# hmatuschek/libsdr

Hardware: AMD Instinct MI355X
Metric: Msamples/s through baseband->FIR->demod chain (higher is better)
Workload: dtype i16

## Files before the change

### include/sdrhip.h

```cpp
#ifndef SDRHIP_H
#define SDRHIP_H

#include <stddef.h>
#include <stdint.h>

#ifdef __cplusplus
extern "C" {
#endif

#define SDRHIP_VERSION 100

enum {
  SDRHIP_OK = 0,
  SDRHIP_E_INVALID = -1,
  SDRHIP_E_NODEVICE = -2,
  SDRHIP_E_HIP = -3,
  SDRHIP_E_NOMEM = -4,
  SDRHIP_E_UNSUPPORTED = -5,
  SDRHIP_E_SIZE = -6
};

enum {
  SDRHIP_EPI_NONE = 0,
  SDRHIP_EPI_FM = 1,
  SDRHIP_EPI_AM = 2,
  SDRHIP_EPI_USB = 3
};

typedef struct sdrhip_ctx sdrhip_ctx;
typedef struct sdrhip_timer sdrhip_timer;
typedef struct sdrhip_iqbb_i16 sdrhip_iqbb_i16;
typedef struct sdrhip_fir sdrhip_fir;
typedef struct sdrhip_demod sdrhip_demod;
typedef struct sdrhip_subsample sdrhip_subsample;
typedef struct sdrhip_fftconv sdrhip_fftconv;
typedef struct sdrhip_fbb_f32 sdrhip_fbb_f32;

int sdrhip_version(void);
const char *sdrhip_strerror(int code);
const char *sdrhip_last_error(void);
int sdrhip_device_count(int *count);

int sdrhip_ctx_create(int device, void *stream, sdrhip_ctx **out);
int sdrhip_ctx_destroy(sdrhip_ctx *ctx);
int sdrhip_ctx_synchronize(sdrhip_ctx *ctx);
int sdrhip_ctx_device_name(sdrhip_ctx *ctx, char *buf, size_t len);

int sdrhip_malloc(sdrhip_ctx *ctx, size_t bytes, void **dptr);
int sdrhip_free(sdrhip_ctx *ctx, void *dptr);
int sdrhip_memcpy_h2d(sdrhip_ctx *ctx, void *dst_dev, const void *src_host, size_t bytes);
int sdrhip_memcpy_d2h(sdrhip_ctx *ctx, void *dst_host, const void *src_dev, size_t bytes);
int sdrhip_memset(sdrhip_ctx *ctx, void *dst_dev, int value, size_t bytes);

int sdrhip_timer_create(sdrhip_ctx *ctx, sdrhip_timer **out);
int sdrhip_timer_start(sdrhip_timer *t);
int sdrhip_timer_stop(sdrhip_timer *t);
int sdrhip_timer_elapsed_ms(sdrhip_timer *t, float *ms);
int sdrhip_timer_destroy(sdrhip_timer *t);

int sdrhip_bench_stream_read(sdrhip_ctx *ctx, const void *dev, size_t bytes, int iters, double *gb_per_s);

int sdrhip_design_iqbb_taps(double filter_freq, double width, double sample_rate, int order, int32_t *taps);
int sdrhip_design_bb_taps(double filter_freq, double width, double sample_rate, int order, int32_t *taps);
int sdrhip_design_iqbb_decim(double sample_rate, int sub_sample, double out_rate, int *decim);
int sdrhip_design_freqshift_lut_i16(int32_t *lut);
int sdrhip_design_freqshift_inc(double shift, double sample_rate, uint32_t *inc);
int sdrhip_design_fir_lowpass(int order, double upper_freq, double sample_rate, double *alpha);
int sdrhip_design_fftfilt_kernel(int n, double fmin, double fmax, double sample_rate, float *h);
int sdrhip_design_fftfilt_spectrum(int n, const float *h, float *spectrum);
int sdrhip_design_fftfilt_kernel_f64(int n, double fmin, double fmax, double sample_rate, double *h);
int sdrhip_design_fftfilt_spectrum_f64(int n, const double *h, double *spectrum);

int sdrhip_iqbb_i16_create(sdrhip_ctx *ctx, const int32_t *taps, int order, const int32_t *lut,
                           uint32_t lut_inc, int negative, int decim, int channels, size_t max_in,
                           int epilogue, sdrhip_iqbb_i16 **out);
int sdrhip_iqbb_i16_path(sdrhip_iqbb_i16 *h, int *path);
int sdrhip_iqbb_i16_kernel_names(sdrhip_iqbb_i16 *h, char *buf, size_t len);
int sdrhip_iqbb_i16_plan_info(sdrhip_iqbb_i16 *h, int *info, int n);
int sdrhip_iqbb_i16_out_count(sdrhip_iqbb_i16 *h, size_t n_in, size_t *n_out);
int sdrhip_iqbb_i16_process(sdrhip_iqbb_i16 *h, const int16_t *in_host, size_t n_in, size_t in_stride,
                            void *out_host, size_t out_stride, size_t *n_out);
int sdrhip_iqbb_i16_process_dev(sdrhip_iqbb_i16 *h, const int16_t *in_dev, size_t n_in, size_t in_stride,
                                void *out_dev, size_t out_stride, size_t *n_out);
int sdrhip_iqbb_i16_process_dev_multi(sdrhip_iqbb_i16 *h, const int16_t *in_dev, size_t n_buffers, size_t n_per_buffer, size_t in_stride,
                                      void *out_dev, size_t out_stride, size_t *n_out_per_buffer, size_t *n_out_total);
enum { SDRHIP_IN_CS16 = 0, SDRHIP_IN_CU8 = 1 };
int sdrhip_iqbb_i16_set_input_format(sdrhip_iqbb_i16 *h, int format);
int sdrhip_bb_i16_create(sdrhip_ctx *ctx, const int32_t *taps, int order, const int32_t *lut,
                         uint32_t lut_inc, int negative, int decim, int channels, size_t max_in,
                         int epilogue, sdrhip_iqbb_i16 **out);
int sdrhip_design_freqshift_lut_i8(int32_t *lut);
int sdrhip_iqbb_i8_create(sdrhip_ctx *ctx, const int32_t *taps, int order, const int32_t *lut, uint32_t lut_inc,
                          int negative, int decim, int channels, size_t max_in, int epilogue, sdrhip_iqbb_i16 **out);
int sdrhip_iqbb_i16_set_taps(sdrhip_iqbb_i16 *h, const int32_t *taps);
int sdrhip_iqbb_i16_set_shift(sdrhip_iqbb_i16 *h, uint32_t lut_inc, int negative);
int sdrhip_iqbb_i16_reset(sdrhip_iqbb_i16 *h, int keep_history);
enum { SDRHIP_KEEP_RING = 1, SDRHIP_KEEP_FM = 2, SDRHIP_KEEP_COUNTERS = 4 };
int sdrhip_iqbb_i16_adopt_state(sdrhip_iqbb_i16 *h, sdrhip_iqbb_i16 *from, int what);
int sdrhip_iqbb_i16_destroy(sdrhip_iqbb_i16 *h);

typedef struct sdrhip_tuner_i16 sdrhip_tuner_i16;
int sdrhip_tuner_i16_create(sdrhip_ctx *ctx, const int32_t *taps, int order, const int32_t *lut, const uint32_t *lut_inc,
                            const int *negative, int decim, int channels, size_t max_in, int epilogue, sdrhip_tuner_i16 **out);
int sdrhip_tunermodes_i16_create(sdrhip_ctx *ctx, const int32_t *taps, int order, const int32_t *lut, const uint32_t *lut_inc,
                                 const int *negative, const int *modes, int decim, int channels, size_t max_in,
                                 sdrhip_tuner_i16 **out);
int sdrhip_tunerbb_i16_create(sdrhip_ctx *ctx, const int32_t *taps, int order, const int32_t *lut, const uint32_t *lut_inc,
                              const int *negative, int decim, int channels, size_t max_in, int epilogue, sdrhip_tuner_i16 **out);
int sdrhip_tunermodes_bb_i16_create(sdrhip_ctx *ctx, const int32_t *taps, int order, const int32_t *lut, const uint32_t *lut_inc,
                                    const int *negative, const int *modes, int decim, int channels, size_t max_in,
                                    sdrhip_tuner_i16 **out);
int sdrhip_tunermodes_i16_set_mode(sdrhip_tuner_i16 *h, int channel, int mode);
int sdrhip_tunermodes_i16_get_modes(sdrhip_tuner_i16 *h, int *modes, int n);
int sdrhip_tuner_i16_kernel_names(sdrhip_tuner_i16 *h, char *buf, size_t len);
int sdrhip_tuner_i16_plan_info(sdrhip_tuner_i16 *h, size_t n_in, int *info, int n);
int sdrhip_tuner_i16_out_count(sdrhip_tuner_i16 *h, size_t n_in, size_t *n_out);
int sdrhip_tuner_i16_process(sdrhip_tuner_i16 *h, const void *in_host, size_t n_in, void *out_host, size_t out_stride, size_t *n_out);
int sdrhip_tuner_i16_process_dev(sdrhip_tuner_i16 *h, const void *in_dev, size_t n_in, void *out_dev, size_t out_stride, size_t *n_out);
int sdrhip_tuner_i16_set_taps(sdrhip_tuner_i16 *h, int channel, const int32_t *taps);
int sdrhip_tuner_i16_set_shift(sdrhip_tuner_i16 *h, int channel, uint32_t lut_inc, int negative);
int sdrhip_tuner_i16_set_input_format(sdrhip_tuner_i16 *h, int format);
int sdrhip_tuner_i16_reset(sdrhip_tuner_i16 *h, int keep_history);
int sdrhip_tuner_i16_destroy(sdrhip_tuner_i16 *h);

enum {
  SDRHIP_FIR_CS16_EXACT = 0,
  SDRHIP_FIR_CF32 = 1
};
int sdrhip_fir_create(sdrhip_ctx *ctx, int kind, const double *alpha, int order, int decim, int channels,
                      size_t max_in, int epilogue, sdrhip_fir **out);
int sdrhip_fir_out_count(sdrhip_fir *h, size_t n_in, size_t *n_out);
int sdrhip_fir_kernel_names(sdrhip_fir *h, size_t n_in, char *buf, size_t len);
int sdrhip_fir_last_kernels(sdrhip_fir *h, char *buf, size_t len);
int sdrhip_fir_process(sdrhip_fir *h, const void *in_host, size_t n_in, size_t in_stride, void *out_host,
                       size_t out_stride, size_t *n_out);
int sdrhip_fir_process_dev(sdrhip_fir *h, const void *in_dev, size_t n_in, size_t in_stride, void *out_dev,
                           size_t out_stride, size_t *n_out);
int sdrhip_fir_set_taps(sdrhip_fir *h, const double *alpha);
int sdrhip_fir_reset(sdrhip_fir *h);
int sdrhip_fir_destroy(sdrhip_fir *h);

enum { SDRHIP_T_CS16 = 0, SDRHIP_T_CF32 = 1, SDRHIP_T_CS8 = 2 ,
       SDRHIP_T_CF64 = 3  };
int sdrhip_demod_create(sdrhip_ctx *ctx, int kind, int dtype, int channels, size_t max_in, int inplace_fm0,
                        sdrhip_demod **out);
int sdrhip_demod_process(sdrhip_demod *h, const void *in_host, size_t n, size_t in_stride, void *out_host,
                         size_t out_stride);
int sdrhip_demod_process_dev(sdrhip_demod *h, const void *in_dev, size_t n, size_t in_stride, void *out_dev,
                             size_t out_stride);
int sdrhip_demod_reset(sdrhip_demod *h);
int sdrhip_demod_destroy(sdrhip_demod *h);

typedef struct sdrhip_deemph sdrhip_deemph;
int sdrhip_design_fmdeemph_alpha(double sample_rate, int *alpha);
int sdrhip_deemph_i16_create(sdrhip_ctx *ctx, int alpha, int channels, size_t max_in, sdrhip_deemph **out);
int sdrhip_deemph_i16_process(sdrhip_deemph *h, const int16_t *in_host, size_t n, size_t in_stride, int16_t *out_host,
                              size_t out_stride);
int sdrhip_deemph_i16_process_dev(sdrhip_deemph *h, const int16_t *in_dev, size_t n, size_t in_stride, int16_t *out_dev,
                                  size_t out_stride);
int sdrhip_deemph_i16_kernel_names(sdrhip_deemph *h, size_t n, char *buf, size_t len);
int sdrhip_deemph_i16_reset(sdrhip_deemph *h);
int sdrhip_deemph_i16_destroy(sdrhip_deemph *h);

int sdrhip_design_fsk_lut(double sample_rate, float baud, float freq, int *corr_len, float *lut, int lut_cap);
enum { SDRHIP_DET_FSK = 0, SDRHIP_DET_ASK = 1 };
typedef struct sdrhip_detector sdrhip_detector;
int sdrhip_detector_create(sdrhip_ctx *ctx, int kind, const float *mark_lut, const float *space_lut, int corr_len, int invert,
                           int channels, size_t max_in, sdrhip_detector **out);
int sdrhip_detector_process(sdrhip_detector *h, const int16_t *in_host, size_t n, size_t in_stride, uint8_t *out_host,
                            size_t out_stride);
int sdrhip_detector_process_dev(sdrhip_detector *h, const int16_t *in_dev, size_t n, size_t in_stride, uint8_t *out_dev,
                                size_t out_stride);
int sdrhip_detector_kernel_names(sdrhip_detector *h, char *buf, size_t len);
int sdrhip_detector_reset(sdrhip_detector *h);
int sdrhip_detector_destroy(sdrhip_detector *h);
enum { SDRHIP_BITS_NORMAL = 0, SDRHIP_BITS_TRANSITION = 1 };
typedef struct sdrhip_bits sdrhip_bits;
int sdrhip_bits_create(sdrhip_ctx *ctx, double sample_rate, float baud, int mode, int channels, size_t max_in, sdrhip_bits **out);
int sdrhip_bits_corr_len(sdrhip_bits *h, int *corr_len);
int sdrhip_bits_out_capacity(sdrhip_bits *h, size_t n_in, size_t *cap);
int sdrhip_bits_process(sdrhip_bits *h, const uint8_t *sym_host, size_t n, size_t in_stride, uint8_t *bits_host, size_t out_stride,
                        uint32_t *counts_host);
int sdrhip_bits_process_dev(sdrhip_bits *h, const uint8_t *sym_dev, size_t n, size_t in_stride, uint8_t *bits_dev, size_t out_stride,
                            uint32_t *counts_dev);
int sdrhip_bits_kernel_names(sdrhip_bits *h, char *buf, size_t len);
int sdrhip_bits_reset(sdrhip_bits *h);
int sdrhip_bits_destroy(sdrhip_bits *h);
int sdrhip_detectorbank_create(sdrhip_ctx *ctx, const int *kinds, const int *corr_len, const int *invert, const float *mark_luts,
                               const float *space_luts, int max_corr_len, int channels, size_t max_in, sdrhip_detector **out);
int sdrhip_detectorbank_set_channel(sdrhip_detector *h, int channel, int kind, const float *mark_lut, const float *space_lut,
                                    int corr_len, int invert);
int sdrhip_bitsbank_create(sdrhip_ctx *ctx, double sample_rate, const float *baud, const int *mode, int channels, size_t max_in,
                           int max_corr_len, sdrhip_bits **out);
int sdrhip_bitsbank_set_channel(sdrhip_bits *h, int channel, float baud, int mode);
int sdrhip_bitsbank_channel_info(sdrhip_bits *h, int channel, size_t n_in, int *corr_len, float *omega_min, float *omega_max,
                                 size_t *cap);

int sdrhip_subsample_create(sdrhip_ctx *ctx, int dtype, size_t n, int channels, size_t max_in,
                            sdrhip_subsample **out);
int sdrhip_subsample_out_count(sdrhip_subsample *h, size_t n_in, size_t *n_out);
int sdrhip_subsample_process(sdrhip_subsample *h, const void *in_host, size_t n_in, size_t in_stride,
                             void *out_host, size_t out_stride, size_t *n_out);
int sdrhip_subsample_process_dev(sdrhip_subsample *h, const void *in_dev, size_t n_in, size_t in_stride,
                                 void *out_dev, size_t out_stride, size_t *n_out);
int sdrhip_subsample_reset(sdrhip_subsample *h);
int sdrhip_subsample_destroy(sdrhip_subsample *h);

enum {
  SDRHIP_FFTCONV_OLA = 0,
  SDRHIP_FFTCONV_OLS = 1
};
int sdrhip_fftconv_create(sdrhip_ctx *ctx, int mode, int fft_size, const float *kernel, int n_taps,
                          int channels, size_t max_in, sdrhip_fftconv **out);
int sdrhip_fftconv_create_bank(sdrhip_ctx *ctx, int mode, int fft_size, const float *kernels, int n_taps, int n_bands,
                               int channels, size_t max_in, sdrhip_fftconv **out);
int sdrhip_fftconv_bands(sdrhip_fftconv *h, int *n_bands);
int sdrhip_fftconv_set_kernel(sdrhip_fftconv *h, int band, const float *kernel);
int sdrhip_fftconv_process(sdrhip_fftconv *h, const float *in_host, size_t n_in, size_t in_stride,
                           float *out_host, size_t out_stride);
int sdrhip_fftconv_process_dev(sdrhip_fftconv *h, const float *in_dev, size_t n_in, size_t in_stride,
                               float *out_dev, size_t out_stride);
int sdrhip_fftconv_last_kernels(sdrhip_fftconv *h, char *buf, size_t len);
int sdrhip_fftconv_reset(sdrhip_fftconv *h);
int sdrhip_fftconv_destroy(sdrhip_fftconv *h);
int sdrhip_fftconv_f64_create_bank(sdrhip_ctx *ctx, int mode, int fft_size, const double *kernels, int n_taps, int n_bands,
                                   int channels, size_t max_in, sdrhip_fftconv **out);
int sdrhip_fftconv_f64_set_kernel(sdrhip_fftconv *h, int band, const double *kernel);
int sdrhip_fftconv_f64_process(sdrhip_fftconv *h, const double *in_host, size_t n_in, size_t in_stride,
                               double *out_host, size_t out_stride);
int sdrhip_fftconv_f64_process_dev(sdrhip_fftconv *h, const double *in_dev, size_t n_in, size_t in_stride,
                                   double *out_dev, size_t out_stride);
// ... 70 lines not shown
```

### libsdr_amd/abi.py

```python
import ctypes as C
import os
import re

_HERE = os.path.dirname(os.path.abspath(__file__))
ROOT = os.path.dirname(_HERE)
SO_PATH = os.path.join(_HERE, "libsdrhip.so")
if os.environ.get("SDRHIP_LIB"):
    SO_PATH = os.path.abspath(os.environ["SDRHIP_LIB"])
HEADER = os.path.join(ROOT, "include", "sdrhip.h")

OK, E_INVALID, E_NODEVICE, E_HIP, E_NOMEM, E_UNSUPPORTED, E_SIZE = 0, -1, -2, -3, -4, -5, -6
EPI_NONE, EPI_FM, EPI_AM, EPI_USB = 0, 1, 2, 3
FIR_CS16_EXACT, FIR_CF32 = 0, 1
T_CS16, T_CF32, T_CS8, T_CF64 = 0, 1, 2, 3
IN_CS16, IN_CU8 = 0, 1
KEEP_RING, KEEP_FM, KEEP_COUNTERS = 1, 2, 4
FFTCONV_OLA, FFTCONV_OLS = 0, 1
DET_FSK, DET_ASK = 0, 1
BITS_NORMAL, BITS_TRANSITION = 0, 1


class SdrHipError(RuntimeError):
    def __init__(self, code, text):
        super().__init__("sdrhip error %d: %s" % (code, text))
        self.code = code


def header_functions():
    src = open(HEADER).read()
    src = re.sub(r"/\*.*?\*/", "", src, flags=re.S)
    return sorted(set(re.findall(r"\b(sdrhip_[a-z0-9_]+)\s*\(", src)))


def _signatures():
    vp, sz = C.c_void_p, C.c_size_t
    pvp, psz = C.POINTER(C.c_void_p), C.POINTER(C.c_size_t)
    i32p, f32p, f64p = C.POINTER(C.c_int32), C.POINTER(C.c_float), C.POINTER(C.c_double)
    return {
        "sdrhip_version": (C.c_int, []),
        "sdrhip_strerror": (C.c_char_p, [C.c_int]),
        "sdrhip_last_error": (C.c_char_p, []),
        "sdrhip_device_count": (C.c_int, [C.POINTER(C.c_int)]),
        "sdrhip_ctx_create": (C.c_int, [C.c_int, vp, pvp]),
        "sdrhip_ctx_destroy": (C.c_int, [vp]),
        "sdrhip_ctx_synchronize": (C.c_int, [vp]),
        "sdrhip_ctx_device_name": (C.c_int, [vp, C.c_char_p, sz]),
        "sdrhip_malloc": (C.c_int, [vp, sz, pvp]),
        "sdrhip_free": (C.c_int, [vp, vp]),
        "sdrhip_memcpy_h2d": (C.c_int, [vp, vp, vp, sz]),
        "sdrhip_memcpy_d2h": (C.c_int, [vp, vp, vp, sz]),
        "sdrhip_memset": (C.c_int, [vp, vp, C.c_int, sz]),
        "sdrhip_timer_create": (C.c_int, [vp, pvp]),
        "sdrhip_timer_start": (C.c_int, [vp]),
        "sdrhip_timer_stop": (C.c_int, [vp]),
        "sdrhip_timer_elapsed_ms": (C.c_int, [vp, f32p]),
        "sdrhip_timer_destroy": (C.c_int, [vp]),
        "sdrhip_bench_stream_read": (C.c_int, [vp, vp, sz, C.c_int, C.POINTER(C.c_double)]),
        "sdrhip_design_iqbb_taps": (C.c_int, [C.c_double, C.c_double, C.c_double, C.c_int, i32p]),
        "sdrhip_design_bb_taps": (C.c_int, [C.c_double, C.c_double, C.c_double, C.c_int, i32p]),
        "sdrhip_design_iqbb_decim": (C.c_int, [C.c_double, C.c_int, C.c_double, C.POINTER(C.c_int)]),
        "sdrhip_design_freqshift_lut_i16": (C.c_int, [i32p]),
        "sdrhip_design_freqshift_inc": (C.c_int, [C.c_double, C.c_double, C.POINTER(C.c_uint32)]),
        "sdrhip_design_fir_lowpass": (C.c_int, [C.c_int, C.c_double, C.c_double, f64p]),
        "sdrhip_design_fftfilt_kernel": (C.c_int, [C.c_int, C.c_double, C.c_double, C.c_double, f32p]),
        "sdrhip_design_fftfilt_spectrum": (C.c_int, [C.c_int, f32p, f32p]),
        "sdrhip_iqbb_i16_create": (C.c_int, [vp, i32p, C.c_int, i32p, C.c_uint32, C.c_int, C.c_int, C.c_int,
                                             sz, C.c_int, pvp]),
        "sdrhip_bb_i16_create": (C.c_int, [vp, i32p, C.c_int, i32p, C.c_uint32, C.c_int, C.c_int, C.c_int,
                                           sz, C.c_int, pvp]),
        "sdrhip_iqbb_i16_path": (C.c_int, [vp, C.POINTER(C.c_int)]),
        "sdrhip_design_freqshift_lut_i8": (C.c_int, [i32p]),
        "sdrhip_iqbb_i8_create": (C.c_int, [vp, i32p, C.c_int, i32p, C.c_uint32, C.c_int, C.c_int, C.c_int, sz, C.c_int, pvp]),
        "sdrhip_iqbb_i16_kernel_names": (C.c_int, [vp, C.c_char_p, sz]),
        "sdrhip_iqbb_i16_set_taps": (C.c_int, [vp, i32p]),
        "sdrhip_iqbb_i16_set_shift": (C.c_int, [vp, C.c_uint32, C.c_int]),
        "sdrhip_iqbb_i16_out_count": (C.c_int, [vp, sz, psz]),
        "sdrhip_iqbb_i16_process": (C.c_int, [vp, vp, sz, sz, vp, sz, psz]),
        "sdrhip_iqbb_i16_process_dev": (C.c_int, [vp, vp, sz, sz, vp, sz, psz]),
        "sdrhip_iqbb_i16_plan_info": (C.c_int, [vp, C.POINTER(C.c_int), C.c_int]),
        "sdrhip_iqbb_i16_process_dev_multi": (C.c_int, [vp, vp, sz, sz, sz, vp, sz, psz, psz]),
        "sdrhip_iqbb_i16_reset": (C.c_int, [vp, C.c_int]),
        "sdrhip_iqbb_i16_adopt_state": (C.c_int, [vp, vp, C.c_int]),
        "sdrhip_iqbb_i16_destroy": (C.c_int, [vp]),
        "sdrhip_tuner_i16_create": (C.c_int, [vp, i32p, C.c_int, i32p, C.POINTER(C.c_uint32), C.POINTER(C.c_int), C.c_int, C.c_int,
                                              sz, C.c_int, pvp]),
        "sdrhip_tunermodes_i16_create": (C.c_int, [vp, i32p, C.c_int, i32p, C.POINTER(C.c_uint32), C.POINTER(C.c_int), C.POINTER(C.c_int),
                                                   C.c_int, C.c_int, sz, pvp]),
        "sdrhip_tunerbb_i16_create": (C.c_int, [vp, i32p, C.c_int, i32p, C.POINTER(C.c_uint32), C.POINTER(C.c_int), C.c_int, C.c_int,
                                                sz, C.c_int, pvp]),
        "sdrhip_tunermodes_bb_i16_create": (C.c_int, [vp, i32p, C.c_int, i32p, C.POINTER(C.c_uint32), C.POINTER(C.c_int), C.POINTER(C.c_int),
                                                      C.c_int, C.c_int, sz, pvp]),
        "sdrhip_tunermodes_i16_set_mode": (C.c_int, [vp, C.c_int, C.c_int]),
        "sdrhip_tunermodes_i16_get_modes": (C.c_int, [vp, C.POINTER(C.c_int), C.c_int]),
        "sdrhip_tuner_i16_kernel_names": (C.c_int, [vp, C.c_char_p, sz]),
        "sdrhip_tuner_i16_plan_info": (C.c_int, [vp, sz, C.POINTER(C.c_int), C.c_int]),
        "sdrhip_tuner_i16_out_count": (C.c_int, [vp, sz, psz]),
        "sdrhip_tuner_i16_process": (C.c_int, [vp, vp, sz, vp, sz, psz]),
        "sdrhip_tuner_i16_process_dev": (C.c_int, [vp, vp, sz, vp, sz, psz]),
        "sdrhip_tuner_i16_set_taps": (C.c_int, [vp, C.c_int, i32p]),
        "sdrhip_tuner_i16_set_shift": (C.c_int, [vp, C.c_int, C.c_uint32, C.c_int]),
        "sdrhip_tuner_i16_set_input_format": (C.c_int, [vp, C.c_int]),
        "sdrhip_tuner_i16_reset": (C.c_int, [vp, C.c_int]),
        "sdrhip_tuner_i16_destroy": (C.c_int, [vp]),
        "sdrhip_fir_create": (C.c_int, [vp, C.c_int, f64p, C.c_int, C.c_int, C.c_int, sz, C.c_int, pvp]),
        "sdrhip_fir_out_count": (C.c_int, [vp, sz, psz]),
        "sdrhip_fir_kernel_names": (C.c_int, [vp, sz, C.c_char_p, sz]),
        "sdrhip_fir_last_kernels": (C.c_int, [vp, C.c_char_p, sz]),
        "sdrhip_fir_process": (C.c_int, [vp, vp, sz, sz, vp, sz, psz]),
        "sdrhip_fir_process_dev": (C.c_int, [vp, vp, sz, sz, vp, sz, psz]),
        "sdrhip_fir_reset": (C.c_int, [vp]),
        "sdrhip_fir_set_taps": (C.c_int, [vp, f64p]),
        "sdrhip_fir_destroy": (C.c_int, [vp]),
        "sdrhip_demod_create": (C.c_int, [vp, C.c_int, C.c_int, C.c_int, sz, C.c_int, pvp]),
        "sdrhip_demod_process": (C.c_int, [vp, vp, sz, sz, vp, sz]),
        "sdrhip_demod_process_dev": (C.c_int, [vp, vp, sz, sz, vp, sz]),
        "sdrhip_demod_reset": (C.c_int, [vp]),
        "sdrhip_demod_destroy": (C.c_int, [vp]),
        "sdrhip_design_fmdeemph_alpha": (C.c_int, [C.c_double, C.POINTER(C.c_int)]),
        "sdrhip_deemph_i16_create": (C.c_int, [vp, C.c_int, C.c_int, sz, pvp]),
        "sdrhip_deemph_i16_process": (C.c_int, [vp, vp, sz, sz, vp, sz]),
        "sdrhip_deemph_i16_process_dev": (C.c_int, [vp, vp, sz, sz, vp, sz]),
        "sdrhip_deemph_i16_kernel_names": (C.c_int, [vp, sz, C.c_char_p, sz]),
        "sdrhip_deemph_i16_reset": (C.c_int, [vp]),
        "sdrhip_deemph_i16_destroy": (C.c_int, [vp]),
        "sdrhip_design_fsk_lut": (C.c_int, [C.c_double, C.c_float, C.c_float, C.POINTER(C.c_int), f32p, C.c_int]),
        "sdrhip_detector_create": (C.c_int, [vp, C.c_int, f32p, f32p, C.c_int, C.c_int, C.c_int, sz, pvp]),
        "sdrhip_detector_process": (C.c_int, [vp, vp, sz, sz, vp, sz]),
        "sdrhip_detector_process_dev": (C.c_int, [vp, vp, sz, sz, vp, sz]),
        "sdrhip_detector_kernel_names": (C.c_int, [vp, C.c_char_p, sz]),
        "sdrhip_detector_reset": (C.c_int, [vp]),
        "sdrhip_detector_destroy": (C.c_int, [vp]),
        "sdrhip_bits_create": (C.c_int, [vp, C.c_double, C.c_float, C.c_int, C.c_int, sz, pvp]),
        "sdrhip_bits_corr_len": (C.c_int, [vp, C.POINTER(C.c_int)]),
        "sdrhip_bits_out_capacity": (C.c_int, [vp, sz, psz]),
        "sdrhip_bits_process": (C.c_int, [vp, vp, sz, sz, vp, sz, vp]),
        "sdrhip_bits_process_dev": (C.c_int, [vp, vp, sz, sz, vp, sz, vp]),
        "sdrhip_bits_kernel_names": (C.c_int, [vp, C.c_char_p, sz]),
        "sdrhip_bits_reset": (C.c_int, [vp]),
        "sdrhip_bits_destroy": (C.c_int, [vp]),
        "sdrhip_detectorbank_create": (C.c_int, [vp, C.POINTER(C.c_int), C.POINTER(C.c_int), C.POINTER(C.c_int), f32p, f32p,
                                                         C.c_int, C.c_int, sz, pvp]),
        "sdrhip_detectorbank_set_channel": (C.c_int, [vp, C.c_int, C.c_int, f32p, f32p, C.c_int, C.c_int]),
        "sdrhip_bitsbank_create": (C.c_int, [vp, C.c_double, f32p, C.POINTER(C.c_int), C.c_int, sz, C.c_int, pvp]),
        "sdrhip_bitsbank_set_channel": (C.c_int, [vp, C.c_int, C.c_float, C.c_int]),
        "sdrhip_bitsbank_channel_info": (C.c_int, [vp, C.c_int, sz, C.POINTER(C.c_int), f32p, f32p, psz]),
        "sdrhip_iqbb_i16_set_input_format": (C.c_int, [vp, C.c_int]),
        "sdrhip_subsample_create": (C.c_int, [vp, C.c_int, sz, C.c_int, sz, pvp]),
        "sdrhip_subsample_out_count": (C.c_int, [vp, sz, psz]),
        "sdrhip_subsample_process": (C.c_int, [vp, vp, sz, sz, vp, sz, psz]),
        "sdrhip_subsample_process_dev": (C.c_int, [vp, vp, sz, sz, vp, sz, psz]),
        "sdrhip_subsample_reset": (C.c_int, [vp]),
        "sdrhip_subsample_destroy": (C.c_int, [vp]),
        "sdrhip_fftconv_create": (C.c_int, [vp, C.c_int, C.c_int, f32p, C.c_int, C.c_int, sz, pvp]),
        "sdrhip_fftconv_process": (C.c_int, [vp, vp, sz, sz, vp, sz]),
        "sdrhip_fftconv_process_dev": (C.c_int, [vp, vp, sz, sz, vp, sz]),
        "sdrhip_fftconv_last_kernels": (C.c_int, [vp, C.c_char_p, sz]),
        "sdrhip_fftconv_reset": (C.c_int, [vp]),
        "sdrhip_fftconv_destroy": (C.c_int, [vp]),
        "sdrhip_fft_c2c": (C.c_int, [vp, C.c_int, C.c_int, C.c_int, vp, vp]),
        "sdrhip_fft_c2c_f64": (C.c_int, [vp, C.c_int, C.c_int, C.c_int, vp, vp]),
        "sdrhip_fft_exec": (C.c_int, [vp, C.c_int, C.c_int, C.c_int, vp, vp]),
        "sdrhip_fbb_f32_create": (C.c_int, [vp, C.c_double, C.c_double, f64p, C.c_int, C.c_int, C.c_int, sz, pvp]),
        "sdrhip_fbb_f32_out_count": (C.c_int, [vp, sz, psz]),
        "sdrhip_fbb_f32_kernel_names": (C.c_int, [vp, sz, C.c_char_p, sz]),
        "sdrhip_fbb_f32_last_kernels": (C.c_int, [vp, C.c_char_p, sz]),
        "sdrhip_fbb_f32_process": (C.c_int, [vp, vp, sz, sz, vp, sz, psz]),
        "sdrhip_fbb_f32_process_dev": (C.c_int, [vp, vp, sz, sz, vp, sz, psz]),
        "sdrhip_fbb_f32_reset": (C.c_int, [vp]),
        "sdrhip_fbb_f32_set_taps": (C.c_int, [vp, f64p]),
        "sdrhip_fbb_f32_set_shift": (C.c_int, [vp, C.c_double]),
        "sdrhip_fbb_f32_destroy": (C.c_int, [vp]),
        "sdrhip_fftconv_create_bank": (C.c_int, [vp, C.c_int, C.c_int, f32p, C.c_int, C.c_int, C.c_int, sz, pvp]),
        "sdrhip_fftconv_bands": (C.c_int, [vp, C.POINTER(C.c_int)]),
        "sdrhip_fftconv_set_kernel": (C.c_int, [vp, C.c_int, f32p]),
        "sdrhip_design_fftfilt_kernel_f64": (C.c_int, [C.c_int, C.c_double, C.c_double, C.c_double, f64p]),
        "sdrhip_design_fftfilt_spectrum_f64": (C.c_int, [C.c_int, f64p, f64p]),
        "sdrhip_fftconv_f64_create_bank": (C.c_int, [vp, C.c_int, C.c_int, f64p, C.c_int, C.c_int, C.c_int, sz, pvp]),
        "sdrhip_fftconv_f64_set_kernel": (C.c_int, [vp, C.c_int, f64p]),
        "sdrhip_fftconv_f64_process": (C.c_int, [vp, vp, sz, sz, vp, sz]),
        "sdrhip_fftconv_f64_process_dev": (C.c_int, [vp, vp, sz, sz, vp, sz]),
        "sdrhip_fft_plan_create": (C.c_int, [vp, C.c_int, C.c_int, pvp]),
        "sdrhip_fft_plan_form": (C.c_int, [vp, C.POINTER(C.c_char_p)]),
        "sdrhip_fft_plan_exec_dev": (C.c_int, [vp, C.c_int, C.c_int, vp, vp]),
        "sdrhip_fft_plan_exec": (C.c_int, [vp, C.c_int, vp, vp]),
        "sdrhip_fft_plan_destroy": (C.c_int, [vp]),
        "sdrhip_fftsink_create": (C.c_int, [vp, C.c_int, C.c_int, C.c_int, sz, pvp]),
        "sdrhip_fftsink_process": (C.c_int, [vp, vp, sz, sz, vp, sz]),
        "sdrhip_fftsink_process_dev": (C.c_int, [vp, vp, sz, sz, vp, sz]),
        "sdrhip_fftsink_form": (C.c_int, [vp, C.POINTER(C.c_char_p)]),
        "sdrhip_fftsink_destroy": (C.c_int, [vp]),
        "sdrhip_fftsource_create": (C.c_int, [vp, C.c_int, C.c_int, vp, C.c_int, sz, pvp]),
        "sdrhip_fftsource_set_kernel": (C.c_int, [vp, vp]),
        "sdrhip_fftsource_process": (C.c_int, [vp, vp, sz, sz, vp, sz]),
        "sdrhip_fftsource_process_dev": (C.c_int, [vp, vp, sz, sz, vp, sz]),
        "sdrhip_fftsource_form": (C.c_int, [vp, C.POINTER(C.c_char_p)]),
        "sdrhip_fftsource_reset": (C.c_int, [vp]),
        "sdrhip_fftsource_destroy": (C.c_int, [vp]),
        "sdrhip_comm_create": (C.c_int, [C.POINTER(C.c_int), C.c_int, pvp]),
        "sdrhip_comm_size": (C.c_int, [vp, C.POINTER(C.c_int)]),
        "sdrhip_comm_ctx": (C.c_int, [vp, C.c_int, pvp]),
        "sdrhip_comm_transport": (C.c_int, [vp, C.POINTER(C.c_char_p)]),
        "sdrhip_comm_broadcast": (C.c_int, [vp, pvp, sz, C.c_int]),
        "sdrhip_comm_gather": (C.c_int, [vp, pvp, psz, vp, C.c_int]),
        "sdrhip_comm_gather_begin": (C.c_int, [vp, C.c_int, pvp, psz, vp, C.c_int]),
        "sdrhip_comm_gather_wait": (C.c_int, [vp, C.c_int]),
        "sdrhip_comm_synchronize": (C.c_int, [vp]),
        "sdrhip_comm_destroy": (C.c_int, [vp]),
        "sdrhip_host_alloc": (C.c_int, [sz, pvp]),
        "sdrhip_host_free": (C.c_int, [vp]),
        "sdrhip_host_register": (C.c_int, [vp, sz]),
        "sdrhip_host_unregister": (C.c_int, [vp]),
        "sdrhip_memcpy_h2d_async": (C.c_int, [vp, vp, vp, sz]),
        "sdrhip_memcpy_d2h_async": (C.c_int, [vp, vp, vp, sz]),
        "sdrhip_memcpy2d_d2h_async": (C.c_int, [vp, vp, sz, vp, sz, sz, sz]),
    }


SIGNATURES = _signatures()

_lib = None


def lib():
    global _lib
    if _lib is None:
        if not os.path.exists(SO_PATH):
            raise ImportError("libsdrhip.so not built: run `python -c 'import __graft_entry__ as g; g.build()'` "
                              "(make -C libsdr_amd/csrc); there is no CPU fallback")
        L = C.CDLL(SO_PATH)
        for name, (res, args) in SIGNATURES.items():
            fn = getattr(L, name)
            fn.restype, fn.argtypes = res, args
# ... 10 lines not shown
```

### libsdr_amd/csrc/iqbb_common.hpp

```cpp
#pragma once
#include "fm_phi.hpp"
#include "sdrhip_internal.hpp"

#include <cstdlib>

using namespace sdrhip;

namespace sdrhip {

constexpr int TPB = 256;
constexpr int R = 8;
constexpr int TI = TPB * R;
constexpr int TAPC = 8;
constexpr int MAX_ORDER = 2048;

typedef short s16x2 __attribute__((ext_vector_type(2)));
typedef int v4i __attribute__((ext_vector_type(4)));
typedef int v16i __attribute__((ext_vector_type(16)));

struct IqbbArgs {
  const uint32_t *in; long in_stride;
  int in_cu8;
  int in_real;
  int i8;
  const uint32_t *hist_old; uint32_t *hist_new;
  const int2 *acc_old; int2 *acc_new;
  const short *fm_old; short *fm_new;
  const uint2 *taps;
  const int2 *lut; uint32_t inc; int negative;
  int OP, HH, D, N;
  uint32_t n0_lo;
  int base0_rel;
  int n_groups;
  int n_out;
  int extra0;
  int CG, OG, ovl;
  int CGr;
  void *out; long out_stride; int epilogue;
  const v4i *tapfrag; int cre, cim;
  unsigned ah_mask;
  int lpg;
  int tiles, tpw;
  int bt_hi;
  int fix_lo, fix_hi;
};

constexpr int HOT_EPI_PARTIAL = 4;

struct HotArgs {
  const void *in; long in_stride;
  void *out; long out_stride;
  const v4i *tapfrag; const int2 *lut;
  uint32_t inc, n0_lo; int negative;
  int base0_rel, OG, ovl;
  int t_lo, t_hi, tpw;
  int G, U, dq, dr;
  int N, n_out;
  int C;
  int cre, cim;
  int D, GS, lpg_sh; float inv_d;
  short *philast; int philast_stride;
  int tiles_h;
  long long reserved[2];
  int2 *part; int part_stride;
  int Dreal, base_real;
  int fin_groups, fin_out, fin_epi;
  int mb_q1, mb_p, mb_qlast; unsigned mb_magic;
  unsigned long long *stamps;
};

}

namespace {

__device__ __forceinline__ uint32_t cast_cu8(uint32_t u16) {
  return (((u16 & 0xffu) + 129u) & 0xffu) << 8 | ((((u16 >> 8) & 0xffu) + 129u) & 0xffu) << 24;
}
__device__ __forceinline__ uint32_t raw_x(const IqbbArgs &a, int c, long rel) {
  if (a.in_cu8) return cast_cu8(reinterpret_cast<const uint16_t *>(a.in)[(long)c * a.in_stride + rel]);
  if (a.in_real) return (uint32_t)(int)reinterpret_cast<const short *>(a.in)[(long)c * a.in_stride + rel];
  if (a.i8) {
    const uint32_t u = reinterpret_cast<const uint16_t *>(a.in)[(long)c * a.in_stride + rel];
    return ((uint32_t)(int)(signed char)(u & 0xffu) & 0xffffu) | ((uint32_t)(int)(signed char)(u >> 8) << 16);
  }
  return a.in[(long)c * a.in_stride + rel];
}
__device__ __forceinline__ uint32_t load_x(const IqbbArgs &a, int c, int rel) {
  if (rel >= 0) return rel < a.N ? raw_x(a, c, rel) : 0u;
  const int h = a.HH + rel;
  return h >= 0 ? a.hist_old[(long)c * a.HH + h] : 0u;
}

__device__ __forceinline__ int dot2(uint32_t x, uint32_t k, int acc) {
  return __builtin_amdgcn_sdot2(__builtin_bit_cast(s16x2, x), __builtin_bit_cast(s16x2, k), acc, false);
}

__device__ __forceinline__ int2 rotate_i16(uint32_t inc, int negative, const int2 *lut_s, int2 r, uint32_t n_lo) {
  if (inc == 0) return r;
  uint32_t idx = (__umul24(n_lo & 32767u, inc & 32767u) & 32767u) >> 8;
  if (negative) idx = 127u - idx;
  const int2 L = lut_s[idx];
  int2 v;
  v.x = (int)((unsigned)__mul24(L.x, r.x) - (unsigned)__mul24(L.y, r.y)) >> 16;
  v.y = (int)((unsigned)__mul24(L.x, r.y) + (unsigned)__mul24(L.y, r.x)) >> 16;
  return v;
}
__device__ __forceinline__ int2 rotate(const IqbbArgs &a, const int2 *lut_s, int2 r, uint32_t n_lo) {
  if (a.i8) {
    r.x = (short)r.x; r.y = (short)r.y;
    if (a.inc == 0) return r;
    uint32_t idx = (__umul24(n_lo & 32767u, a.inc & 32767u) & 32767u) >> 8;
    if (a.negative) idx = 127u - idx;
    const int2 L = lut_s[idx];
    int2 v;
    v.x = (int)(short)(mulw(L.x, r.x) - mulw(L.y, r.y)) >> 8;
    v.y = (int)(short)(mulw(L.x, r.y) + mulw(L.y, r.x)) >> 8;
    return v;
  }
  return rotate_i16(a.inc, a.negative, lut_s, r, n_lo);
}

__device__ __forceinline__ int box_div(int s, int D) {
  const int n = mulw(D, D);
  const int r = mulw(s, D);
  if (n == 0) return 0;
  if (r == (int)0x80000000 && n == -1) return r;
  return r / n;
}


struct BigdArgs {
  const int2 *part; int part_stride;
  int D, base0_rel, N, n_groups, n_out, epi, C;
  const int2 *acc_old; int2 *acc_new;
  const short *fm_old; short *fm_new;
  void *out; long out_stride;
};
__device__ __forceinline__ void bigd_finish_group(const BigdArgs &a, int c, int q) {
  const int2 *pc = a.part + (long)c * a.part_stride;
  auto group_sum = [&](int g) {
    const long lo = g == 0 ? 0 : (long)a.base0_rel + (long)g * a.D, hi = min((long)a.base0_rel + (long)(g + 1) * a.D, (long)a.N);
    int2 s = make_int2(0, 0);
    if (g == 0) s = a.acc_old[c];
    for (long sl = lo >> 9; sl <= (hi - 1) >> 9; sl++) {
      const long x0 = sl << 9;
      const int gf = x0 < a.base0_rel ? 0 : (int)((x0 - a.base0_rel) / a.D);
      const int2 v = pc[3 * sl + (g - gf)];
      s.x = (int)((unsigned)s.x + (unsigned)v.x); s.y = (int)((unsigned)s.y + (unsigned)v.y);
    }
    return s;
  };
  const int2 s = group_sum(q);
  const bool emits = q < a.n_out;
  if (q == a.n_groups - 1) a.acc_new[c] = emits ? make_int2(0, 0) : s;
  if (!emits) return;
  const int yr = (short)box_div(s.x, a.D), yi = (short)box_div(s.y, a.D);
  if (a.epi == SDRHIP_EPI_NONE) {
    reinterpret_cast<uint32_t *>(a.out)[(long)c * a.out_stride + q] = ((uint32_t)(uint16_t)yr) | ((uint32_t)(uint16_t)yi << 16);
  } else if (a.epi == SDRHIP_EPI_AM) {
    reinterpret_cast<short *>(a.out)[(long)c * a.out_stride + q] = am_i16(yr, yi);
  } else if (a.epi == SDRHIP_EPI_USB) {
    reinterpret_cast<short *>(a.out)[(long)c * a.out_stride + q] = usb_i16(yr, yi);
  } else {
    const int phi = fm_phi(yr, yi);
    short o;
    if (q == 0) o = (short)yr;
    else if (q == 1) o = (short)((int)a.fm_old[c] - phi);
    else {
      const int2 sp = group_sum(q - 1);
      o = (short)(fm_phi((short)box_div(sp.x, a.D), (short)box_div(sp.y, a.D)) - phi);
    }
    reinterpret_cast<short *>(a.out)[(long)c * a.out_stride + q] = o;
    if (q == a.n_out - 1 && a.n_out >= 2) a.fm_new[c] = (short)phi;
  }
}

__device__ __forceinline__ void finalize_group(const IqbbArgs &a, int c, const int2 *lut_s, uint32_t *ybuf, int ql, int q, int2 s, int D) {
  if (q == 0) {
    const int2 carry = a.acc_old[c];
    s.x = (int)((unsigned)s.x + (unsigned)carry.x);
    s.y = (int)((unsigned)s.y + (unsigned)carry.y);
    if (a.extra0) {
      int er = 0, ei = 0;
      for (int i = 0; i < a.OP; i++) {
        const uint32_t x = load_x(a, c, -(a.OP - 1) + i);
        const uint2 k = a.taps[i];
        er = dot2(x, k.x, er); ei = dot2(x, k.y, ei);
      }
      const int2 v = rotate(a, lut_s, make_int2(er >> 14, ei >> 14), a.n0_lo);
      s.x = (int)((unsigned)s.x + (unsigned)v.x);
      s.y = (int)((unsigned)s.y + (unsigned)v.y);
    }
  }
  const bool emits = q < a.n_out;
  if (emits) {
    int yr = (short)box_div(s.x, D), yi = (short)box_div(s.y, D);
    if (a.i8) { yr = (signed char)yr; yi = (signed char)yi; }
    ybuf[ql] = ((uint32_t)(uint16_t)yr) | ((uint32_t)(uint16_t)yi << 16);
    if (a.epilogue == SDRHIP_EPI_FM) reinterpret_cast<int *>(ybuf + a.CGr)[ql] = fm_phi(yr, yi);
  }
  if (q == a.n_groups - 1) a.acc_new[c] = emits ? make_int2(0, 0) : s;
}

__device__ __forceinline__ void epilogue_and_roll(const IqbbArgs &a, int c, int tile, int tid, int q0, int groups_here,
                                                  const uint32_t *ybuf) {
  for (int ql = a.ovl + tid; ql < groups_here; ql += TPB) {
    const int j = q0 + ql;
    if (j >= a.n_out) continue;
    const uint32_t y = ybuf[ql];
    const int yr = (short)(y & 0xffffu), yi = (short)(y >> 16);
    if (a.epilogue == SDRHIP_EPI_NONE) {
      if (a.i8) reinterpret_cast<uint16_t *>(a.out)[(long)c * a.out_stride + j] = (uint16_t)((yr & 0xff) | ((yi & 0xff) << 8));
      else reinterpret_cast<uint32_t *>(a.out)[(long)c * a.out_stride + j] = y;
    } else {
      short o;
      if (a.epilogue == SDRHIP_EPI_AM) o = am_i16(yr, yi);
      else if (a.epilogue == SDRHIP_EPI_USB) o = usb_i16(yr, yi);
      else {
        const int *phib = reinterpret_cast<const int *>(ybuf + a.CGr);
        const int phi = phib[ql];
// ... 229 lines not shown
```

### libsdr_amd/csrc/iqbb_hot.hpp

```cpp
#pragma once
#include <atomic>
#include "iqbb_common.hpp"

#include <iterator>
#include <type_traits>
#include <utility>

namespace sdrhip {

enum { HOT_CS16 = 0, HOT_CU8 = 1, HOT_REAL = 2, HOT_CS8 = 3 };
constexpr bool hot_one_plane(int in) { return in == HOT_CU8 || in == HOT_CS8; }
constexpr int hot_halo(int S, int in) { return in == HOT_REAL ? 32 * S - 16 : 16 * (S - 1); }
constexpr int hot_win(int S, int in) { return 512 + hot_halo(S, in) + (in == HOT_REAL ? 16 : 0); }
constexpr int hot_plb(int S, int in) { return in == HOT_REAL ? hot_win(S, in) : 2 * hot_win(S, in) + 32; }
constexpr int hot_bufb(int S, int in) { return hot_one_plane(in) ? hot_plb(S, in) : 2 * hot_plb(S, in); }
constexpr int hot_lds_bytes(int S, int NH, int in, int NW, bool wide) {
  return (wide ? 4096 : 1024) + (S + NH) * 1024 + NW * 2 * hot_bufb(S, in);
}
constexpr int hot_lds_cap(int NW, int S = 0) { return S >= 33 ? 163840 : NW == 4 ? 40960 : NW == 8 ? 81920 : 163840; }
constexpr bool hot_wide(int S, int NH, int in, int NW, int extra = 0) { return hot_lds_bytes(S, NH, in, NW, true) + extra <= hot_lds_cap(NW, S); }
constexpr int hot_anyd_extra(int, int, bool = true, int NW = 4) { return NW * 512; }

constexpr int hot_sd_extra(int S, int in, bool rot, int NW = 4) { return (hot_bufb(S, in) >= 2048 ? 0 : NW * 2048) + (rot ? 0 : NW * 2048); }
constexpr bool hot_sd_fits(int S, int NH, int in, bool rot, int NW = 4) { return hot_lds_bytes(S, NH, in, NW, false) + hot_sd_extra(S, in, rot, NW) <= hot_lds_cap(NW); }
constexpr int hot_sd_nw(int S, int NH, int in, bool rot, int nw0) {
  for (int nw = nw0; nw <= 16; nw *= 2) if (hot_sd_fits(S, NH, in, rot, nw)) return nw;
  return 0;
}

struct HotRange { int S0, NH, NW; };
constexpr HotRange hot_ranges_2[] = {{0, 2, 4}};
constexpr HotRange hot_ranges_3[] = {{1, 2, 4}, {0, 3, 4}};
constexpr HotRange hot_ranges_5[] = {{1, 3, 4}, {0, 5, 4}};
constexpr HotRange hot_ranges_9[] = {{3, 3, 4}, {2, 5, 4}, {1, 7, 4}, {0, 9, 4}};
constexpr HotRange hot_ranges_17[] = {{6, 5, 8}, {4, 9, 8}, {0, 17, 16}};
constexpr HotRange hot_ranges_33[] = {{12, 9, 8}, {16, 9, 8}, {18, 9, 8}, {8, 17, 8}, {0, 33, 8}};
struct HotLoRange { int L0, NL; };
constexpr HotLoRange hot_lo_ranges_9[] = {{1, 7}, {0, 9}};
template <int S> constexpr HotLoRange hot_lo_full[] = {{0, S}};

constexpr int hot_steps[] = {2, 3, 5, 9, 17, 33};
template <int S> constexpr auto &hot_ranges_of() {
  if constexpr (S == 2) return hot_ranges_2;
  else if constexpr (S == 3) return hot_ranges_3;
  else if constexpr (S == 5) return hot_ranges_5;
  else if constexpr (S == 9) return hot_ranges_9;
  else if constexpr (S == 17) return hot_ranges_17;
  else return hot_ranges_33;
}
template <int S> constexpr auto &hot_lo_ranges_of() {
  if constexpr (S == 9) return hot_lo_ranges_9;
  else return hot_lo_full<S>;
}
template <int N, class F, int... I>
void hot_pick(int i, F &&f, std::integer_sequence<int, I...>) {
  if (i < 0 || i >= N) i = N - 1;
  ((i == I ? f(std::integral_constant<int, I>{}) : void()), ...);
}
template <int N, class F> void hot_pick(int i, F &&f) { hot_pick<N>(i, f, std::make_integer_sequence<int, N>{}); }
template <class F> bool hot_with_steps(int S, F &&f) {
  constexpr int N = (int)std::size(hot_steps);
  for (int i = 0; i < N; i++)
    if (hot_steps[i] == S) { hot_pick<N>(i, [&](auto k) { f(std::integral_constant<int, hot_steps[decltype(k)::value]>{}); }); return true; }
  return false;
}
inline const HotRange *hot_ranges(int S, int *count) {
  const HotRange *r = nullptr;
  *count = 0;
  hot_with_steps(S, [&](auto s) { r = hot_ranges_of<s>(); *count = (int)std::size(hot_ranges_of<s>()); });
  return r;
}
inline const HotLoRange *hot_lo_ranges(int S, int *count) {
  const HotLoRange *r = nullptr;
  *count = 0;
  hot_with_steps(S, [&](auto s) { r = hot_lo_ranges_of<s>(); *count = (int)std::size(hot_lo_ranges_of<s>()); });
  return r;
}

enum { HOT_D8 = 0, HOT_ANYD = 1, HOT_SD = 2 };
constexpr bool hot_class(int form, int S, int in) {
  if (in == HOT_REAL) return S == 3 || S == 5 || S == 9;
  if (in == HOT_CS8) return form != HOT_SD && (S == 2 || S == 3 || S == 5 || S == 9);
  return S == 2 || S == 3 || S == 5 || S == 9 || S == 17 || (S == 33 && form != HOT_SD);
}
constexpr int hot_sd_range_waves(int S, const HotRange &r, int in, bool rot) {
  const int nw = hot_sd_nw(S, r.NH, in, rot, r.NW);
  return in != HOT_REAL || nw == 4 ? nw : 0;
}
inline int hot_sd_waves(int S, int in, int range, bool rot) {
  int n = 0;
  const HotRange *rg = hot_ranges(S, &n);
  if (!hot_class(HOT_SD, S, in)) return 0;
  return hot_sd_range_waves(S, rg[range >= 0 && range < n ? range : n - 1], in, rot);
}

struct HotLaunch { unsigned grid; hipStream_t stream; };
template <int FORM, int S, int IN> struct HotClass {
  static void launch(int range, int lo, bool rot, int epi, const HotLaunch &, const HotArgs &, const IqbbArgs &);
};
void hot_launch(int form, int S, int in, int range, int lo, bool rot, int epi, const HotLaunch &, const HotArgs &, const IqbbArgs &);

}

namespace {

__device__ __forceinline__ uint32_t ror8(uint32_t x) { return __builtin_amdgcn_alignbit(x, x, 8); }
__device__ __forceinline__ uint32_t add129_rot(uint32_t x) {
  unsigned k = 0x81008100u;
  asm("" : "+s"(k));
  uint32_t t;
  asm("v_pk_add_u16 %0, %1, %2" : "=v"(t) : "v"(x), "s"(k));
  t = ror8(t);
  asm("v_pk_add_u16 %0, %1, %2" : "=v"(t) : "v"(t), "s"(k));
  return t;
}

__host__ __device__ __forceinline__ bool slice_is_hot(int halo, int win, int base0_rel, int OG, int ovl, int N, int n_out, int tile, int w,
                                                      int D = 8, int GS = 64) {
  const int qf = tile * OG - ovl + w * (GS - ovl);
  const int ws = base0_rel + qf * D - halo;
  return ws >= 0 && ws + win <= N && qf >= (GS == 1 ? 2 : 1) && qf + GS - 1 < n_out - 1;
}

template <int S, int S0, int NH, bool ROT, int EPI, int IN, int NW, bool DG = false, bool SD = false, int L0 = 0, int NL = S>
__device__ __forceinline__ void iqbb_hot_body(const HotArgs &a, const IqbbArgs &b_kernarg) {
  IqbbArgs b_late;
  const IqbbArgs &b = DG ? b_late : b_kernarg;
  constexpr bool CS8 = IN == HOT_CS8, CU8 = IN == HOT_CU8 || CS8, REAL = IN == HOT_REAL;
  static_assert(!CS8 || (!SD && EPI != HOT_EPI_PARTIAL && (EPI == SDRHIP_EPI_NONE || EPI == SDRHIP_EPI_FM)), "int8 chain: /8 and any-D forms, no demodulator or FM");
  constexpr bool PART = EPI == HOT_EPI_PARTIAL;
  static_assert(!PART || (DG && !SD), "partial sums: a variant of the any-D form");
  static_assert(!SD || DG, "the small-decimation form is a variant of the any-D form");

  const int DD = DG ? a.D : 8, GS = DG ? a.GS : 64;
  static_assert(S >= 2 && S0 >= 0 && NH >= 1 && S0 + NH <= S, "high-plane range inside the K loop");
  static_assert(L0 >= 0 && L0 + NL <= S && S0 >= L0 && S0 + NH <= L0 + NL, "high-plane range inside the low-plane range");
  static_assert(!REAL || NW == 4, "real input: 4-wave workgroups");
  static_assert(NW == 4 || NW == 8 || NW == 16, "4-wave virtual workgroups");
  constexpr int HALO = hot_halo(S, IN), WIN = hot_win(S, IN), PLB = hot_plb(S, IN), HALF = PLB / 2, BUFB = hot_bufb(S, IN);
  constexpr int NPIECE = (IN == HOT_CS16 ? 4 * WIN : 2 * WIN) / 16;
  constexpr int KSB = REAL ? 32 : 16;
  constexpr int FSH = REAL ? 16 : 14;
  constexpr int NDMA = (NPIECE + 63) / 64;
  constexpr int LASTL = NPIECE - 64 * (NDMA - 1);
  static_assert(NDMA <= 4, "immediate offsets 0 / 1024 / 2048 / 3072");
  constexpr bool WIDE = SD ? false : hot_wide(S, NH, IN, NW, DG ? hot_anyd_extra(S, IN, ROT, NW) : 0);
  static_assert(!SD || hot_sd_fits(S, NH, IN, ROT, NW), "small-decimation form: LDS budget");
  constexpr int NBUF = 2;
  static_assert(hot_lds_bytes(S, NH, IN, NW, WIDE) <= hot_lds_cap(NW, S), "LDS budget for 4 waves per SIMD");
  constexpr int TBLW = WIDE ? 1024 : 256;
  constexpr int TPBH = 64 * NW;
  extern __shared__ __attribute__((aligned(16))) uint32_t smem[];
  int2 *lut_s = reinterpret_cast<int2 *>(smem);
  v4i *taps_s = reinterpret_cast<v4i *>(smem + TBLW);
  const int tid = threadIdx.x, w = __builtin_amdgcn_readfirstlane(tid >> 6), l = tid & 63, n = l & 31, h = l >> 5;
  const int wv = w & 3;
  const int bx = (int)blockIdx.x * (NW / 4) + (w >> 2), gx = (int)gridDim.x * (NW / 4);
  char *wbase = reinterpret_cast<char *>(smem + TBLW + (S + NH) * 64 * 4) + w * (NBUF * BUFB);
  char *pendb = reinterpret_cast<char *>(smem + TBLW + (S + NH) * 64 * 4) + NW * (NBUF * BUFB) + w * 512;
  char *gscb = reinterpret_cast<char *>(smem + TBLW + (S + NH) * 64 * 4) + NW * (NBUF * BUFB) + (SD ? 0 : NW * 512) + w * 2048;
  char *gscb2 = gscb + NW * 2048;
  for (int i = tid; i < S * 64; i += TPBH) taps_s[i] = a.tapfrag[(2 * (i >> 6) + 1) * 64 + (i & 63)];
  for (int i = tid; i < NH * 64; i += TPBH) taps_s[S * 64 + i] = a.tapfrag[(2 * (S0 + (i >> 6))) * 64 + (i & 63)];
  if (tid < 256) {
    const int2 e = a.lut[(tid & 127) ^ (a.negative ? 127 : 0)];
    if (WIDE) reinterpret_cast<v4i *>(smem)[tid] = v4i{e.x, e.y, -e.y, 0};
    else if (tid < 128) lut_s[tid] = e;
  }

  const int OGw = GS - a.ovl, gw = wv * OGw;
  int hl = a.t_lo, hh = a.t_hi;
  while (hl < hh && !slice_is_hot(HALO, WIN, a.base0_rel, a.OG, a.ovl, a.N, a.n_out, hl, wv, DD, GS)) hl++;
  while (hh > hl && !slice_is_hot(HALO, WIN, a.base0_rel, a.OG, a.ovl, a.N, a.n_out, hh - 1, wv, DD, GS)) hh--;
  int u = bx;
  int c = u / a.G, g = u - c * a.G;
  int tile = max(a.t_lo + g * a.tpw, hl), tend = min(a.t_lo + g * a.tpw + a.tpw, hh);
  auto next_unit = [&](int &u_, int &c_, int &g_, int &tile_, int &tend_) {
    do {
      u_ += gx; c_ += a.dq; g_ += a.dr;
      if (g_ >= a.G) { g_ -= a.G; c_++; }
      tile_ = max(a.t_lo + g_ * a.tpw, hl); tend_ = min(a.t_lo + g_ * a.tpw + a.tpw, hh);
    } while (u_ < a.U && tile_ >= tend_);
  };
  if (u < a.U && tile >= tend) next_unit(u, c, g, tile, tend);
  const uint32_t lane_byte = 16u * (uint32_t)l;
  constexpr int SB = IN == HOT_CS16 ? 4 : 2;
  constexpr int OB = (EPI == SDRHIP_EPI_NONE && !CS8) ? 4 : 2;
  const int tile_in_bytes = a.OG * DD * SB, tile_out_bytes = a.OG * OB;
  const uint32_t tile_cnt = (uint32_t)(a.OG * DD) * a.inc;
  const uint32_t cnt0 = (a.n0_lo + (uint32_t)(a.base0_rel + (gw - a.ovl) * DD)) * a.inc;
  auto chan_src = [&](int c_) { return reinterpret_cast<const char *>(a.in) + ((long)c_ * a.in_stride + (a.base0_rel + (gw - a.ovl) * DD - HALO)) * SB; };
  auto chan_out = [&](int c_) { return reinterpret_cast<char *>(a.out) + ((long)c_ * a.out_stride + (gw - a.ovl)) * OB; };
  const char *srcb = chan_src(c);
  char *outb = chan_out(c);
  auto dma_issue = [&](const char *src, char *buf) {
    const unsigned ldsb = __builtin_amdgcn_readfirstlane((unsigned)(uintptr_t)buf);
#pragma clang diagnostic push
#pragma clang diagnostic ignored "-Winline-asm"
    if (NDMA == 1) {
      if (l < LASTL) asm volatile("s_mov_b32 m0, %1\n\ts_nop 0\n\tglobal_load_lds_dwordx4 %0, off" :: "v"(src), "s"(ldsb) : "memory", "m0");
    } else if (NDMA == 2) {
      asm volatile("s_mov_b32 m0, %1\n\ts_nop 0\n\tglobal_load_lds_dwordx4 %0, off" :: "v"(src), "s"(ldsb) : "memory", "m0");
      if (l < LASTL) asm volatile("s_mov_b32 m0, %1\n\ts_nop 0\n\tglobal_load_lds_dwordx4 %0, off offset:1024" :: "v"(src), "s"(ldsb) : "memory", "m0");
    } else if (NDMA == 3) {
      asm volatile("s_mov_b32 m0, %1\n\ts_nop 0\n\tglobal_load_lds_dwordx4 %0, off\n\tglobal_load_lds_dwordx4 %0, off offset:1024" :: "v"(src), "s"(ldsb) : "memory", "m0");
      if (l < LASTL) asm volatile("s_mov_b32 m0, %1\n\ts_nop 0\n\tglobal_load_lds_dwordx4 %0, off offset:2048" :: "v"(src), "s"(ldsb) : "memory", "m0");
    } else {
      asm volatile("s_mov_b32 m0, %1\n\ts_nop 0\n\tglobal_load_lds_dwordx4 %0, off\n\tglobal_load_lds_dwordx4 %0, off offset:1024\n\tglobal_load_lds_dwordx4 %0, off offset:2048"
                   :: "v"(src), "s"(ldsb) : "memory", "m0");
      if (l < LASTL) asm volatile("s_mov_b32 m0, %1\n\ts_nop 0\n\tglobal_load_lds_dwordx4 %0, off offset:3072" :: "v"(src), "s"(ldsb) : "memory", "m0");
    }
#pragma clang diagnostic pop
  };
  if (u < a.U) dma_issue(srcb + (long)tile * tile_in_bytes + lane_byte, wbase);
  __syncthreads();

  int dofs[NDMA];
#pragma unroll
  for (int k = 0; k < NDMA; k++) {
    const int p = l + 64 * k;
    if (REAL) dofs[k] = 8 * p;
    else if (CU8) dofs[k] = (p & 1) * HALF + (p >> 1) * 16;
    else { const int j = p >> 1; dofs[k] = (j & 1) * HALF + (j >> 1) * 16 + (p & 1) * 8; }
  }
  const int coff = REAL ? 16 * (n + h) : h * HALF + 16 * n;
  const uint32_t lane_cnt = (uint32_t)(MF_BLK * n + 8 * h) * a.inc;
  const uint32_t lane_pair = (lane_cnt & 0xffffu) | ((lane_cnt + a.inc) << 16);

  v16i cinit;
#pragma unroll
  for (int r = 0; r < 16; r++) cinit[r] = (r & 1) ? a.cim : a.cre;
  asm volatile("" : "+v"(cinit));

#ifdef K1_STAMPS
  unsigned long long st_acc[6] = {0, 0, 0, 0, 0, 0}, st_t = __builtin_amdgcn_s_memtime();
  const unsigned long long st_r0 = __builtin_amdgcn_s_memrealtime();
  unsigned st_tiles = 0;
#define K1_STAMP(i_) do { asm volatile("s_waitcnt lgkmcnt(0)" ::: "memory"); const unsigned long long t_ = __builtin_amdgcn_s_memtime(); st_acc[i_] += t_ - st_t; st_t = t_; } while (0)
#else
#define K1_STAMP(i_) do { } while (0)
#endif
  constexpr int K1_PRIO_ROT = 1, K1_PRIO_SHIFT = 11;
  unsigned prio_it = 0;
  const unsigned prio_slot = __builtin_amdgcn_s_getreg((3 << 11) | 4) & 3u;

  auto stageP = [&](char *cb) __attribute__((always_inline)) {
    uint4 x[NDMA];
#pragma unroll
    for (int k = 0; k < NDMA; k++)
      if (k < NDMA - 1 || l < LASTL) x[k] = *reinterpret_cast<const uint4 *>(cb + 16 * (l + 64 * k));
    asm volatile("" ::: "memory");
#pragma unroll
    for (int k = 0; k < NDMA; k++) {
      if (k < NDMA - 1 || l < LASTL) {
        if (CS8) {
          *reinterpret_cast<uint4 *>(cb + dofs[k]) = make_uint4(x[k].x, x[k].y, x[k].z, x[k].w);
        } else if (CU8) {
          *reinterpret_cast<uint4 *>(cb + dofs[k]) = make_uint4(add129_rot(x[k].x), add129_rot(x[k].y), add129_rot(x[k].z), add129_rot(x[k].w));
        } else {
          uint2 l2, h2;
          l2.x = __builtin_amdgcn_perm(x[k].y, x[k].x, 0x06040200u) ^ 0x80808080u;
          l2.y = __builtin_amdgcn_perm(x[k].w, x[k].z, 0x06040200u) ^ 0x80808080u;
          h2.x = __builtin_amdgcn_perm(x[k].y, x[k].x, 0x07050301u);
          h2.y = __builtin_amdgcn_perm(x[k].w, x[k].z, 0x07050301u);
          *reinterpret_cast<uint2 *>(cb + dofs[k]) = l2;
          *reinterpret_cast<uint2 *>(cb + PLB + dofs[k]) = h2;
        }
      }
    }
  };
  struct KOps { v4i uh, ul, Al, Ah; };
  auto stageK_begin = [&](const char *cb, KOps &o) __attribute__((always_inline)) {
    const char *pl = cb + coff + KSB * L0, *ph = cb + (CU8 ? 0 : PLB) + coff + KSB * L0;
    o.uh = *reinterpret_cast<const v4i *>(ph); o.ul = o.uh;
    if (!CU8) o.ul = *reinterpret_cast<const v4i *>(pl);
    o.Al = taps_s[L0 * 64 + l]; o.Ah = o.Al;
    if (S0 == L0) o.Ah = taps_s[S * 64 + l];
  };
  auto stageK = [&](const char *cb, KOps &o, v16i &acc_hh, v16i &acc_mid, v16i &acc_ll) __attribute__((always_inline)) {
    constexpr int SA = L0, SB = L0 + NL;
    const char *pl = cb + coff, *ph = cb + (CU8 ? 0 : PLB) + coff;
#pragma unroll
    for (int s = SA; s < SB; s++) {
      KOps nx = o;
      if (s + 1 < SB) {
        nx.uh = *reinterpret_cast<const v4i *>(ph + KSB * (s + 1));
        if (!CU8) nx.ul = *reinterpret_cast<const v4i *>(pl + KSB * (s + 1));
        nx.Al = taps_s[(s + 1) * 64 + l];
        if (s + 1 >= S0 && s + 1 < S0 + NH) nx.Ah = taps_s[(S + s + 1 - S0) * 64 + l];
      }
      acc_mid = __builtin_amdgcn_mfma_i32_32x32x32_i8(o.Al, o.uh, acc_mid, 0, 0, 0);
      asm volatile("" : "+v"(acc_mid));
      if (s >= S0 && s < S0 + NH) {
        acc_hh = __builtin_amdgcn_mfma_i32_32x32x32_i8(o.Ah, o.uh, acc_hh, 0, 0, 0);
        asm volatile("" : "+v"(acc_hh));
        if (!CU8) { acc_mid = __builtin_amdgcn_mfma_i32_32x32x32_i8(o.Ah, o.ul, acc_mid, 0, 0, 0); asm volatile("" : "+v"(acc_mid)); }
      }
      if (!CU8) { acc_ll = __builtin_amdgcn_mfma_i32_32x32x32_i8(o.Al, o.ul, acc_ll, 0, 0, 0); asm volatile("" : "+v"(acc_ll)); }
      o = nx;
    }
  };
  int tm_sp = 8, tm_a0 = 0, tm_a1 = 0;
  unsigned tm_m[4] = {0u, 0u, 0u, 0u};
  bool tm_end = false;
  if (DG) {
    const int Lb = 2 * n + h;
    const int g = (8 * Lb + DD - 1) / DD, pos = g * DD;
    tm_sp = (g <= GS && pos < 8 * Lb + 8) ? pos - 8 * Lb : 8;
    const int kk = min(l >> a.lpg_sh, GS - 1);
    const int b0 = (kk * DD) >> 3, b1 = ((kk + 1) * DD) >> 3, b1c = min(b1, 63);
    tm_a0 = 4 * ((b0 >> 1) + 32 * (b0 & 1));
    tm_a1 = 4 * ((b1c >> 1) + 32 * (b1c & 1));
    tm_end = b1 >= 64;
    const int spm = tm_sp < 8 ? tm_sp : (Lb == 63 && GS * DD == 512) ? 8 : 0;
#pragma unroll
    for (int jj = 0; jj < 4; jj++) tm_m[jj] = (2 * jj < spm ? 1u : 0u) | (2 * jj + 1 < spm ? 0x10000u : 0u);
  }
  (void)tm_sp; (void)tm_a0; (void)tm_a1; (void)tm_end; (void)tm_m;
  auto stageE = [&](auto edge_, const v16i &acc_hh, const v16i &acc_mid, const v16i &acc_ll, uint32_t wave_cnt, char *escr, int erel0,
                    int2 *pdst = nullptr, int ob0 = 0) __attribute__((always_inline)) {
    constexpr bool EDGE = decltype(edge_)::value;
    int L[8][3];
    if (ROT) {
      typedef int v2i __attribute__((ext_vector_type(2)));
#pragma unroll
      for (int jj = 0; jj < 4; jj++) {
        const uint32_t wc = (wave_cnt + 2u * jj * a.inc) & 0xffffu, wpair = wc | (wc << 16);
        uint32_t pr, o0, o1;
        asm("v_pk_add_u16 %0, %1, %2" : "=v"(pr) : "v"(lane_pair), "s"(wpair));
        if (WIDE) {
          asm("v_lshlrev_b32_sdwa %0, %1, %2 dst_sel:DWORD dst_unused:UNUSED_PAD src0_sel:DWORD src1_sel:BYTE_1" : "=v"(o0) : "s"(4), "v"(pr));
          asm("v_lshlrev_b32_sdwa %0, %1, %2 dst_sel:DWORD dst_unused:UNUSED_PAD src0_sel:DWORD src1_sel:BYTE_3" : "=v"(o1) : "s"(4), "v"(pr));
          const v4i e0 = *reinterpret_cast<__attribute__((address_space(3))) const v4i *>((uintptr_t)o0);
          const v4i e1 = *reinterpret_cast<__attribute__((address_space(3))) const v4i *>((uintptr_t)o1);
          L[2 * jj][0] = e0.x; L[2 * jj][1] = e0.y; L[2 * jj][2] = e0.z;
          L[2 * jj + 1][0] = e1.x; L[2 * jj + 1][1] = e1.y; L[2 * jj + 1][2] = e1.z;
        } else {
          o0 = (pr >> 5) & (127u << 3); o1 = (pr >> 21) & (127u << 3);
          const v2i e0 = *reinterpret_cast<__attribute__((address_space(3))) const v2i *>((uintptr_t)o0);
          const v2i e1 = *reinterpret_cast<__attribute__((address_space(3))) const v2i *>((uintptr_t)o1);
          L[2 * jj][0] = e0.x; L[2 * jj][1] = e0.y; L[2 * jj + 1][0] = e1.x; L[2 * jj + 1][1] = e1.y;
        }
      }
    }
    int2 sum = make_int2(0, 0);
    int vx[8], vy[8];
#pragma unroll
    for (int j = 0; j < 8; j++) {
      unsigned tre = ((unsigned)acc_hh[2 * j] << 8) + (unsigned)acc_mid[2 * j];
      unsigned tim = ((unsigned)acc_hh[2 * j + 1] << 8) + (unsigned)acc_mid[2 * j + 1];
      int rr, ri;
      if (CS8) {
        asm("v_bfe_i32 %0, %1, 14, 16" : "=v"(rr) : "v"(tre));
        asm("v_bfe_i32 %0, %1, 14, 16" : "=v"(ri) : "v"(tim));
      } else if (CU8) {
        asm("v_bfe_i32 %0, %1, 6, 18" : "=v"(rr) : "v"(tre));
        asm("v_bfe_i32 %0, %1, 6, 18" : "=v"(ri) : "v"(tim));
      } else {
        asm("" : "+v"(tre)); asm("" : "+v"(tim));
        rr = (int)((tre << 8) + (unsigned)acc_ll[2 * j]) >> FSH; ri = (int)((tim << 8) + (unsigned)acc_ll[2 * j + 1]) >> FSH;
      }
      if (EDGE) {
        const int rel = erel0 + j;
        if (rel < 0 || rel >= a.N) { rr = 0; ri = 0; }
      }
      if (ROT) {
        int x = WIDE ? mad24a(L[j][0], rr, mul24a(L[j][2], ri)) : sub32(mul24a(L[j][0], rr), mul24a(L[j][1], ri));
        int y = mad24a(L[j][0], ri, mul24a(L[j][1], rr));
        if (CS8) {
          asm("v_bfe_i32 %0, %0, 8, 8" : "+v"(x));
          asm("v_bfe_i32 %0, %0, 8, 8" : "+v"(y));
        }
        if (DG) { vx[j] = x; vy[j] = y; }
        else if (CS8) { sum.x += x; sum.y += y; }
        else { sum.x = add_hi16(x, sum.x); sum.y = add_hi16(y, sum.y); }
      } else if (DG) {
        vx[j] = rr; vy[j] = ri;
      } else {
        sum.x = (int)((unsigned)sum.x + (unsigned)rr); sum.y = (int)((unsigned)sum.y + (unsigned)ri);
      }
    }
    if (SD) {
      unsigned *gsc = reinterpret_cast<unsigned *>(BUFB >= 2048 ? escr : gscb);
      unsigned *gsy = reinterpret_cast<unsigned *>(BUFB >= 2048 ? gscb : gscb2);
      unsigned q8[8];
#pragma unroll
      for (int j = 0; j < 8; j++) q8[j] = ROT ? __builtin_amdgcn_perm((unsigned)vy[j], (unsigned)vx[j], 0x07060302u) : (unsigned)vx[j];
      *reinterpret_cast<uint4 *>(gsc + 8 * (2 * n + h)) = make_uint4(q8[0], q8[1], q8[2], q8[3]);
      *reinterpret_cast<uint4 *>(gsc + 8 * (2 * n + h) + 4) = make_uint4(q8[4], q8[5], q8[6], q8[7]);
      if (!ROT) {
        *reinterpret_cast<uint4 *>(gsy + 8 * (2 * n + h)) = make_uint4((unsigned)vy[0], (unsigned)vy[1], (unsigned)vy[2], (unsigned)vy[3]);
        *reinterpret_cast<uint4 *>(gsy + 8 * (2 * n + h) + 4) = make_uint4((unsigned)vy[4], (unsigned)vy[5], (unsigned)vy[6], (unsigned)vy[7]);
      }
      asm volatile("" ::: "memory");
      return sum;
    }
    if (DG) {
      int tX, tY, aX, aY;
      int px[4], py[4];
      if (ROT) {
#pragma unroll
        for (int jj = 0; jj < 4; jj++) {
          px[jj] = (int)__builtin_amdgcn_perm((unsigned)vx[2 * jj + 1], (unsigned)vx[2 * jj], CS8 ? 0x05040100u : 0x07060302u);
          py[jj] = (int)__builtin_amdgcn_perm((unsigned)vy[2 * jj + 1], (unsigned)vy[2 * jj], CS8 ? 0x05040100u : 0x07060302u);
        }
        auto dsum = [&](const int *p4, unsigned m0, unsigned m1, unsigned m2, unsigned m3) __attribute__((always_inline)) {
          int acc = __builtin_amdgcn_sdot2(__builtin_bit_cast(s16x2, p4[0]), __builtin_bit_cast(s16x2, m0), 0, false);
          acc = __builtin_amdgcn_sdot2(__builtin_bit_cast(s16x2, p4[1]), __builtin_bit_cast(s16x2, m1), acc, false);
          acc = __builtin_amdgcn_sdot2(__builtin_bit_cast(s16x2, p4[2]), __builtin_bit_cast(s16x2, m2), acc, false);
          return __builtin_amdgcn_sdot2(__builtin_bit_cast(s16x2, p4[3]), __builtin_bit_cast(s16x2, m3), acc, false);
        };
        unsigned ones = 0x00010001u;
        asm("" : "+s"(ones));
        tX = dsum(px, ones, ones, ones, ones); tY = dsum(py, ones, ones, ones, ones);
        if (!PART) { aX = dsum(px, tm_m[0], tm_m[1], tm_m[2], tm_m[3]); aY = dsum(py, tm_m[0], tm_m[1], tm_m[2], tm_m[3]); }
        else { aX = 0; aY = 0; }
      } else {
        int rx[8], ry[8];
        rx[0] = vx[0]; ry[0] = vy[0];
#pragma unroll
        for (int j = 1; j < 8; j++) { rx[j] = (int)((unsigned)rx[j - 1] + (unsigned)vx[j]); ry[j] = (int)((unsigned)ry[j - 1] + (unsigned)vy[j]); }
        const int ti = tm_sp - 1;
        const bool tb0 = (ti & 1) != 0, tb1 = (ti & 2) != 0, tb2 = (ti & 4) != 0, tok = ti >= 0 && ti <= 6;
        auto pick7 = [&](const int *v) __attribute__((always_inline)) {
          const int t0 = tb0 ? v[1] : v[0], t1 = tb0 ? v[3] : v[2], t2 = tb0 ? v[5] : v[4], t3 = v[6];
          const int u0 = tb1 ? t1 : t0, u1 = tb1 ? t3 : t2;
          return tok ? (tb2 ? u1 : u0) : 0;
        };
        tX = rx[7]; tY = ry[7];
        aX = pick7(rx); aY = pick7(ry);
        if (PART) {
#pragma unroll
          for (int j = 0; j < 8; j++) { vx[j] = rx[j]; vy[j] = ry[j]; }
        }
      }
      const auto tx = __builtin_amdgcn_permlane32_swap((unsigned)tX, (unsigned)tX, false, false);
      const auto ty = __builtin_amdgcn_permlane32_swap((unsigned)tY, (unsigned)tY, false, false);
      const int cx = (int)(tx[0] + tx[1]), cy = (int)(ty[0] + ty[1]);
      int ix = cx, iy = cy;
      ix += __builtin_amdgcn_update_dpp(0, ix, 0x111, 0xf, 0xf, true); iy += __builtin_amdgcn_update_dpp(0, iy, 0x111, 0xf, 0xf, true);
      ix += __builtin_amdgcn_update_dpp(0, ix, 0x112, 0xf, 0xf, true); iy += __builtin_amdgcn_update_dpp(0, iy, 0x112, 0xf, 0xf, true);
      ix += __builtin_amdgcn_update_dpp(0, ix, 0x114, 0xf, 0xf, true); iy += __builtin_amdgcn_update_dpp(0, iy, 0x114, 0xf, 0xf, true);
      ix += __builtin_amdgcn_update_dpp(0, ix, 0x118, 0xf, 0xf, true); iy += __builtin_amdgcn_update_dpp(0, iy, 0x118, 0xf, 0xf, true);
      ix += __builtin_amdgcn_update_dpp(0, ix, 0x142 , 0xa, 0xf, false); iy += __builtin_amdgcn_update_dpp(0, iy, 0x142, 0xa, 0xf, false);
      const int bpx = ix - (h ? (int)tx[1] : cx), bpy = iy - (h ? (int)ty[1] : cy);
      if (PART) {
        const int totx = __builtin_amdgcn_readlane(ix, 31), toty = __builtin_amdgcn_readlane(iy, 31);
        auto prefix_at = [&](int p, int &ox, int &oy) __attribute__((always_inline)) {
          const int j = p & 7, lb = p >> 3, ln = (lb >> 1) + 32 * (lb & 1);
          int wx = bpx, wy = bpy;
          if (ROT) {
            unsigned m[4];
// ... 333 lines not shown
    if (CS8) { yr = (signed char)yr; yi = (signed char)yi; }
    if (EPI == SDRHIP_EPI_NONE && CS8) {
      if (emits) reinterpret_cast<uint16_t *>(a.out)[(long)cc * a.out_stride + q] = (uint16_t)((yr & 0xff) | ((yi & 0xff) << 8));
    } else if (EPI == SDRHIP_EPI_NONE) {
      if (emits) reinterpret_cast<uint32_t *>(a.out)[(long)cc * a.out_stride + q] = ((uint32_t)(uint16_t)yr) | ((uint32_t)(uint16_t)yi << 16);
    } else if (EPI == SDRHIP_EPI_AM) {
      const short o = am_i16(yr, yi);
      if (emits) reinterpret_cast<short *>(a.out)[(long)cc * a.out_stride + q] = o;
    } else if (EPI == SDRHIP_EPI_USB) {
      const short o = usb_i16(yr, yi);
      if (emits) reinterpret_cast<short *>(a.out)[(long)cc * a.out_stride + q] = o;
    } else {
      const int phi = fm_phi(yr, yi);
      const int prev = __builtin_amdgcn_ds_bpermute(4 * (((k - 1) << lsh) & 63), phi);
      short o;
      if (q == 0) o = CS8 ? (short)((yr & 0xff) | ((yi & 0xff) << 8))
                          : (short)yr;
      else if (q == 1) o = (short)((int)b.fm_old[cc] - phi);
      else o = (short)((k > 0 ? prev : 0) - phi);
      if (emits) reinterpret_cast<short *>(a.out)[(long)cc * a.out_stride + q] = o;
      if (emits && k == GS - 1) a.philast[(long)cc * a.philast_stride + sid] = (short)phi;
      if (emits && q == b.n_out - 1 && b.n_out >= 2) b.fm_new[cc] = (short)phi;
    }
  };

#if defined(__HIP_DEVICE_COMPILE__)
  if (DG) {
    typedef const uint32_t __attribute__((address_space(4))) *KernargP;
    constexpr size_t B_OFF = (sizeof(HotArgs) + alignof(IqbbArgs) - 1) / alignof(IqbbArgs) * alignof(IqbbArgs);
    const char __attribute__((address_space(4))) *kp = (const char __attribute__((address_space(4))) *)__builtin_amdgcn_kernarg_segment_ptr();
    asm volatile("" : "+s"(kp) :: "memory");
    static_assert(sizeof(IqbbArgs) % 4 == 0, "copied by dwords");
    uint32_t *dst = reinterpret_cast<uint32_t *>(&b_late);
#pragma unroll
    for (int i = 0; i < (int)(sizeof(IqbbArgs) / 4); i++) dst[i] = ((KernargP)(kp + B_OFF))[i];
  }
#endif
  {
    char *cb = wbase;
    for (int cc = bx; cc < a.C; cc += gx) {
      for (int t = 0; t < (DG ? a.tiles_h : b.tiles); t = DG ? t + 1 : (t == 0 ? max(b.bt_hi, 1) : t + 1)) {
        const int q0 = t * a.OG - a.ovl, groups_here = DG ? 0 : min(b.CG, b.n_groups - q0);
        if (DG) { if ((t >= hl && t < hh) || (q0 + gw) >= b.n_groups) continue; }
        else if (slice_is_hot(HALO, WIN, a.base0_rel, a.OG, a.ovl, a.N, a.n_out, t, wv) || gw + a.ovl >= groups_here) continue;
        const int first = a.base0_rel + (q0 + gw) * DD - HALO;
        const uint32_t *hrow = b.hist_old + (long)cc * b.HH;
        if (REAL) {
          const uint16_t *row = reinterpret_cast<const uint16_t *>(a.in) + (long)cc * a.in_stride;
          uint32_t v[NDMA][8];
#pragma unroll
          for (int k = 0; k < NDMA; k++) {
            const int pp = min(l + 64 * k, NPIECE - 1);
#pragma unroll
            for (int j = 0; j < 8; j++) v[k][j] = row[max(min(first + 8 * pp + j, a.N - 1), 0)];
          }
#pragma unroll
          for (int k = 0; k < NDMA; k++) {
            const int pp = min(l + 64 * k, NPIECE - 1);
#pragma unroll
            for (int j = 0; j < 8; j++) {
              const int rel = first + 8 * pp + j;
              if (rel >= a.N) v[k][j] = 0u;
              if (first < 0) {
                const uint32_t xh = hrow[max(b.HH + rel, 0)];
                if (rel < 0) v[k][j] = (b.HH + rel >= 0) ? (xh & 0xffffu) : 0u;
              }
            }
            if (k < NDMA - 1 || l < LASTL) {
              const uint32_t x0 = v[k][0] | (v[k][1] << 16), x1 = v[k][2] | (v[k][3] << 16), x2 = v[k][4] | (v[k][5] << 16), x3 = v[k][6] | (v[k][7] << 16);
              uint2 l2, h2;
              l2.x = __builtin_amdgcn_perm(x1, x0, 0x06040200u) ^ 0x80808080u;
              l2.y = __builtin_amdgcn_perm(x3, x2, 0x06040200u) ^ 0x80808080u;
              h2.x = __builtin_amdgcn_perm(x1, x0, 0x07050301u);
              h2.y = __builtin_amdgcn_perm(x3, x2, 0x07050301u);
              *reinterpret_cast<uint2 *>(cb + dofs[k]) = l2;
              *reinterpret_cast<uint2 *>(cb + PLB + dofs[k]) = h2;
            }
          }
        } else if (CU8) {
          const uint16_t *row = reinterpret_cast<const uint16_t *>(a.in) + (long)cc * a.in_stride;
          uint32_t v[NDMA][8];
#pragma unroll
          for (int k = 0; k < NDMA; k++) {
            const int pp = min(l + 64 * k, NPIECE - 1);
#pragma unroll
            for (int j = 0; j < 8; j++) v[k][j] = row[max(min(first + 8 * pp + j, a.N - 1), 0)];
          }
#pragma unroll
          for (int k = 0; k < NDMA; k++) {
            const int pp = min(l + 64 * k, NPIECE - 1);
#pragma unroll
            for (int j = 0; j < 8; j++) {
              const int rel = first + 8 * pp + j;
              uint32_t hb = CS8 ? v[k][j] : ((v[k][j] + 0x81u) & 0xffu) | ((v[k][j] + 0x8100u) & 0xff00u);
              if (rel >= a.N) hb = 0u;
              if (first < 0) {
                const uint32_t xh = hrow[max(b.HH + rel, 0)];
                if (rel < 0) hb = (b.HH + rel >= 0) ? (CS8 ? ((xh & 0xffu) | ((xh >> 8) & 0xff00u)) : (((xh >> 8) & 0xffu) | ((xh >> 16) & 0xff00u))) : 0u;
              }
              v[k][j] = hb;
            }
            auto rotb = [](uint32_t d) __attribute__((always_inline)) { return CS8 ? d : ror8(d); };
            if (k < NDMA - 1 || l < LASTL)
              *reinterpret_cast<uint4 *>(cb + dofs[k]) = make_uint4(rotb(v[k][0] | (v[k][1] << 16)), rotb(v[k][2] | (v[k][3] << 16)),
                                                                    rotb(v[k][4] | (v[k][5] << 16)), rotb(v[k][6] | (v[k][7] << 16)));
          }
        } else {
          const uint32_t *row = reinterpret_cast<const uint32_t *>(a.in) + (long)cc * a.in_stride;
          uint32_t v[NDMA][4];
#pragma unroll
          for (int k = 0; k < NDMA; k++) {
            const int pp = min(l + 64 * k, NPIECE - 1);
#pragma unroll
            for (int j = 0; j < 4; j++) {
              const int rel = first + 4 * pp + j, hh = b.HH + rel;
              const uint32_t *src = rel >= 0 ? row + min(rel, a.N - 1) : hrow + max(hh, 0);
              v[k][j] = *src;
            }
          }
#pragma unroll
          for (int k = 0; k < NDMA; k++) {
            const int pp = min(l + 64 * k, NPIECE - 1);
#pragma unroll
            for (int j = 0; j < 4; j++) {
              const int rel = first + 4 * pp + j;
              if (rel >= a.N || b.HH + rel < 0) v[k][j] = 0u;
            }
            if (k < NDMA - 1 || l < LASTL) {
              uint2 l2, h2;
              l2.x = __builtin_amdgcn_perm(v[k][1], v[k][0], 0x06040200u) ^ 0x80808080u;
              l2.y = __builtin_amdgcn_perm(v[k][3], v[k][2], 0x06040200u) ^ 0x80808080u;
              h2.x = __builtin_amdgcn_perm(v[k][1], v[k][0], 0x07050301u);
              h2.y = __builtin_amdgcn_perm(v[k][3], v[k][2], 0x07050301u);
              *reinterpret_cast<uint2 *>(cb + dofs[k]) = l2;
              *reinterpret_cast<uint2 *>(cb + PLB + dofs[k]) = h2;
            }
          }
        }
        asm volatile("" ::: "memory");
        v16i acc_hh = {0}, acc_mid = {0}, acc_ll = {0};
        if (!CU8) {
#pragma unroll
          for (int r = 0; r < 16; r++) acc_ll[r] = (r & 1) ? a.cim : a.cre;
        }
        const char *pl = cb + coff, *ph = cb + (CU8 ? 0 : PLB) + coff;
#pragma unroll
        for (int s_ = 0; s_ < S; s_++) {
          const v4i uh = *reinterpret_cast<const v4i *>(ph + KSB * s_);
          const v4i Al = taps_s[s_ * 64 + l];
          acc_mid = __builtin_amdgcn_mfma_i32_32x32x32_i8(Al, uh, acc_mid, 0, 0, 0);
          if (!CU8) {
            const v4i ul = *reinterpret_cast<const v4i *>(pl + KSB * s_);
            acc_ll = __builtin_amdgcn_mfma_i32_32x32x32_i8(Al, ul, acc_ll, 0, 0, 0);
            if (s_ >= S0 && s_ < S0 + NH) {
              const v4i Ah = taps_s[(S + s_ - S0) * 64 + l];
              acc_hh = __builtin_amdgcn_mfma_i32_32x32x32_i8(Ah, uh, acc_hh, 0, 0, 0);
              acc_mid = __builtin_amdgcn_mfma_i32_32x32x32_i8(Ah, ul, acc_mid, 0, 0, 0);
            }
          } else if (s_ >= S0 && s_ < S0 + NH) {
            acc_hh = __builtin_amdgcn_mfma_i32_32x32x32_i8(taps_s[(S + s_ - S0) * 64 + l], uh, acc_hh, 0, 0, 0);
          }
        }
        if (DG) {
          const int s0 = a.base0_rel + (q0 + gw) * DD;
          int2 *pdst = nullptr;
          int ob0 = 0;
          if (PART) {
            const int t0 = s0 - a.base_real;
            ob0 = t0 < 0 ? a.Dreal - t0 : a.Dreal - (int)((unsigned)t0 % (unsigned)a.Dreal);
            pdst = a.part + (long)cc * a.part_stride + 3 * (4 * t + wv);
          }
          const int2 sum = stageE(std::true_type{}, acc_hh, acc_mid, acc_ll, (a.n0_lo + (uint32_t)s0) * a.inc, cb, s0 + MF_BLK * n + 8 * h, pdst, ob0);
          if (SD) sd_finish_cold(cb, cc, 4 * t + wv);
          else if (!PART) cold_finish_gen(sum, cc, 4 * t + wv);
        } else {
          const int tb = a.base0_rel + q0 * 8, rel0 = tb + 8 * gw + MF_BLK * n + 8 * h;
          const int2 sum = group_sum<ROT, CU8, true, WIDE ? 2 : 1, FSH, CS8>(b, acc_hh, acc_mid, acc_ll, rel0);
          group_finish(b, b.lut, cc, n, h, gw, q0, groups_here, sum);
        }
        asm volatile("" ::: "memory");
      }
      for (int k = tid & 255; k < b.HH; k += 256) {
        const long qq = (long)a.N + k;
        b.hist_new[(long)cc * b.HH + k] = qq < b.HH ? b.hist_old[(long)cc * b.HH + qq] : raw_x(b, cc, qq - b.HH);
      }
    }
  }
  if (DG && EPI == SDRHIP_EPI_FM) {
    if (b.fix_hi > b.fix_lo) {
      __syncthreads();
      for (int cc = bx; cc < a.C; cc += gx) {
        short *row = reinterpret_cast<short *>(a.out) + (long)cc * a.out_stride;
        short *pl = a.philast + (long)cc * a.philast_stride;
        for (int sl = b.fix_lo + (tid & 255); sl < b.fix_hi; sl += 256) {
          short *o = row + (long)sl * GS;
          *o = (short)(*o + pl[sl - 1]);
        }
      }
    }
  }
  if (PART) {
    if (a.fin_groups > 0) {
      __syncthreads();
      BigdArgs f;
      f.part = a.part; f.part_stride = a.part_stride;
      f.D = a.Dreal; f.base0_rel = a.base_real; f.N = a.N; f.n_groups = a.fin_groups; f.n_out = a.fin_out; f.epi = a.fin_epi; f.C = a.C;
      f.acc_old = b.acc_old; f.acc_new = b.acc_new; f.fm_old = b.fm_old; f.fm_new = b.fm_new;
      f.out = a.out; f.out_stride = a.out_stride;
      for (int cc = bx; cc < a.C; cc += gx)
        for (int q = tid & 255; q < f.n_groups; q += 256) bigd_finish_group(f, cc, q);
    }
  }
#ifdef K1_STAMPS
  if (l == 0 && a.stamps) {
    unsigned long long *o = a.stamps + (size_t)((((unsigned)bx * 4 + wv) & 32767u) * 16);
    for (int i = 0; i < 6; i++) o[i] = st_acc[i];
    o[8] = st_tiles; o[9] = __builtin_amdgcn_s_getreg((15 << 11) | 4);
    o[10] = st_r0; o[11] = __builtin_amdgcn_s_memrealtime(); o[12] = __builtin_amdgcn_s_getreg((3 << 11) | 20);
  }
#endif
}

constexpr int K1_MINWAVES = 4;
template <int S, int S0, int NH, bool ROT, int EPI, int IN, int NW, int L0 = 0, int NL = S>
__global__ __launch_bounds__(64 * NW, K1_MINWAVES) void iqbb_hot_kernel(const HotArgs a, const IqbbArgs b) {
  iqbb_hot_body<S, S0, NH, ROT, EPI, IN, NW, false, false, L0, NL>(a, b);
}
template <int S, int S0, int NH, bool ROT, int EPI, int IN, int NW = 4>
__global__ __launch_bounds__(64 * NW, K1_MINWAVES) void iqbb_hot_anyd_kernel(const HotArgs a, const IqbbArgs b) {
  iqbb_hot_body<S, S0, NH, ROT, EPI, IN, NW, true>(a, b);
}

template <int S, int S0, int NH, bool ROT, int EPI, int IN, int NW = 4>
__global__ __launch_bounds__(64 * NW, K1_MINWAVES) void iqbb_hot_sd_kernel(const HotArgs a, const IqbbArgs b) {
  iqbb_hot_body<S, S0, NH, ROT, EPI, IN, NW, true, true>(a, b);
}

template <class F>
inline void once_per_device(std::atomic<uint64_t> &mask, F &&set_attributes) {
  int d = 0;
  SDRHIP_CHECK_HIP(hipGetDevice(&d));
  const uint64_t bit = 1ull << (d & 63);
  if (mask.load(std::memory_order_acquire) & bit) return;
  set_attributes();
  mask.fetch_or(bit, std::memory_order_release);
}

template <int FORM, int S, int S0, int NH, bool ROT, int EPI, int IN, int NW, int L0, int NL>
constexpr auto hot_kernel() {
  if constexpr (FORM == HOT_D8) return &iqbb_hot_kernel<S, S0, NH, ROT, EPI, IN, NW, L0, NL>;
  else if constexpr (FORM == HOT_ANYD) return &iqbb_hot_anyd_kernel<S, S0, NH, ROT, EPI, IN, NW>;
  else return &iqbb_hot_sd_kernel<S, S0, NH, ROT, EPI, IN, NW>;
}
constexpr bool hot_has_epi(int form, int in, int epi) {
  if (epi == HOT_EPI_PARTIAL) return form == HOT_ANYD && in != HOT_REAL && in != HOT_CS8;
  return in != HOT_CS8 || epi == SDRHIP_EPI_FM || epi == SDRHIP_EPI_NONE;
}

template <int FORM, int S, int S0, int NH, int IN, int NW, int L0, int NL>
void hot_launch_form(bool rot, int epi, const HotLaunch &hl, const HotArgs &ha, const IqbbArgs &b) {
  auto run = [&](auto rot_c) {
    constexpr bool ROT = decltype(rot_c)::value;
    constexpr int NWL = FORM == HOT_SD ? hot_sd_range_waves(S, HotRange{S0, NH, NW}, IN, ROT) : NW;
    if constexpr (NWL > 0) {
      constexpr int extra = FORM == HOT_ANYD ? hot_anyd_extra(S, IN, ROT, NW) : FORM == HOT_SD ? hot_sd_extra(S, IN, ROT, NWL) : 0;
      constexpr size_t lds = FORM == HOT_D8 ? hot_lds_bytes(S, NH, IN, NW, hot_wide(S, NH, IN, NW))
                           : FORM == HOT_ANYD ? hot_lds_bytes(S, NH, IN, NW, hot_wide(S, NH, IN, NW, extra)) + extra
                                              : hot_lds_bytes(S, NH, IN, NWL, false) + extra;
      static_assert(FORM != HOT_ANYD || hot_lds_bytes(S, NH, IN, NW, false) + hot_anyd_extra(S, IN, false, NW) <= 163840, "any-D form: a workgroup's LDS");
      constexpr int anyd_cap = hot_lds_cap(NW, S) + hot_anyd_extra(S, IN, false, NW);
      constexpr int attr = FORM == HOT_ANYD ? (anyd_cap > 163840 ? 163840 : anyd_cap) : (int)lds;
      if constexpr (IN != HOT_CS8) if (FORM == HOT_ANYD ? NW > 4 : lds > 64 * 1024) {
        static std::atomic<uint64_t> attr_set{0};
        once_per_device(attr_set, [] {
          auto set = [](auto e) {
            constexpr int E = decltype(e)::value;
            if constexpr (E != HOT_EPI_PARTIAL || FORM == HOT_ANYD)
              SDRHIP_CHECK_HIP(hipFuncSetAttribute(reinterpret_cast<const void *>(hot_kernel<FORM, S, S0, NH, ROT, E, IN, NWL, L0, NL>()),
                                                   hipFuncAttributeMaxDynamicSharedMemorySize, attr));
          };
          set(std::integral_constant<int, SDRHIP_EPI_FM>{}); set(std::integral_constant<int, SDRHIP_EPI_AM>{});
          set(std::integral_constant<int, SDRHIP_EPI_USB>{}); set(std::integral_constant<int, SDRHIP_EPI_NONE>{});
          set(std::integral_constant<int, HOT_EPI_PARTIAL>{});
        });
      }
      auto go = [&](auto e) {
        constexpr int E = decltype(e)::value;
        if constexpr (hot_has_epi(FORM, IN, E))
          hipLaunchKernelGGL((hot_kernel<FORM, S, S0, NH, ROT, E, IN, NWL, L0, NL>()), dim3(hl.grid, 1), dim3(64 * NWL), lds, hl.stream, ha, b);
      };
      switch (epi) {
        case SDRHIP_EPI_FM: go(std::integral_constant<int, SDRHIP_EPI_FM>{}); break;
        case SDRHIP_EPI_AM: go(std::integral_constant<int, SDRHIP_EPI_AM>{}); break;
        case SDRHIP_EPI_USB: go(std::integral_constant<int, SDRHIP_EPI_USB>{}); break;
        case HOT_EPI_PARTIAL: go(std::integral_constant<int, HOT_EPI_PARTIAL>{}); break;
        default: go(std::integral_constant<int, SDRHIP_EPI_NONE>{}); break;
      }
    }
  };
  if (rot) run(std::true_type{}); else run(std::false_type{});
}

}

#ifdef SDRHIP_HOT_INSTANTIATE
namespace sdrhip {
template <int FORM, int S, int IN>
void HotClass<FORM, S, IN>::launch(int range, int lo, bool rot, int epi, const HotLaunch &hl, const HotArgs &ha, const IqbbArgs &b) {
  hot_pick<(int)std::size(hot_ranges_of<S>())>(range, [&](auto r) {
    constexpr HotRange R = hot_ranges_of<S>()[decltype(r)::value];
    if constexpr (FORM == HOT_D8 && (IN == HOT_CS16 || IN == HOT_CU8)) {
      hot_pick<(int)std::size(hot_lo_ranges_of<S>())>(lo, [&](auto l) {
        constexpr HotLoRange L = hot_lo_ranges_of<S>()[decltype(l)::value];
        constexpr bool inside = R.S0 >= L.L0 && R.S0 + R.NH <= L.L0 + L.NL;
        hot_launch_form<FORM, S, R.S0, R.NH, IN, R.NW, inside ? L.L0 : 0, inside ? L.NL : S>(rot, epi, hl, ha, b);
      });
    } else {
      hot_launch_form<FORM, S, R.S0, R.NH, IN, R.NW, 0, S>(rot, epi, hl, ha, b);
    }
  });
}
}
#endif
```

### libsdr_amd/csrc/iqbb_i16.hip

```cpp
#include "iqbb_common.hpp"
#include "iqbb_host.hpp"
#include "iqbb_hot.hpp"
#include "entry.hpp"

namespace {

template <int S, bool ROT, bool CU8>
__global__ __launch_bounds__(TPB, CU8 ? 5 : 4) void iqbb_i16_mfma_kernel(const IqbbArgs a) {
  extern __shared__ __attribute__((aligned(16))) uint32_t smem[];
  const int PLW = (2 * (TI + a.OP) + 64 + 31) / 32 * 8;
  constexpr int NPL = CU8 ? 1 : 2;
  int2 *lut_s = reinterpret_cast<int2 *>(smem);
  uint32_t *planes = smem + 256;
  v4i *taps_s = reinterpret_cast<v4i *>(smem + 256 + 2 * NPL * PLW);

  const int c = blockIdx.y, tid = threadIdx.x;
  const int w = tid >> 6, l = tid & 63, n = l & 31, h = l >> 5;
  for (int i = tid; i < S * 2 * 64; i += TPB) taps_s[i] = a.tapfrag[i];
  if (tid < 128) lut_s[tid] = a.lut[tid];

  constexpr int NQ = (TI + 16 * (S - 1) + 1 + 2 + 4 * TPB - 1) / (4 * TPB);
  struct __attribute__((packed, aligned(4))) Quad { uint32_t v[4]; };
  Quad px[NQ];
  auto fetch = [&](int tile_) {
// ... 472 lines not shown
      const v4i uh = *reinterpret_cast<const v4i *>(ph + 16 * s);
      const v4i Al = taps_s[(2 * s + 1) * 64 + l];
      acc_mid = __builtin_amdgcn_mfma_i32_32x32x32_i8(Al, uh, acc_mid, 0, 0, 0);
      if (CU8) {
        if (has_ah) acc_hh = __builtin_amdgcn_mfma_i32_32x32x32_i8(taps_s[(2 * s) * 64 + l], uh, acc_hh, 0, 0, 0);
      } else {
        const v4i ul = *reinterpret_cast<const v4i *>(pl + 16 * s);
        acc_ll = __builtin_amdgcn_mfma_i32_32x32x32_i8(Al, ul, acc_ll, 0, 0, 0);
        if (has_ah) {
          const v4i Ah = taps_s[(2 * s) * 64 + l];
          acc_hh = __builtin_amdgcn_mfma_i32_32x32x32_i8(Ah, uh, acc_hh, 0, 0, 0);
          acc_mid = __builtin_amdgcn_mfma_i32_32x32x32_i8(Ah, ul, acc_mid, 0, 0, 0);
        }
      }
    }
    const int pos0 = 512 * w + MF_BLK * n + 2 * h;
    uint32_t cnt0 = 0;
    if (ROT) cnt0 = (a.n0_lo + (uint32_t)(tb + pos0)) * a.inc;
    const uint32_t negx = a.negative ? (127u << 3) : 0u;
#pragma unroll
    for (int k = 0; k < 8; k++) {
      const int rr = 4 * (k >> 1) + 2 * (k & 1), dk = 4 * (k >> 1) + (k & 1);
      unsigned tre = ((unsigned)acc_hh[rr] << 8) + (unsigned)acc_mid[rr];
      unsigned tim = ((unsigned)acc_hh[rr + 1] << 8) + (unsigned)acc_mid[rr + 1];
      int2 v;
      if (CU8) {
        v = make_int2((int)(tre << 8) >> 14, (int)(tim << 8) >> 14);
      } else {
        asm("" : "+v"(tre)); asm("" : "+v"(tim));
        const unsigned sre = (tre << 8) + (unsigned)acc_ll[rr], sim = (tim << 8) + (unsigned)acc_ll[rr + 1];
        v = make_int2((int)sre >> 14, (int)sim >> 14);
      }
      if (ROT) {
        const uint32_t off = (((cnt0 + (uint32_t)dk * a.inc) >> 5) & (127u << 3)) ^ negx;
        const int2 L = *reinterpret_cast<const int2 *>(reinterpret_cast<const char *>(lut_s) + off);
        const int2 r = v;
        v.x = mad24a(L.x, r.x, -mul24a(L.y, r.y)) >> 16;
        v.y = mad24a(L.x, r.y, mul24a(L.y, r.x)) >> 16;
      }
      const int rel = tb + pos0 + dk;
      if (rel < 0 || rel >= a.N) v = make_int2(0, 0);
      vbuf[PADV(pos0 + dk)] = v;
    }
  }
  __syncthreads();

  {
    const int lpg = a.lpg, sub = tid & (lpg - 1), gpp = TPB / lpg;
    for (int g0 = 0; g0 < groups_here; g0 += gpp) {
      const int ql = g0 + tid / lpg, q = q0 + ql;
      int2 s = make_int2(0, 0);
      if (ql < groups_here) {
        for (int k = sub; k < a.D; k += lpg) {
          const int2 v = vbuf[PADV(ql * a.D + k)];
          s.x = (int)((unsigned)s.x + (unsigned)v.x);
          s.y = (int)((unsigned)s.y + (unsigned)v.y);
        }
      }
      for (int m = lpg >> 1; m >= 1; m >>= 1) {
        s.x = (int)((unsigned)s.x + (unsigned)__shfl_xor(s.x, m));
        s.y = (int)((unsigned)s.y + (unsigned)__shfl_xor(s.y, m));
      }
      if (sub == 0 && ql < groups_here && q >= 0)
        finalize_group(a, c, lut_s, ybuf, ql, q, s, a.D);
    }
  }
  __syncthreads();
  epilogue_and_roll(a, c, tile, tid, q0, groups_here, ybuf);
  }
}

__global__ void iqbb_fm_fixup_kernel(short *__restrict__ out, long out_stride, const short *__restrict__ philast, int philast_stride, int fix_lo, int fix_hi, int fix_gs, int C) {
  const int c = blockIdx.y, sl = fix_lo + blockIdx.x * blockDim.x + threadIdx.x;
  if (sl >= fix_hi) return;
  short *row = out + (long)c * out_stride;
  row[sl * fix_gs] = (short)(row[sl * fix_gs] + philast[(long)c * philast_stride + sl - 1]);
}

struct MultiFix { int nb; int q[63]; };
__global__ __launch_bounds__(256) void iqbb_fm_multi_fixup_kernel(const IqbbArgs a, const MultiFix f) {
  __shared__ int2 part[256];
  const int c = blockIdx.y, q = f.q[blockIdx.x], tid = threadIdx.x, D = a.D;
  int TL = 1;
  while (TL < 256 && 2 * TL * min(D, 256) <= 256) TL *= 2;
  const int SB = 256 / TL, il = tid / TL, ts = tid - il * TL;
  const int first = a.base0_rel + q * D;
  int2 vsum = make_int2(0, 0);
  for (int p0 = 0; p0 < D; p0 += SB) {
    const int i = p0 + il, rel = first + i;
    int er = 0, ei = 0;
    if (i < D)
      for (int k = ts; k < a.OP; k += TL) {
        const uint32_t x = load_x(a, c, rel - (a.OP - 1) + k);
        const uint2 kk = a.taps[k];
        if (a.in_real) { er = (int)((unsigned)er + (unsigned)mulw((int)kk.x, (int)x)); ei = (int)((unsigned)ei + (unsigned)mulw((int)kk.y, (int)x)); }
        else { er = dot2(x, kk.x, er); ei = dot2(x, kk.y, ei); }
      }
    part[tid] = make_int2(er, ei);
    __syncthreads();
    if (ts == 0 && i < D) {
      for (int t = 1; t < TL; t++) { er = (int)((unsigned)er + (unsigned)part[tid + t].x); ei = (int)((unsigned)ei + (unsigned)part[tid + t].y); }
      const int sh = a.in_real ? 16 : 14;
      const int2 v = rotate(a, a.lut, make_int2(er >> sh, ei >> sh), a.n0_lo + (uint32_t)rel);
      vsum.x = (int)((unsigned)vsum.x + (unsigned)v.x); vsum.y = (int)((unsigned)vsum.y + (unsigned)v.y);
    }
    __syncthreads();
  }
  part[tid] = vsum;
  __syncthreads();
  if (tid == 0) {
    int sx = 0;
    for (int t = 0; t < 256; t += TL) sx = (int)((unsigned)sx + (unsigned)part[t].x);
    short *row = reinterpret_cast<short *>(a.out) + (long)c * a.out_stride;
    const short l0 = row[q], l1 = row[q + 1];
    row[q + 1] = (short)(l0 + l1);
    row[q] = (short)box_div(sx, D);
  }
}

__global__ __launch_bounds__(256) void iqbb_bigd_finish_kernel(const BigdArgs a) {
  const int q = blockIdx.x * 256 + threadIdx.x;
  if (q < a.n_groups) bigd_finish_group(a, (int)blockIdx.y, q);
}

}

void sdrhip::hot_launch(int form, int S, int in, int range, int lo, bool rot, int epi, const HotLaunch &hl, const HotArgs &ha, const IqbbArgs &b) {
  bool done = false;
  hot_with_steps(S, [&](auto s) {
    hot_pick<3>(form, [&](auto f) {
      hot_pick<4>(in, [&](auto k) {
        constexpr int SC = decltype(s)::value, F = decltype(f)::value, IN = decltype(k)::value;
        if constexpr (hot_class(F, SC, IN))
          if (form == F && in == IN) { HotClass<F, SC, IN>::launch(range, lo, rot, epi, hl, ha, b); done = true; }
      });
    });
  });
  SDRHIP_REQUIRE(done, SDRHIP_E_UNSUPPORTED, "no hot kernel class for form %d, %d K steps, input kind %d", form, S, in);
}

namespace {
bool check_taps(const int32_t *taps, int order, bool real, bool need_planes) {
  bool planes = true;
  for (int i = 0; i < 2 * order; i++) {
    SDRHIP_REQUIRE(tap_in_range(taps[i], real), SDRHIP_E_UNSUPPORTED,
                   real ? "tap %d = %d exceeds 24 bits" : "tap %d = %d does not fit the packed int16 path", i / 2, taps[i]);
    const bool fits = tap_fits_planes(taps[i]);
    if (need_planes)
      SDRHIP_REQUIRE(fits, SDRHIP_E_UNSUPPORTED, "tap %d = %d does not fit the plan's int8 byte planes: create a new plan", i / 2, taps[i]);
    planes = planes && fits;
  }
  return planes;
}
}

struct sdrhip_iqbb_i16 {
  sdrhip_ctx *ctx = nullptr;
  int order = 0, OP = 0, HH = 0, D = 1, C = 1, epi = 0, negative = 0;
  uint32_t inc = 0;
  size_t max_in = 0;
  uint64_t n0 = 0;
  uint64_t phase0 = 0;
  uint64_t ring_n0 = 0;
  int ring_off0 = 0;
  int ring_offset() const { return (int)(((uint64_t)ring_off0 + (n0 - ring_n0)) % (uint64_t)order); }
  int par = 0, par_fm = 0;
  int CG = 0, OG = 0, ovl = 0;
  bool fast8 = false;
  bool use_hot = true;
  int env_tpw = 0, env_wgpcu = 0;
  int env_fm_resident = -1;
  int hot_range = -1;
  int lo_range = -1;
  bool env_trim = true;
  int in_cu8 = 0, real = 0, i8 = 0;
  int path = 0, S = 0, cre = 0, cim = 0;
  uint64_t ah_mask = 0;
  uint64_t al_mask = 0;
  DevBuf<v4i> tapfrag;
  DevBuf<v4i> tapfrag_hot;
  DevBuf<v4i> tapfrag_rot;
  size_t lds_bytes = 0;
  DevBuf<uint2> taps;
  DevBuf<int2> lut;
  DevBuf<uint32_t> hist[2];
  DevBuf<int2> acc[2];
  DevBuf<short> fm[2];
  Staging stage;
  size_t max_out = 0;
#ifdef K1_STAMPS
  DevBuf<unsigned long long> k1_stamps;
#endif
  DevBuf<short> philast;
  DevBuf<int2> part;
  int bigd_min = 257, bigd_skip_lo = 465;
  bool bigd_always = false;


  void load_taps(const int32_t *taps) {
    ah_mask = 0; al_mask = 0; hot_range = -1; lo_range = -1;
    std::vector<uint2> tp(OP);
    pack_valu_taps(taps, order, OP, real, tp.data());
    if (path == 4) {
      const int OPm = 32 * S - 15, padm = OPm - order;
      std::vector<int> kre(OPm, 0), kim(OPm, 0);
      for (int i = 0; i < order; i++) { kre[padm + i] = taps[2 * i]; kim[padm + i] = taps[2 * i + 1]; }
      cre = planes_const(kre.data(), OPm); cim = planes_const(kim.data(), OPm);
      std::vector<int8_t> frag((size_t)S * 2 * 64 * 16, 0);
      for (int st = 0; st < S; st++)
        for (int l = 0; l < 64; l++)
          for (int j = 0; j < 16; j++) {
            const int hh = l >> 5;
            int t, comp, ah, al;
            hot_row(l & 31, t, comp);
            const int idx = 32 * st + 16 * hh + j - t;
            split_planes((idx >= 0 && idx < OPm) ? (comp ? kim[idx] : kre[idx]) : 0, ah, al);
            frag[(((size_t)(2 * st) * 64 + l) * 16) + j] = (int8_t)ah;
            if (ah != 0) ah_mask |= (uint64_t)1 << st;
            if (al != 0) al_mask |= (uint64_t)1 << st;
            frag[(((size_t)(2 * st + 1) * 64 + l) * 16) + j] = (int8_t)al;
          }
      if (!tapfrag.p) tapfrag.alloc((size_t)S * 2 * 64);
      tapfrag.upload(reinterpret_cast<const v4i *>(frag.data()), (size_t)S * 2 * 64, ctx->stream);
    } else if (path >= 1) {
      const int OPm = 16 * (S - 1) + 1, padm = OPm - order;
      std::vector<int> are(2 * OPm, 0), aim(2 * OPm, 0);
      for (int i = 0; i < order; i++) {
        const int kr = taps[2 * i], ki = taps[2 * i + 1];
        are[2 * (padm + i)] = kr; are[2 * (padm + i) + 1] = -ki;
        aim[2 * (padm + i)] = ki; aim[2 * (padm + i) + 1] = kr;
      }
      cre = planes_const(are.data(), 2 * OPm); cim = planes_const(aim.data(), 2 * OPm);
      std::vector<int8_t> frag((size_t)S * 2 * 64 * 16, 0);
      auto build = [&](bool permuted) {
        for (int st = 0; st < S; st++)
          for (int l = 0; l < 64; l++)
            for (int j = 0; j < 16; j++) {
              const int m = l & 31, hh = l >> 5;
              int t = m >> 1, comp = m & 1, ah, al;
              if (permuted) hot_row(m, t, comp);
              const int idx = 32 * st + 16 * hh + j - 2 * t;
              split_planes((idx >= 0 && idx < 2 * OPm) ? (comp ? aim[idx] : are[idx]) : 0, ah, al);
              frag[(((size_t)(2 * st) * 64 + l) * 16) + j] = (int8_t)ah;
              if (ah != 0) ah_mask |= (uint64_t)1 << st;
              if (al != 0) al_mask |= (uint64_t)1 << st;
              frag[(((size_t)(2 * st + 1) * 64 + l) * 16) + j] = (int8_t)al;
            }
      };
      auto upload_rot = [&]() {
        std::vector<int8_t> r(frag.size());
        for (size_t i = 0; i < frag.size(); i++) r[i] = frag[(i & ~(size_t)3) | ((i + 1) & 3)];
        if (!tapfrag_rot.p) tapfrag_rot.alloc((size_t)S * 2 * 64);
        tapfrag_rot.upload(reinterpret_cast<const v4i *>(r.data()), (size_t)S * 2 * 64, ctx->stream);
      };
      if (path == 3) {
        build(true);
        if (!tapfrag_hot.p) tapfrag_hot.alloc((size_t)S * 2 * 64);
        tapfrag_hot.upload(reinterpret_cast<const v4i *>(frag.data()), (size_t)S * 2 * 64, ctx->stream);
        upload_rot();
      }
      build(path == 1);
      if (path == 1) upload_rot();
      if (!tapfrag.p) tapfrag.alloc((size_t)S * 2 * 64);
      tapfrag.upload(reinterpret_cast<const v4i *>(frag.data()), (size_t)S * 2 * 64, ctx->stream);
    }
    if (path != 0) pick_hot_ranges();
    if (!this->taps.p) this->taps.alloc(OP);
    this->taps.upload(tp.data(), OP, ctx->stream);
  }
  void pick_hot_ranges() {
    auto covers = [](uint64_t mask, int first, int n) { return (mask & ~((((uint64_t)1 << n) - 1u) << first)) == 0; };
    int nr = 0, nl = 0;
    const HotRange *rg = hot_ranges(S, &nr);
    for (int r = 0; r < nr && hot_range < 0; r++)
      if (covers(ah_mask, rg[r].S0, rg[r].NH)) hot_range = r;
    if (path != 1 || hot_range < 0) return;
    const HotLoRange *lr = hot_lo_ranges(S, &nl);
    for (int r = 0; r < nl && lo_range < 0; r++) {
      const bool inside = rg[hot_range].S0 >= lr[r].L0 && rg[hot_range].S0 + rg[hot_range].NH <= lr[r].L0 + lr[r].NL;
      if ((covers(al_mask, lr[r].L0, lr[r].NL) && inside && env_trim) || r == nl - 1) lo_range = r;
    }
  }
  size_t valu_lds() const { return (TI + (size_t)OP + 8 + 256 + 2 * (((size_t)CG + 3) & ~(size_t)3)) * 4 + (fast8 ? 0 : (size_t)TI * 8); }
  int hot_nw() const { int n = 0; const HotRange *rg = hot_ranges(S, &n); return rg[std::min(hot_range, n - 1)].NW; }

  Geometry geometry(size_t N) const { return call_geometry(n0, N, D, real != 0); }
  size_t out_elem_bytes() const { return epi == SDRHIP_EPI_NONE ? (i8 ? 2 : 4) : 2; }
  size_t in_elem_bytes() const { return (in_cu8 || real || i8) ? 2 : 4; }

  HotArgs hot_args(const uint32_t *in_dev, size_t N, size_t in_stride, void *out_dev, size_t out_stride, const v4i *tapfrag_) const {
    HotArgs ha{};
    ha.in = in_dev; ha.in_stride = (long)in_stride; ha.out = out_dev; ha.out_stride = (long)out_stride;
    ha.tapfrag = tapfrag_; ha.lut = lut.p; ha.inc = inc; ha.n0_lo = (uint32_t)(n0 - phase0); ha.negative = negative;
    ha.cre = cre; ha.cim = cim; ha.N = (int)N; ha.C = C; ha.stamps = nullptr;
    return ha;
  }
  unsigned hot_grid(HotArgs &ha, int tiles, int NW, bool resident) const {
    const int nvwg = wgpcu() * ctx->prop.multiProcessorCount;
    int htpw = 4; while (htpw > 1 && (size_t)ceil_div((size_t)tiles, (size_t)htpw) * C < 4 * (size_t)nvwg) htpw >>= 1;
    if (resident) htpw = tiles;
    else if (env_tpw) htpw = env_tpw;
    ha.tpw = htpw;
    ha.G = (int)ceil_div((size_t)tiles, (size_t)htpw); ha.U = ha.G * C;
    const int vper = NW / 4;
    const int grid = (int)ceil_div((size_t)std::max(1, std::min(nvwg, std::max(ha.U, C))), (size_t)vper);
    const int gx = grid * vper;
    ha.dq = gx / ha.G; ha.dr = gx % ha.G;
    return (unsigned)grid;
  }

  bool launch_hot_call(IqbbArgs &a, const Geometry &g, const uint32_t *in_dev, size_t N, size_t in_stride, void *out_dev,
                       size_t out_stride, int tiles) {
    const int kind = hot_kind(), halo = hot_halo(S, kind), win = hot_win(S, kind);
    auto host_hot = [&](int t, int w) { return slice_is_hot(halo, win, g.base0_rel, OG, ovl, (int)N, g.n_out, t, w); };
    long t = tiles - 1;
    while (t >= 2 && !(host_hot((int)t - 1, 0) && host_hot((int)t - 1, 1) && host_hot((int)t - 1, 2) && host_hot((int)t - 1, 3))) t--;
    if (t < 2) return false;
    HotArgs ha = hot_args(in_dev, N, in_stride, out_dev, out_stride, in_cu8 ? tapfrag_rot.p : tapfrag.p);
    ha.base0_rel = g.base0_rel; ha.OG = OG; ha.ovl = ovl; ha.t_lo = 0; ha.t_hi = tiles; ha.n_out = g.n_out;
    ha.D = 8; ha.GS = 64; ha.lpg_sh = 0; ha.inv_d = 0.125f; ha.philast = nullptr; ha.philast_stride = 0; ha.part = nullptr; ha.fin_groups = 0;
    ha.mb_p = 0; ha.mb_q1 = 0; ha.mb_qlast = 0; ha.mb_magic = 0;
    if (!mb_q.empty() && epi == SDRHIP_EPI_FM && !i8) {
      const int per = 64 - ovl;
      long P = mb_q.size() >= 2 ? (long)mb_q[1] - mb_q[0] : (long)1 << 30;
      bool uniform = P >= 128;
      for (size_t j = 2; j < mb_q.size(); j++) uniform = uniform && (long)mb_q[j] - mb_q[j - 1] == P;
      if (uniform) {
        ha.mb_q1 = mb_q[0]; ha.mb_p = (int)P; ha.mb_qlast = mb_q.back(); ha.mb_magic = (unsigned)((((unsigned long long)1) << 32) / (unsigned long long)P);
        std::vector<int> left;
        for (int q : mb_q) {
          const int tl = q / OG, w = (q % OG) / per, lane = (q % OG) % per + ovl;
          if (!(lane <= 62 && host_hot(tl, w))) left.push_back(q);
        }
        mb_q.swap(left);
      }
    }
#ifdef K1_STAMPS
    if (!k1_stamps.p) { k1_stamps.alloc(32768 * 16); k1_stamps.zero(ctx->stream); }
    ha.stamps = k1_stamps.p;
#endif
    const HotLaunch hl{hot_grid(ha, tiles, hot_nw(), false), ctx->stream};
    a.bt_hi = (int)t; a.tpw = 1;
    hot_launch(HOT_D8, S, kind, hot_range, lo_range, inc != 0, epi, hl, ha, a);
    return true;
  }

  bool bigd_plan() const {
    return path == 3 && use_hot && hot_range >= 0 && S <= 33 && !i8 && !real && D >= bigd_min && D >= 257 && !(D >= bigd_skip_lo && D <= 512) && part.p != nullptr;
  }
  bool launch_bigd_call(const IqbbArgs &a0, const Geometry &g, const uint32_t *in_dev, size_t N, size_t in_stride, void *out_dev, size_t out_stride) {
    const int kind = hot_kind(), halo = hot_halo(S, kind), win = hot_win(S, kind);
    const int nsl = (int)ceil_div(N, (size_t)512), tiles_h = (int)ceil_div((size_t)nsl, (size_t)4);
    auto slice_hot = [&](int sl) { return slice_is_hot(halo, win, 0, 4, 0, (int)N, nsl, sl >> 2, sl & 3, 512, 1); };
    int s_lo = 0, s_hi = 4 * tiles_h;
    while (s_lo < s_hi && !slice_hot(s_lo)) s_lo++;
    while (s_hi > s_lo && !slice_hot(s_hi - 1)) s_hi--;
    if (s_hi - s_lo < 16 && !bigd_always) return false;
    SDRHIP_REQUIRE(part.n >= (size_t)C * 12 * tiles_h, SDRHIP_E_SIZE, "part holds %zu entries, the call needs %zu", part.n, (size_t)C * 12 * tiles_h);
    IqbbArgs a = a0;
    a.base0_rel = 0; a.n_groups = nsl; a.n_out = nsl; a.extra0 = 0; a.D = 512; a.fix_lo = a.fix_hi = 0;
    HotArgs ha = hot_args(in_dev, N, in_stride, out_dev, out_stride, in_cu8 ? tapfrag_rot.p : tapfrag_hot.p);
    ha.base0_rel = 0; ha.OG = 4; ha.ovl = 0; ha.t_lo = s_lo >> 2; ha.t_hi = (s_hi + 3) >> 2; ha.n_out = nsl;
    ha.D = 512; ha.GS = 1; ha.tiles_h = tiles_h; ha.lpg_sh = 6; ha.inv_d = 0.f;
    ha.philast = nullptr; ha.philast_stride = 0;
    ha.part = part.p; ha.part_stride = 12 * tiles_h; ha.Dreal = D; ha.base_real = g.base0_rel;
    const bool resident = channel_units();
    ha.fin_groups = resident ? g.n_groups : 0; ha.fin_out = g.n_out; ha.fin_epi = epi;
    const HotLaunch hl{hot_grid(ha, tiles_h, hot_nw(), resident), ctx->stream};
    hot_launch(HOT_ANYD, S, kind, hot_range, -1, inc != 0, HOT_EPI_PARTIAL, hl, ha, a);
    if (resident) return true;
    BigdArgs f;
    f.part = part.p; f.part_stride = 12 * tiles_h;
    f.D = D; f.base0_rel = g.base0_rel; f.N = (int)N; f.n_groups = g.n_groups; f.n_out = g.n_out; f.epi = epi; f.C = C;
    f.acc_old = a0.acc_old; f.acc_new = a0.acc_new; f.fm_old = a0.fm_old; f.fm_new = a0.fm_new;
    f.out = out_dev; f.out_stride = (long)out_stride;
    hipLaunchKernelGGL(iqbb_bigd_finish_kernel, dim3((unsigned)ceil_div((size_t)g.n_groups, (size_t)256), (unsigned)C), dim3(256), 0, ctx->stream, f);
    return true;
  }
  int wgpcu() const { return env_wgpcu ? env_wgpcu : S >= 33 ? 2 : 4; }
  bool long_filter() const { return (path == 1 || path == 3) && (S >= 33 || i8); }
  bool channel_units() const {
    if (env_fm_resident >= 0) return env_fm_resident != 0;
    const size_t nvwg = (size_t)wgpcu() * (size_t)ctx->prop.multiProcessorCount, rounds = ceil_div((size_t)C, nvwg);
    return (size_t)C * 100 >= rounds * nvwg * 97;
  }
  bool real_anyd() const { return path == 4 && D != R; }
  int hot_kind() const { return real ? HOT_REAL : i8 ? HOT_CS8 : in_cu8 ? HOT_CU8 : HOT_CS16; }
  bool anyd_plan() const {
    if (!(((path == 3 && !real) || real_anyd()) && use_hot && hot_range >= 0 && S <= 33)) return false;
    if (D >= 9 && D <= 512) return true;
    if (i8) return false;
    return D >= 1 && D <= 7 && hot_sd_waves(S, hot_kind(), hot_range, inc != 0) != 0;
  }
  bool launch_anyd_call(IqbbArgs &a, const Geometry &g, const uint32_t *in_dev, size_t N, size_t in_stride, void *out_dev,
                        size_t out_stride) {
    const int kind = hot_kind(), halo = hot_halo(S, kind), win = hot_win(S, kind);
    const int GS = 512 / D, OGh = 4 * GS;
    const int tiles_h = (int)ceil_div((size_t)g.n_groups, (size_t)OGh);
    auto slice_hot = [&](int sl) { return slice_is_hot(halo, win, g.base0_rel, OGh, 0, (int)N, g.n_out, sl >> 2, sl & 3, D, GS); };
    int s_lo = 0, s_hi = 4 * tiles_h;
    while (s_lo < s_hi && !slice_hot(s_lo)) s_lo++;
    while (s_hi > s_lo && !slice_hot(s_hi - 1)) s_hi--;
    if (s_hi - s_lo < 16) return false;
    const int t_lo = s_lo >> 2, t_hi = (s_hi + 3) >> 2;
    HotArgs ha = hot_args(in_dev, N, in_stride, out_dev, out_stride, real ? tapfrag.p : in_cu8 ? tapfrag_rot.p : tapfrag_hot.p);
    ha.base0_rel = g.base0_rel; ha.OG = OGh; ha.ovl = 0; ha.t_lo = t_lo; ha.t_hi = t_hi; ha.n_out = g.n_out;
    ha.D = D; ha.GS = GS; ha.tiles_h = tiles_h;
    { int lpg = 1; while (2 * lpg <= 64 && 2 * lpg * GS <= 64) lpg *= 2; int sh = 0; while ((1 << sh) < lpg) sh++; ha.lpg_sh = sh; }
    ha.inv_d = (float)((1.0 / D) * (1.0 - 1.0 / 1048576.0));
    ha.philast = nullptr; ha.philast_stride = 4 * tiles_h; ha.part = nullptr; ha.fin_groups = 0;
    if (epi == SDRHIP_EPI_FM) {
      SDRHIP_REQUIRE(philast.n >= (size_t)C * 4 * tiles_h, SDRHIP_E_SIZE, "philast holds %zu entries, the call needs %zu", philast.n, (size_t)C * 4 * tiles_h);
      ha.philast = philast.p;
    }
#ifdef K1_STAMPS
    if (!k1_stamps.p) { k1_stamps.alloc(32768 * 16); k1_stamps.zero(ctx->stream); }
    ha.stamps = k1_stamps.p;
#endif
    const int fix_lo = GS == 1 ? 2 : 1, fix_hi = epi == SDRHIP_EPI_FM ? (int)ceil_div((size_t)g.n_out, (size_t)GS) : 0;
    const bool resident = fix_hi > fix_lo && channel_units();
    a.fix_lo = resident ? fix_lo : 0; a.fix_hi = resident ? fix_hi : 0;
    const int NW = D < 8 ? hot_sd_waves(S, kind, hot_range, inc != 0) : hot_nw();
    const HotLaunch hl{hot_grid(ha, tiles_h, NW, resident), ctx->stream};
    hot_launch(D < 8 ? HOT_SD : HOT_ANYD, S, kind, hot_range, -1, inc != 0, epi, hl, ha, a);
    if (!resident && fix_hi > fix_lo)
      hipLaunchKernelGGL(iqbb_fm_fixup_kernel, dim3((unsigned)ceil_div((size_t)(fix_hi - fix_lo), (size_t)256), (unsigned)C), dim3(256), 0, ctx->stream,
                         reinterpret_cast<short *>(out_dev), (long)out_stride, philast.p, 4 * tiles_h, fix_lo, fix_hi, GS, C);
    return true;
  }

  void launch(const uint32_t *in_dev, size_t N, size_t in_stride, void *out_dev, size_t out_stride, size_t *n_out) {
    ctx->use();
    if (N == 0) { if (n_out) *n_out = 0; return; }
    const Geometry g = geometry(N);
    SDRHIP_REQUIRE(out_stride >= (size_t)g.n_out, SDRHIP_E_SIZE, "out_stride %zu < outputs %d", out_stride, g.n_out);
    IqbbArgs a;
    a.in = in_dev; a.in_stride = (long)in_stride; a.in_cu8 = in_cu8; a.in_real = real; a.i8 = i8;
    a.hist_old = hist[par].p; a.hist_new = hist[par ^ 1].p; a.HH = HH;
    a.acc_old = acc[par].p; a.acc_new = acc[par ^ 1].p;
    const bool fm_flip = (epi == SDRHIP_EPI_FM && g.n_out >= 2);
    a.fm_old = fm[par_fm].p; a.fm_new = fm[par_fm ^ 1].p;
    a.taps = taps.p; a.lut = lut.p; a.inc = inc; a.negative = negative;
    a.OP = OP; a.D = D; a.N = (int)N; a.n0_lo = (uint32_t)(n0 - phase0);
    a.base0_rel = g.base0_rel; a.n_groups = g.n_groups; a.n_out = g.n_out; a.extra0 = g.extra0;
    a.CG = CG; a.OG = OG; a.ovl = ovl; a.CGr = (CG + 3) & ~3;
    a.out = out_dev; a.out_stride = (long)out_stride; a.epilogue = epi;
    a.tapfrag = tapfrag.p; a.cre = cre; a.cim = cim; a.ah_mask = (unsigned)ah_mask;
    const int tiles = (int)ceil_div((size_t)g.n_groups, (size_t)OG);
    int tpw = 1;
    const bool mf8 = (path == 1 && !long_filter()) || (path == 4 && D == R);
    if (mf8) { tpw = 8; while (tpw > 1 && (size_t)ceil_div((size_t)tiles, (size_t)tpw) * C < 2048) tpw >>= 1; }
    if (env_tpw && mf8) tpw = env_tpw;
    a.tiles = tiles; a.tpw = tpw; a.bt_hi = 0; a.fix_lo = a.fix_hi = 0;
    a.lpg = 1; while (a.lpg < 64 && a.lpg * 8 < D) a.lpg <<= 1;
    bool done = false;
    const CallForms cf = call_forms();
    for (int i = 0; i < cf.n_long && !done; i++) {
      if (cf.long_form[i] == LONG_HOT8) done = tiles >= 3 && launch_hot_call(a, g, in_dev, N, in_stride, out_dev, out_stride, tiles);
      else if (cf.long_form[i] == LONG_BIGD) done = launch_bigd_call(a, g, in_dev, N, in_stride, out_dev, out_stride);
      else done = launch_anyd_call(a, g, in_dev, N, in_stride, out_dev, out_stride);
    }
    if (!done) launch_short(cf.short_form, a, tiles);
    SDRHIP_CHECK_HIP(hipGetLastError());
    par ^= 1;
    if (fm_flip) par_fm ^= 1;
    n0 += N;
    if (n_out) *n_out = (size_t)g.n_out;
    last_args = a;
  }
  enum { LONG_HOT8, LONG_BIGD, LONG_ANYD };
  enum { SHORT_REAL_MFMA, SHORT_VALU, SHORT_MFMAG, SHORT_MFMA_CU8, SHORT_MFMA_DMA };
// ... 3 lines not shown
    if ((path == 1 || (path == 4 && D == R)) && use_hot && hot_range >= 0) f.long_form[f.n_long++] = LONG_HOT8;
    if (bigd_plan()) f.long_form[f.n_long++] = LONG_BIGD;
    if (anyd_plan()) f.long_form[f.n_long++] = LONG_ANYD;
    f.short_form = path == 4 && D == R ? SHORT_REAL_MFMA
                 : path == 0 || path == 4 || long_filter() ? SHORT_VALU
                 : path == 3 ? SHORT_MFMAG
                 : in_cu8 ? SHORT_MFMA_CU8 : SHORT_MFMA_DMA;
    return f;
  }
  std::string call_kernel_names() const {
    const CallForms f = call_forms();
    static const char *const general[] = {"bb_real_mfma_kernel", "iqbb_i16_kernel", "iqbb_i16_mfmag_kernel", "iqbb_i16_mfma_kernel", "iqbb_i16_mfma_dma_kernel"};
    if (f.n_long == 0) return general[f.short_form];
    if (f.long_form[0] == LONG_HOT8) return "iqbb_hot_kernel";
    if (f.long_form[0] == LONG_BIGD) return channel_units() ? "iqbb_hot_anyd_kernel" : "iqbb_hot_anyd_kernel,iqbb_bigd_finish_kernel";
    const bool fixup = epi == SDRHIP_EPI_FM && !channel_units();
    return std::string(D < 8 ? "iqbb_hot_sd_kernel" : "iqbb_hot_anyd_kernel") + (fixup ? ",iqbb_fm_fixup_kernel" : "");
  }
  void launch_short(int form, IqbbArgs &a, int tiles) {
    const dim3 grid((unsigned)ceil_div((size_t)tiles, (size_t)a.tpw), C), block(TPB);
    switch (form) {
      case SHORT_REAL_MFMA:
#define SDRHIP_MFR(S_) do { if (inc != 0) hipLaunchKernelGGL((bb_real_mfma_kernel<S_, true>), grid, block, lds_bytes, ctx->stream, a); \
                             else hipLaunchKernelGGL((bb_real_mfma_kernel<S_, false>), grid, block, lds_bytes, ctx->stream, a); } while (0)
        switch (S) {
          case 3: SDRHIP_MFR(3); break;
          case 5: SDRHIP_MFR(5); break;
          default: SDRHIP_MFR(9); break;
        }
#undef SDRHIP_MFR
        break;
      case SHORT_MFMAG: {
        int tpw3 = 8; while (tpw3 > 1 && (size_t)ceil_div((size_t)tiles, (size_t)tpw3) * C < 2048) tpw3 >>= 1;
        if (env_tpw) tpw3 = env_tpw;
        a.tpw = tpw3;
        const dim3 grid3((unsigned)ceil_div((size_t)tiles, (size_t)tpw3), C);
#define SDRHIP_MFG(S_) do { if (in_cu8 && inc != 0) hipLaunchKernelGGL((iqbb_i16_mfmag_kernel<S_, true, true>), grid3, block, lds_bytes, ctx->stream, a); \
                             else if (in_cu8) hipLaunchKernelGGL((iqbb_i16_mfmag_kernel<S_, false, true>), grid3, block, lds_bytes, ctx->stream, a); \
                             else if (inc != 0) hipLaunchKernelGGL((iqbb_i16_mfmag_kernel<S_, true, false>), grid3, block, lds_bytes, ctx->stream, a); \
                             else hipLaunchKernelGGL((iqbb_i16_mfmag_kernel<S_, false, false>), grid3, block, lds_bytes, ctx->stream, a); } while (0)
        switch (S) {
          case 2: SDRHIP_MFG(2); break;
          case 3: SDRHIP_MFG(3); break;
          case 5: SDRHIP_MFG(5); break;
          case 9: SDRHIP_MFG(9); break;
          default: SDRHIP_MFG(17); break;
        }
#undef SDRHIP_MFG
        break;
      }
      case SHORT_MFMA_DMA: {
        const size_t PLWd = (2 * (size_t)(TI + OP) + 64 + 31) / 32 * 8, quads = (TI + OP + 4) / 4;
        const size_t ldsd = (256 + 2 * PLWd + 4 * ((quads + 63) / 64 * 64)) * 4 + (size_t)S * 2 * 64 * 16;
#define SDRHIP_MFD(S_) do { if (inc != 0) hipLaunchKernelGGL((iqbb_i16_mfma_dma_kernel<S_, true>), grid, block, ldsd, ctx->stream, a); \
                             else hipLaunchKernelGGL((iqbb_i16_mfma_dma_kernel<S_, false>), grid, block, ldsd, ctx->stream, a); } while (0)
        switch (S) {
          case 2: SDRHIP_MFD(2); break;
          case 3: SDRHIP_MFD(3); break;
          case 5: SDRHIP_MFD(5); break;
          case 9: SDRHIP_MFD(9); break;
          default: SDRHIP_MFD(17); break;
        }
#undef SDRHIP_MFD
        break;
      }
      case SHORT_MFMA_CU8: {
        const size_t lds1 = lds_bytes - 2 * (((2 * (size_t)(TI + OP) + 64 + 31) / 32 * 8) * 4);
#define SDRHIP_MF(S_) do { if (inc != 0) hipLaunchKernelGGL((iqbb_i16_mfma_kernel<S_, true, true>), grid, block, lds1, ctx->stream, a); \
                            else hipLaunchKernelGGL((iqbb_i16_mfma_kernel<S_, false, true>), grid, block, lds1, ctx->stream, a); } while (0)
        switch (S) {
          case 2: SDRHIP_MF(2); break;
          case 3: SDRHIP_MF(3); break;
          case 5: SDRHIP_MF(5); break;
          case 9: SDRHIP_MF(9); break;
          default: SDRHIP_MF(17); break;
        }
#undef SDRHIP_MF
        break;
      }
      default:
        if (fast8 && real) hipLaunchKernelGGL((iqbb_i16_kernel<true, true>), grid, block, lds_bytes, ctx->stream, a);
        else if (fast8) hipLaunchKernelGGL((iqbb_i16_kernel<true, false>), grid, block, lds_bytes, ctx->stream, a);
        else if (real) hipLaunchKernelGGL((iqbb_i16_kernel<false, true>), grid, block, lds_bytes, ctx->stream, a);
        else hipLaunchKernelGGL((iqbb_i16_kernel<false, false>), grid, block, lds_bytes, ctx->stream, a);
        break;
    }
  }

  IqbbArgs last_args{};
  int last_multi_left = -1;
  std::vector<int> mb_q;

  void launch_multi(const uint32_t *in_dev, size_t B, size_t nb, size_t in_stride, void *out_dev, size_t out_stride, size_t *counts, size_t *total) {
    std::vector<size_t> qs(B + 1, 0);
    for (size_t j = 1; j <= B; j++) qs[j] = (size_t)geometry(j * nb).n_out;
    for (size_t j = 0; j < B && counts; j++) counts[j] = qs[j + 1] - qs[j];
    if (total) *total = qs[B];
    bool one_launch = B >= 2 && !i8 && B <= 64;
    if (epi == SDRHIP_EPI_FM) for (size_t j = 0; j < B; j++) if (qs[j + 1] - qs[j] < 2) one_launch = false;
    if (!one_launch) {
      const size_t ib = in_elem_bytes(), ob = out_elem_bytes();
      for (size_t j = 0; j < B; j++)
        launch(reinterpret_cast<const uint32_t *>(reinterpret_cast<const char *>(in_dev) + j * nb * ib), nb, in_stride,
               reinterpret_cast<char *>(out_dev) + qs[j] * ob, out_stride, nullptr);
      return;
    }
    mb_q.clear();
    if (epi == SDRHIP_EPI_FM) for (size_t j = 1; j < B; j++) mb_q.push_back((int)qs[j]);
    try { launch(in_dev, B * nb, in_stride, out_dev, out_stride, nullptr); } catch (...) { mb_q.clear(); throw; }
    std::vector<int> left;
    left.swap(mb_q);
    last_multi_left = (int)left.size();
    if (left.empty()) return;
    MultiFix f{};
    f.nb = (int)left.size();
    for (size_t j = 0; j < left.size(); j++) f.q[j] = left[j];
    hipLaunchKernelGGL(iqbb_fm_multi_fixup_kernel, dim3((unsigned)left.size(), (unsigned)C), dim3(256), 0, ctx->stream, last_args, f);
    SDRHIP_CHECK_HIP(hipGetLastError());
  }
};

namespace {

int create_baseband(sdrhip_ctx *ctx, const int32_t *taps, int order, const int32_t *lut, uint32_t lut_inc,
                    int negative, int decim, int channels, size_t max_in, int epilogue, bool real,
                    sdrhip_iqbb_i16 **out, bool i8 = false) {
  return guarded([&] {
    make_handle(ctx, out, taps && lut, [&](sdrhip_iqbb_i16 *h) {
      SDRHIP_REQUIRE(order >= 1 && order <= MAX_ORDER, SDRHIP_E_UNSUPPORTED, "order %d outside [1,%d]", order, MAX_ORDER);
      SDRHIP_REQUIRE(decim >= 1, SDRHIP_E_INVALID, "decim %d < 1", decim);
      require_channels(channels, 65535);
      require_max_in(max_in);
      SDRHIP_REQUIRE(epilogue >= SDRHIP_EPI_NONE && epilogue <= SDRHIP_EPI_USB, SDRHIP_E_INVALID, "bad epilogue %d", epilogue);
      const int ovl = epilogue == SDRHIP_EPI_FM ? 1 : 0;
      const bool beyond = TI / decim - ovl < 1;
      const int CG = beyond ? 1 + ovl : TI / decim;
      SDRHIP_REQUIRE(!beyond || (!real && !i8 && order <= 257 && decim <= 32768), SDRHIP_E_UNSUPPORTED,
                     "decim %d too large (max %d; complex<int16> / complex<uint8> plans of up to 257 taps: 32768)", decim, TI / (1 + ovl));
      const bool planes = check_taps(taps, order, real, false);
      for (int i = 0; i < 256; i++)
        SDRHIP_REQUIRE(lut[i] > -(1 << 23) && lut[i] < (1 << 23), SDRHIP_E_UNSUPPORTED, "LUT entry %d = %d exceeds 24 bits", i / 2, lut[i]);
      h->order = order; h->D = decim; h->C = channels; h->epi = epilogue;
      h->negative = negative ? 1 : 0; h->inc = lut_inc; h->max_in = max_in; h->real = real ? 1 : 0; h->i8 = i8 ? 1 : 0;
      SDRHIP_REQUIRE(!i8 || epilogue == SDRHIP_EPI_NONE || epilogue == SDRHIP_EPI_FM, SDRHIP_E_UNSUPPORTED,
                     "the int8 chain is IQBaseBand<int8_t> (-> FMDemod<int8_t,int16_t>): epilogue NONE or FM");
      { const char *d = getenv("SDRHIP_IQBB_HOT"); if (d && d[0] == '0') h->use_hot = false; }
      const int mfma_max_order = h->use_hot ? 513 : 257;
      const bool i8_hot = i8 && h->use_hot && order <= 129;
      bool mfma_ok = !real && (!i8 || i8_hot) && (decim == R) && (order <= mfma_max_order) && planes;
      { const char *e = getenv("SDRHIP_IQBB_TPW"); if (e) h->env_tpw = std::max(1, atoi(e)); }
      { const char *e = getenv("SDRHIP_IQBB_WGPCU"); if (e) h->env_wgpcu = std::max(1, atoi(e)); }
      { const char *e = getenv("SDRHIP_IQBB_FM_RESIDENT"); if (e) h->env_fm_resident = atoi(e) != 0; }
      { const char *e = getenv("SDRHIP_IQBB_TRIM"); if (e && e[0] == '0') h->env_trim = false; }
      const char *force = getenv("SDRHIP_IQBB_PATH");
      if (force && !strcmp(force, "valu")) mfma_ok = false;
      h->path = mfma_ok ? 1 : 0;
      bool mfmag_ok = !real && (!i8 || (i8_hot && decim >= 9 && decim <= 512)) && decim != R && order <= mfma_max_order && (order <= 257 || decim >= 9) && planes;
      if (force && !strcmp(force, "valu")) mfmag_ok = false;
      if (h->path == 0 && mfmag_ok) h->path = 3;
      SDRHIP_REQUIRE(!beyond || (h->path == 3 && h->use_hot), SDRHIP_E_UNSUPPORTED,
                     "decim %d too large (max %d) for this plan: beyond it only the hot kernel's large-decimation form exists (tap high bytes within int8, SDRHIP_IQBB_HOT / SDRHIP_IQBB_PATH unset)",
                     decim, TI / (1 + ovl));
      h->bigd_always = beyond;
      if (real && !i8 && (decim == R || (decim <= 512 && h->use_hot)) && order <= 273 && !(force && !strcmp(force, "valu")) && planes)
        h->path = 4;
      if (h->path == 4) {
        h->S = order <= 81 ? 3 : order <= 145 ? 5 : 9;
        h->OP = decim == R ? 32 * h->S - 15 : (int)ceil_div((size_t)order, (size_t)TAPC) * TAPC;
      } else if (h->path == 1 || h->path == 3) {
        h->S = order <= 17 ? 2 : order <= 33 ? 3 : order <= 65 ? 5 : order <= 129 ? 9 : order <= 257 ? 17 : 33;
        h->OP = (h->S >= 33 || i8) ? (int)ceil_div((size_t)order, (size_t)TAPC) * TAPC : 16 * (h->S - 1) + 1;
      } else {
        h->OP = (int)ceil_div((size_t)order, (size_t)TAPC) * TAPC;
      }
      h->HH = h->OP;
      if (h->path == 4) h->HH = std::max(h->OP, 32 * h->S - 15);
      if (h->long_filter()) h->HH = std::max(h->OP, 16 * (h->S - 1) + 1);
      h->CG = CG; h->ovl = ovl; h->OG = CG - ovl;
      if (h->path == 1 || (h->path == 4 && decim == R)) { h->OG = 4 * (64 - ovl); h->CG = h->OG + ovl; }
      h->fast8 = (decim == R);
      if ((h->path == 4 && decim != R) || h->long_filter()) {
        h->lds_bytes = h->valu_lds();
      } else if (h->path == 4) {
        h->lds_bytes = 1024 + (size_t)h->S * 2 * 64 * 16 + 4 * 2 * (size_t)(512 + 32 * h->S);
      } else if (h->path == 3) {
        const size_t PLW = (2 * (size_t)(TI + h->OP) + 64 + 31) / 32 * 8;
        h->lds_bytes = (2 * PLW + 256) * 4 + (size_t)h->S * 2 * 64 * 16 + (size_t)(TI + TI / 16 + 2) * 8 + 2 * (size_t)((CG + 3) & ~3) * 4;
        if (h->lds_bytes > 80 * 1024) {
          h->path = 0; h->OP = (int)ceil_div((size_t)order, (size_t)TAPC) * TAPC; h->HH = h->OP;
          h->lds_bytes = h->valu_lds();
        }
      } else if (h->path == 1) {
        const size_t PLW = (2 * (size_t)(TI + h->OP) + 64 + 31) / 32 * 8;
        h->lds_bytes = (4 * PLW + 256) * 4 + (size_t)h->S * 2 * 64 * 16;
      } else {
        h->lds_bytes = h->valu_lds();
      }
      SDRHIP_REQUIRE(h->lds_bytes <= (h->path == 3 ? 80 : 64) * 1024, SDRHIP_E_UNSUPPORTED, "LDS budget exceeded (%zu B)", h->lds_bytes);
      if (h->path == 3 && h->lds_bytes > 64 * 1024) {
        allow_lds_max(&iqbb_i16_mfmag_kernel<17, true, true>, h->lds_bytes); allow_lds_max(&iqbb_i16_mfmag_kernel<17, false, true>, h->lds_bytes);
        allow_lds_max(&iqbb_i16_mfmag_kernel<17, true, false>, h->lds_bytes); allow_lds_max(&iqbb_i16_mfmag_kernel<17, false, false>, h->lds_bytes);
      }
      h->load_taps(taps);
      h->lut.alloc(128); h->lut.upload(reinterpret_cast<const int2 *>(lut), 128, ctx->stream);
      for (int p = 0; p < 2; p++) {
        h->hist[p].alloc((size_t)channels * h->HH); h->hist[p].zero(ctx->stream);
        h->acc[p].alloc(channels); h->acc[p].zero(ctx->stream);
        h->fm[p].alloc(channels); h->fm[p].zero(ctx->stream);
      }
      h->max_out = max_in / decim + 2;
      if (epilogue == SDRHIP_EPI_FM && (h->path == 3 || h->real_anyd()) && decim >= 1 && decim <= 512) {
        const size_t GS = 512 / (size_t)decim, tiles_h = ceil_div(max_in / (size_t)decim + 2, 4 * GS);
        h->philast.alloc((size_t)channels * 4 * tiles_h + 1024);
      }
      { const char *e = getenv("SDRHIP_IQBB_BIGD_MIN"); if (e) { h->bigd_min = std::max(257, atoi(e)); h->bigd_skip_lo = 513; } }
      { const char *e = getenv("SDRHIP_IQBB_BIGD_ALWAYS"); if (e && atoi(e) != 0 && decim >= 257) { h->bigd_always = true; h->bigd_skip_lo = 513; } }
      if (beyond) { h->bigd_min = 257; h->bigd_skip_lo = 513; }
      if (h->path == 3 && decim >= 257 && decim >= h->bigd_min)
        h->part.alloc((size_t)channels * 12 * ceil_div(ceil_div(max_in, (size_t)512), (size_t)4) + 64);
    });
  });
}

}

static std::vector<uint32_t> reconfigured_ring(const sdrhip_iqbb_i16 *src, int HH_dst) {
  const int HH = src->HH;
  hipStream_t st = src->ctx->stream;
  std::vector<uint32_t> old((size_t)src->C * HH), neu((size_t)src->C * HH_dst, 0u);
  SDRHIP_CHECK_HIP(hipMemcpyAsync(old.data(), src->hist[src->par].p, old.size() * 4, hipMemcpyDeviceToHost, st));
  SDRHIP_CHECK_HIP(hipStreamSynchronize(st));
  for (int c = 0; c < src->C; c++)
    reconfigured_ring_row(old.data() + (size_t)c * HH, HH, src->order, src->ring_offset(), neu.data() + (size_t)c * HH_dst, HH_dst);
  return neu;
}

extern "C" {

int sdrhip_iqbb_i16_create(sdrhip_ctx *ctx, const int32_t *taps, int order, const int32_t *lut, uint32_t lut_inc,
                           int negative, int decim, int channels, size_t max_in, int epilogue,
                           sdrhip_iqbb_i16 **out) {
  return create_baseband(ctx, taps, order, lut, lut_inc, negative, decim, channels, max_in, epilogue, false, out);
}

int sdrhip_bb_i16_create(sdrhip_ctx *ctx, const int32_t *taps, int order, const int32_t *lut, uint32_t lut_inc,
                         int negative, int decim, int channels, size_t max_in, int epilogue,
                         sdrhip_iqbb_i16 **out) {
  return create_baseband(ctx, taps, order, lut, lut_inc, negative, decim, channels, max_in, epilogue, true, out);
}

int sdrhip_iqbb_i8_create(sdrhip_ctx *ctx, const int32_t *taps, int order, const int32_t *lut, uint32_t lut_inc,
                          int negative, int decim, int channels, size_t max_in, int epilogue,
                          sdrhip_iqbb_i16 **out) {
  return create_baseband(ctx, taps, order, lut, lut_inc, negative, decim, channels, max_in, epilogue, false, out, true);
}

int sdrhip_iqbb_i16_path(sdrhip_iqbb_i16 *h, int *path) {
  return guarded([&] {
    SDRHIP_REQUIRE(h && path, SDRHIP_E_INVALID, "NULL argument");
    *path = h->path;
  });
}

int sdrhip_iqbb_i16_plan_info(sdrhip_iqbb_i16 *h, int *info, int n) {
  return guarded([&] {
    SDRHIP_REQUIRE(h && info && n >= 8, SDRHIP_E_INVALID, "info must hold 8 ints");
    int lcnt = 0;
    const HotLoRange *lr = hot_lo_ranges(h->S, &lcnt);
    int cnt = 0;
    const HotRange *rg = hot_ranges(h->S, &cnt);
    const bool hot = h->hot_range >= 0 && h->hot_range < cnt;
    info[0] = h->path; info[1] = h->S; info[2] = hot ? rg[h->hot_range].S0 : 0; info[3] = hot ? rg[h->hot_range].NH : 0;
    info[4] = hot ? rg[h->hot_range].NW : 4; info[5] = h->hot_kind(); info[6] = h->OP; info[7] = h->HH;
    if (n >= 9) info[8] = h->last_multi_left;
    if (n >= 11) {
      const bool lo = hot && h->lo_range >= 0 && h->lo_range < lcnt;
      info[9] = lo ? lr[h->lo_range].L0 : 0; info[10] = lo ? lr[h->lo_range].NL : (hot ? h->S : 0);
    }
  });
}

int sdrhip_iqbb_i16_kernel_names(sdrhip_iqbb_i16 *h, char *buf, size_t len) {
  return guarded([&] {
    SDRHIP_REQUIRE(h && buf && len, SDRHIP_E_INVALID, "NULL argument");
    snprintf(buf, len, "%s", h->call_kernel_names().c_str());
  });
}

int sdrhip_iqbb_i16_out_count(sdrhip_iqbb_i16 *h, size_t n_in, size_t *n_out) {
  return guarded([&] {
    SDRHIP_REQUIRE(h && n_out, SDRHIP_E_INVALID, "NULL argument");
    *n_out = n_in ? (size_t)h->geometry(n_in).n_out : 0;
  });
}

int sdrhip_iqbb_i16_process_dev(sdrhip_iqbb_i16 *h, const int16_t *in_dev, size_t n_in, size_t in_stride,
                                void *out_dev, size_t out_stride, size_t *n_out) {
  return guarded([&] {
    Range roctx_range("sdrhip_iqbb_i16_process_dev");
    if (!call_begin(h, "n_in", n_in, in_dev, out_dev)) { if (n_out) *n_out = 0; return; }
    const size_t no = (size_t)h->geometry(n_in).n_out;
    const Strides s = call_strides("n_in", n_in, in_stride, no, out_stride, STRIDE_IN);
    require_disjoint(in_dev, s.in, n_in, h->in_elem_bytes(), out_dev, s.out, no, h->out_elem_bytes(), (size_t)h->C);
    h->launch(reinterpret_cast<const uint32_t *>(in_dev), n_in, s.in, out_dev, s.out, n_out);
  });
}

int sdrhip_iqbb_i16_process_dev_multi(sdrhip_iqbb_i16 *h, const int16_t *in_dev, size_t n_buffers, size_t n_per_buffer, size_t in_stride,
                                      void *out_dev, size_t out_stride, size_t *n_out_per_buffer, size_t *n_out_total) {
  return guarded([&] {
    Range roctx_range("sdrhip_iqbb_i16_process_dev_multi");
    SDRHIP_REQUIRE(h, SDRHIP_E_INVALID, "handle is NULL");
    const size_t n_in = n_buffers * n_per_buffer;
    SDRHIP_REQUIRE(n_buffers == 0 || n_in / n_buffers == n_per_buffer, SDRHIP_E_SIZE, "n_buffers * n_per_buffer overflows");
    SDRHIP_REQUIRE(n_in <= h->max_in, SDRHIP_E_SIZE, "n_buffers * n_per_buffer = %zu > max_in %zu", n_in, h->max_in);
    if (n_in == 0) {
      for (size_t j = 0; j < n_buffers && n_out_per_buffer; j++) n_out_per_buffer[j] = 0;
      if (n_out_total) *n_out_total = 0;
      return;
    }
    SDRHIP_REQUIRE(in_dev && out_dev, SDRHIP_E_INVALID, "NULL buffer");
    const size_t no = (size_t)h->geometry(n_in).n_out;
    const Strides s = call_strides("n_buffers * n_per_buffer", n_in, in_stride, no, out_stride, STRIDE_IN | STRIDE_OUT);
    require_disjoint(in_dev, s.in, n_in, h->in_elem_bytes(), out_dev, s.out, no, h->out_elem_bytes(), (size_t)h->C);
    h->ctx->use();
    h->launch_multi(reinterpret_cast<const uint32_t *>(in_dev), n_buffers, n_per_buffer, s.in, out_dev, s.out, n_out_per_buffer, n_out_total);
  });
}

int sdrhip_iqbb_i16_process(sdrhip_iqbb_i16 *h, const int16_t *in_host, size_t n_in, size_t in_stride,
                            void *out_host, size_t out_stride, size_t *n_out) {
  return guarded([&] {
    Range roctx_range("sdrhip_iqbb_i16_process");
    if (!call_begin(h, "n_in", n_in, in_host, out_host)) { if (n_out) *n_out = 0; return; }
    const Strides s = call_strides("n_in", n_in, in_stride, (size_t)h->geometry(n_in).n_out, out_stride, STRIDE_OUT);
    const size_t ib = h->in_elem_bytes(), eb = h->out_elem_bytes(), C = (size_t)h->C;
    size_t produced = 0;
    run_staged(h->ctx, h->stage, C * h->max_in * 4, C * h->max_out * 4, {in_host, s.in * ib, n_in * ib, C},
               {out_host, s.out * eb, h->max_out * 4, C}, [&](void *in, void *out) {
                 h->launch(static_cast<const uint32_t *>(in), n_in, n_in, out, h->max_out * 4 / eb, &produced);
                 return produced * eb;
               });
    if (n_out) *n_out = produced;
  });
}

int sdrhip_iqbb_i16_set_input_format(sdrhip_iqbb_i16 *h, int format) {
  return guarded([&] {
    SDRHIP_REQUIRE(h, SDRHIP_E_INVALID, "handle is NULL");
    SDRHIP_REQUIRE(format == SDRHIP_IN_CS16 || format == SDRHIP_IN_CU8, SDRHIP_E_INVALID, "bad input format %d", format);
    SDRHIP_REQUIRE(!h->real && !h->i8, SDRHIP_E_INVALID, "the real-input and the int8 baseband take their own sample type only");
    SDRHIP_REQUIRE(h->n0 == 0, SDRHIP_E_INVALID, "the input format can only change before the first buffer / after a reset");
    h->in_cu8 = format == SDRHIP_IN_CU8;
  });
}

int sdrhip_iqbb_i16_reset(sdrhip_iqbb_i16 *h, int keep_history) {
  return guarded([&] {
    use_handle(h);
    hipStream_t st = h->ctx->stream;
    const bool keep_fm = (keep_history & 2) != 0;
    keep_history &= 1;
    for (int p = 0; p < 2; p++) { h->acc[p].zero(st); if (!keep_fm) h->fm[p].zero(st); }
    if (!keep_history) {
      for (int p = 0; p < 2; p++) h->hist[p].zero(st);
    } else if (h->ring_offset() != 0) {
      const std::vector<uint32_t> neu = reconfigured_ring(h, h->HH);
      SDRHIP_CHECK_HIP(hipMemcpyAsync(h->hist[h->par].p, neu.data(), neu.size() * 4, hipMemcpyHostToDevice, st));
      SDRHIP_CHECK_HIP(hipStreamSynchronize(st));
    }
    h->n0 = 0; h->phase0 = 0; h->ring_n0 = 0; h->ring_off0 = 0;
  });
}

int sdrhip_iqbb_i16_adopt_state(sdrhip_iqbb_i16 *h, sdrhip_iqbb_i16 *from, int what) {
  return guarded([&] {
    SDRHIP_REQUIRE(h && from && h != from, SDRHIP_E_INVALID, "two distinct handles are needed");
    SDRHIP_REQUIRE(h->n0 == 0, SDRHIP_E_INVALID, "the adopting plan must be fresh (no buffer processed since create / reset)");
    SDRHIP_REQUIRE(h->C == from->C && h->real == from->real && h->i8 == from->i8 && h->in_cu8 == from->in_cu8, SDRHIP_E_INVALID,
                   "plans differ in channels (%d / %d) or sample kind", h->C, from->C);
    SDRHIP_REQUIRE(h->ctx->device == from->ctx->device, SDRHIP_E_INVALID, "plans live on different devices");
    const bool ring = (what & SDRHIP_KEEP_RING) != 0, fmk = (what & SDRHIP_KEEP_FM) != 0, stream = (what & SDRHIP_KEEP_COUNTERS) != 0;
    SDRHIP_REQUIRE(!ring || h->order == from->order, SDRHIP_E_INVALID, "SDRHIP_KEEP_RING needs equal orders (%d / %d)", h->order, from->order);
    SDRHIP_REQUIRE(!stream || h->D == from->D, SDRHIP_E_INVALID, "SDRHIP_KEEP_COUNTERS needs equal decimations (%d / %d)", h->D, from->D);
    SDRHIP_REQUIRE(!fmk || (h->epi == SDRHIP_EPI_FM && from->epi == SDRHIP_EPI_FM), SDRHIP_E_INVALID,
                   "SDRHIP_KEEP_FM needs the FM epilogue on both plans (%d / %d)", h->epi, from->epi);
    h->ctx->use();
    hipStream_t st = h->ctx->stream;
    SDRHIP_CHECK_HIP(hipStreamSynchronize(from->ctx->stream));
    const size_t C = (size_t)h->C;
    if (ring && stream) {
      const int order = h->order;
      SDRHIP_CHECK_HIP(hipMemcpy2DAsync(h->hist[h->par].p + (h->HH - order), (size_t)h->HH * 4, from->hist[from->par].p + (from->HH - order),
                                        (size_t)from->HH * 4, (size_t)order * 4, C, hipMemcpyDeviceToDevice, st));
    } else if (ring) {
      const std::vector<uint32_t> neu = reconfigured_ring(from, h->HH);
      SDRHIP_CHECK_HIP(hipMemcpyAsync(h->hist[h->par].p, neu.data(), neu.size() * 4, hipMemcpyHostToDevice, st));
      SDRHIP_CHECK_HIP(hipStreamSynchronize(st));
    }
    if (fmk) SDRHIP_CHECK_HIP(hipMemcpyAsync(h->fm[h->par_fm].p, from->fm[from->par_fm].p, C * sizeof(short), hipMemcpyDeviceToDevice, st));
    if (stream) {
      SDRHIP_CHECK_HIP(hipMemcpyAsync(h->acc[h->par].p, from->acc[from->par].p, C * sizeof(int2), hipMemcpyDeviceToDevice, st));
      h->n0 = from->n0; h->phase0 = from->phase0;
      h->ring_n0 = h->n0; h->ring_off0 = from->ring_offset() < h->order ? from->ring_offset() : 0;
    }
    SDRHIP_CHECK_HIP(hipStreamSynchronize(st));
  });
}

int sdrhip_iqbb_i16_set_taps(sdrhip_iqbb_i16 *h, const int32_t *taps) {
  return guarded([&] {
    SDRHIP_REQUIRE(h && taps, SDRHIP_E_INVALID, "NULL argument");
    check_taps(taps, h->order, h->real, h->path >= 1);
    h->ctx->use();
    h->load_taps(taps);
  });
}

int sdrhip_iqbb_i16_set_shift(sdrhip_iqbb_i16 *h, uint32_t lut_inc, int negative) {
  return guarded([&] {
    SDRHIP_REQUIRE(h, SDRHIP_E_INVALID, "handle is NULL");
    h->inc = lut_inc; h->negative = negative ? 1 : 0;
    h->phase0 = h->n0;
  });
}

int sdrhip_iqbb_i16_destroy(sdrhip_iqbb_i16 *h) {
  return guarded([&] { destroy_handle(h); });
}

}
// ... 9 lines not shown
```

### libsdr_amd/nodes.py

```python
import ctypes as C

import numpy as np

from . import abi
from .abi import (EPI_NONE, EPI_FM, EPI_AM, EPI_USB, FIR_CS16_EXACT, FIR_CF32, T_CS16, T_CF32, T_CF64,
                  FFTCONV_OLA, FFTCONV_OLS, check)


def _p(a, typed=False):
    return a.ctypes.data_as(C.POINTER(np.ctypeslib.as_ctypes_type(a.dtype)) if typed else C.c_void_p)


def _out(ctype, fn, *args):
    v = ctype()
    check(fn(*args, C.byref(v)))
    return v.value


def _text(fn, *args, size=0):
    if not size:
        return _out(C.c_char_p, fn, *args).decode()
    b = C.create_string_buffer(size)
    check(fn(*args, b, size))
    return b.value.decode()
# ... 109 lines not shown
            self._release()
            self._h = C.c_void_p()

    def __del__(self):
        try:
            self.close()
        except Exception:
            pass


class Context(_Handle):
    _borrowed = False

    def __init__(self, device=0, stream=None):
        self._h = C.c_void_p()
        check(abi.lib().sdrhip_ctx_create(device, C.c_void_p(stream) if stream else None, C.byref(self._h)))
        self.device = device

    @classmethod
    def borrowed(cls, handle, device):
        self = cls.__new__(cls)
        self._h, self.device, self._borrowed = C.c_void_p(handle.value if isinstance(handle, C.c_void_p) else handle), device, True
        return self

    @property
    def handle(self):
        return self._h

    def synchronize(self):
        check(abi.lib().sdrhip_ctx_synchronize(self._h))

    def device_name(self):
        return _text(abi.lib().sdrhip_ctx_device_name, self._h, size=256)

    def malloc(self, nbytes):
        return _out(C.c_void_p, abi.lib().sdrhip_malloc, self._h, nbytes)

    def free(self, p):
        check(abi.lib().sdrhip_free(self._h, C.c_void_p(p)))

    def h2d(self, dptr, arr):
        arr = np.ascontiguousarray(arr)
        check(abi.lib().sdrhip_memcpy_h2d(self._h, C.c_void_p(dptr), _p(arr), arr.nbytes))

    def d2h(self, arr, dptr):
        assert arr.flags["C_CONTIGUOUS"]
        check(abi.lib().sdrhip_memcpy_d2h(self._h, _p(arr), C.c_void_p(dptr), arr.nbytes))

    def memset(self, dptr, value, nbytes):
        check(abi.lib().sdrhip_memset(self._h, C.c_void_p(dptr), value, nbytes))

    def _release(self):
        for hook in close_hooks:
            hook(self)
        if not self._borrowed:
            abi.lib().sdrhip_ctx_destroy(self._h)


class Timer(_Handle):

    def __init__(self, ctx):
        self._h = C.c_void_p()
        check(abi.lib().sdrhip_timer_create(ctx.handle, C.byref(self._h)))

    def start(self):
        check(abi.lib().sdrhip_timer_start(self._h))

    def stop(self):
        check(abi.lib().sdrhip_timer_stop(self._h))

    def elapsed_ms(self):
        return _out(C.c_float, abi.lib().sdrhip_timer_elapsed_ms, self._h)

    def _release(self):
        abi.lib().sdrhip_timer_destroy(self._h)


device_router = None
close_hooks = []


class _Node(_Handle):
    _prefix, _calls = None, ""
    _in, _assert_channels = (np.int16, 2), False

    def __init__(self):
        self._h = C.c_void_p()
        self._bind(self._prefix, self._calls + " destroy")

    def _bind(self, prefix, calls):
        L = abi.lib()
        for name in calls.split():
            setattr(self, "_c_" + name, getattr(L, "%s_%s" % (prefix, name)))

    def _release(self):
        self._c_destroy(self._h)

    def _rows(self, x):
        return _rows(x, *self._in, self.channels if self._assert_channels else None)


class _Counted(_Node):
    epilogue, _out_dtype = EPI_NONE, np.int16

    def out_count(self, n_in):
        return _out(C.c_size_t, self._c_out_count, self._h, n_in)

    def _zeros(self, no):
        return np.zeros((self.channels, no, 2) if self.epilogue == EPI_NONE else (self.channels, no), self._out_dtype)

    def _host_in(self, x, n_in):
        return _p(x), n_in, n_in

    def process(self, x):
        x = self._rows(x)
        n_in = x.shape[1]
        no = self.out_count(n_in)
        out = self._zeros(no)
        if device_router is not None and n_in and no:
            return device_router(self.ctx, x, out, lambda i, si, o, so: self._dev_checked(i, n_in, si, o, so, no))
        assert _out(C.c_size_t, self._c_process, self._h, *self._host_in(x, n_in), _p(out), no) == no
        return out

    def _dev_checked(self, i, n_in, si, o, so, no):
        assert self.process_dev(i, n_in, si, o, so) == no

    def process_dev(self, in_ptr, n_in, in_stride, out_ptr, out_stride):
        got = C.c_size_t(0)
        check(self._c_process_dev(self._h, C.c_void_p(in_ptr), n_in, in_stride, C.c_void_p(out_ptr), out_stride, C.byref(got)))
        return got.value

    def reset(self):
        check(self._c_reset(self._h))


class _EqualLength(_Node):

    def _run(self, x, out, rows=None, routed=True):
        n = x.shape[1]
        if routed and device_router is not None and n:
            return device_router(self.ctx, x, out if rows is None else rows, lambda i, si, o, so: self.process_dev(i, n, si, o, so))
        check(self._c_process(self._h, _p(x), n, n, _p(out), n))
        return out

    def process_dev(self, in_ptr, n, in_stride, out_ptr, out_stride):
        check(self._c_process_dev(self._h, C.c_void_p(in_ptr), n, in_stride, C.c_void_p(out_ptr), out_stride))

    def reset(self):
        check(self._c_reset(self._h))


class IQBaseBandI16(_Counted):
    _prefix = "sdrhip_iqbb_i16"
    _calls = ("path kernel_names plan_info out_count process process_dev process_dev_multi reset adopt_state set_taps set_shift "
              "set_input_format")
    _create = "sdrhip_iqbb_i16_create"
    _assert_channels = True

    def __init__(self, ctx, taps, lut, lut_inc, negative, decim, channels=1, max_in=65536, epilogue=EPI_NONE):
        super().__init__()
        taps = np.ascontiguousarray(taps, np.int32).reshape(-1, 2)
        lut = np.ascontiguousarray(lut, np.int32).reshape(128, 2)
        self.ctx, self.channels, self.decim, self.epilogue, self.max_in = ctx, channels, decim, epilogue, max_in
        check(getattr(abi.lib(), self._create)(ctx.handle, _p(taps, True), taps.shape[0], _p(lut, True), lut_inc, int(bool(negative)),
                                               decim, channels, max_in, epilogue, C.byref(self._h)))

    @property
    def path(self):
        return _out(C.c_int, self._c_path, self._h)

    @property
    def kernel_names(self):
        return _text(self._c_kernel_names, self._h, size=256).split(",")

    @property
    def plan_info(self):
        v = (C.c_int * 11)()
        check(self._c_plan_info(self._h, v, 11))
        return dict(zip(("path", "S", "S0", "NH", "NW", "kind", "OP", "HH", "multi_left", "L0", "NL"), list(v)))

    def process_dev_multi(self, in_ptr, n_buffers, n_per_buffer, in_stride, out_ptr, out_stride):
        counts = (C.c_size_t * max(1, n_buffers))()
        total = _out(C.c_size_t, self._c_process_dev_multi, self._h, C.c_void_p(in_ptr), n_buffers, n_per_buffer, in_stride,
                     C.c_void_p(out_ptr), out_stride, counts)
        assert sum(counts[:n_buffers]) == total
        return list(counts[:n_buffers])

    def process_multi(self, x, n_buffers):
        x = self._rows(x)
        assert x.shape[1] % n_buffers == 0
        n_in, nb = x.shape[1], x.shape[1] // n_buffers
        no = self.out_count(n_in)
        out = self._zeros(no)
        counts = []
        run = lambda i, si, o, so: counts.extend(self.process_dev_multi(i, n_buffers, nb, si, o, so))
        if device_router is not None:
            device_router(self.ctx, x, out, run)
        else:
            _roundtrip(self.ctx, x, out, lambda i, o: run(i, n_in, o, no), staged_out=True)
        return out, counts

    def reset(self, keep_history=False, keep_fm=False):
        check(self._c_reset(self._h, int(bool(keep_history)) | (2 if keep_fm else 0)))

    def adopt_state(self, other, what):
        check(self._c_adopt_state(self._h, other._h, int(what)))

    def set_taps(self, taps):
        taps = np.ascontiguousarray(taps, np.int32).reshape(-1, 2)
        check(self._c_set_taps(self._h, _p(taps, True)))

    def set_shift(self, lut_inc, negative):
        check(self._c_set_shift(self._h, lut_inc, int(bool(negative))))

    def set_input_format(self, fmt):
        check(self._c_set_input_format(self._h, fmt))
        self._in = (np.uint8, 2) if fmt == abi.IN_CU8 else type(self)._in


class TunerBankI16(_Counted):
    _prefix = "sdrhip_tuner_i16"
    _calls = "kernel_names plan_info out_count process process_dev set_taps set_shift set_input_format reset"
    _CREATE = {(False, False): "sdrhip_tuner_i16_create", (False, True): "sdrhip_tunermodes_i16_create",
               (True, False): "sdrhip_tunerbb_i16_create", (True, True): "sdrhip_tunermodes_bb_i16_create"}

    def __init__(self, ctx, taps, lut, lut_inc, negative, decim, max_in=65536, epilogue=EPI_NONE, modes=None, real=False):
        super().__init__()
        self._bind("sdrhip_tunermodes_i16", "set_mode get_modes")
        self.real = bool(real)
        taps = np.ascontiguousarray(taps, np.int32)
        assert taps.ndim == 3 and taps.shape[2] == 2, taps.shape
        lut = np.ascontiguousarray(lut, np.int32).reshape(128, 2)
        inc = np.ascontiguousarray(lut_inc, np.uint32).reshape(-1)
        neg = np.ascontiguousarray(np.asarray(negative, bool), np.int32).reshape(-1)
        channels, order = taps.shape[0], taps.shape[1]
        assert inc.size == channels and neg.size == channels
        self.ctx, self.channels, self.order, self.decim, self.epilogue, self.max_in = ctx, channels, order, decim, epilogue, max_in
        if modes is not None:
            m = np.ascontiguousarray(modes, np.intc).reshape(-1)
            assert m.size == channels
            self.epilogue = EPI_FM
            tail = (_p(m, True), decim, channels, max_in)
        else:
            tail = (decim, channels, max_in, epilogue)
        create = getattr(abi.lib(), self._CREATE[self.real, modes is not None])
        check(create(ctx.handle, _p(taps, True), order, _p(lut, True), _p(inc, True), _p(neg, True), *tail, C.byref(self._h)))

    @property
    def kernel_names(self):
        return _text(self._c_kernel_names, self._h, size=256).split(",")

    def plan_info(self, n_in):
        v = (C.c_int * 10)()
        check(self._c_plan_info(self._h, n_in, v, 10))
        return dict(zip(("hot", "S", "CG", "OG", "tiles", "ctiles", "ctw", "grid_y", "PLB", "lds"), list(v)))

    def _rows(self, x):
        x = np.ascontiguousarray(x, self._in[0])
        if self.real:
            assert x.ndim == 1, x.shape
        else:
            assert x.ndim == 2 and x.shape[1] == 2, x.shape
        return x[None]

    def _host_in(self, x, n_in):
        return _p(x[0]), n_in

    def _dev_checked(self, i, n_in, si, o, so, no):
        assert self.process_dev(i, n_in, o, so) == no

    def process_dev(self, in_ptr, n_in, out_ptr, out_stride):
        got = C.c_size_t(0)
        check(self._c_process_dev(self._h, C.c_void_p(in_ptr), n_in, C.c_void_p(out_ptr), out_stride, C.byref(got)))
        return got.value

    def set_taps(self, c, taps):
        taps = np.ascontiguousarray(taps, np.int32).reshape(-1, 2)
        assert taps.shape[0] == self.order
        check(self._c_set_taps(self._h, int(c), _p(taps, True)))

    def set_shift(self, c, lut_inc, negative):
        check(self._c_set_shift(self._h, int(c), lut_inc, int(bool(negative))))

    def set_mode(self, c, mode):
        check(self._c_set_mode(self._h, int(c), int(mode)))

    def modes(self):
        m = (C.c_int * self.channels)()
        check(self._c_get_modes(self._h, m, self.channels))
        return list(m)

    def set_input_format(self, fmt):
        check(self._c_set_input_format(self._h, fmt))
        self._in = (np.uint8 if fmt == abi.IN_CU8 else np.int16, 2)

    def reset(self, keep_history=False, keep_fm=False):
        check(self._c_reset(self._h, int(bool(keep_history)) | (2 if keep_fm else 0)))


class BaseBandI16(IQBaseBandI16):
    _create, _in = "sdrhip_bb_i16_create", (np.int16, 0)


class IQBaseBandI8(IQBaseBandI16):
    _create, _in = "sdrhip_iqbb_i8_create", (np.int8, 2)
    _out_dtype = property(lambda self: np.int8 if self.epilogue == EPI_NONE else np.int16)


class FIR(_Counted):
    _prefix, _calls = "sdrhip_fir", "kernel_names last_kernels out_count process process_dev reset set_taps"

    def __init__(self, ctx, kind, alpha, decim=1, channels=1, max_in=65536, epilogue=EPI_NONE):
        super().__init__()
        alpha = np.ascontiguousarray(alpha, np.float64)
        self.ctx, self.kind, self.channels, self.decim, self.epilogue = ctx, kind, channels, decim, epilogue
        self.order = alpha.shape[0]
        self._out_dtype = np.int16 if kind == FIR_CS16_EXACT else np.float32
        self._in = (self._out_dtype, 2)
        check(abi.lib().sdrhip_fir_create(ctx.handle, kind, _p(alpha, True), alpha.shape[0], decim, channels, max_in, epilogue,
                                          C.byref(self._h)))

    def kernel_names(self, n_in=0):
        return _text(self._c_kernel_names, self._h, n_in, size=256).split(",")

    def last_kernels(self):
        return _split_kernels(_text(self._c_last_kernels, self._h, size=4096))

    def set_taps(self, alpha):
        alpha = np.ascontiguousarray(alpha, np.float64)
        assert alpha.shape == (self.order,)
        check(self._c_set_taps(self._h, _p(alpha, True)))

# ... 395 lines not shown
```

Measured before the change: 567,100.

## Merge half-empty first and last high-plane tap steps into one MFMA step

When the high-byte tap plane's first step has an empty upper half and its last step has an empty lower half (the S=9 hot classes for CS16/CU8 input), the host builds a merged fragment by copying the last step's half into the first. The hot kernel then takes a new HM template variant that skips the high-plane MFMAs on both edge steps and issues one merged MFMA pair instead, saving one high-plane step's MFMAs per tile. This adds a runtime-selected kernel variant (more code size, an extra branch on a.hm), an extra fragment upload, an env switch, and a query API.

```diff
diff --git a/include/sdrhip.h b/include/sdrhip.h
--- a/include/sdrhip.h
+++ b/include/sdrhip.h
@@ -77,6 +77,7 @@
 int sdrhip_iqbb_i16_path(sdrhip_iqbb_i16 *h, int *path);
 int sdrhip_iqbb_i16_kernel_names(sdrhip_iqbb_i16 *h, char *buf, size_t len);
 int sdrhip_iqbb_i16_plan_info(sdrhip_iqbb_i16 *h, int *info, int n);
+int sdrhip_iqbb_i16_high_merge(sdrhip_iqbb_i16 *h, const int32_t *taps, int order, int *info, int n);
 int sdrhip_iqbb_i16_out_count(sdrhip_iqbb_i16 *h, size_t n_in, size_t *n_out);
 int sdrhip_iqbb_i16_process(sdrhip_iqbb_i16 *h, const int16_t *in_host, size_t n_in, size_t in_stride,
                             void *out_host, size_t out_stride, size_t *n_out);
diff --git a/libsdr_amd/abi.py b/libsdr_amd/abi.py
--- a/libsdr_amd/abi.py
+++ b/libsdr_amd/abi.py
@@ -78,6 +78,7 @@
         "sdrhip_iqbb_i16_process": (C.c_int, [vp, vp, sz, sz, vp, sz, psz]),
         "sdrhip_iqbb_i16_process_dev": (C.c_int, [vp, vp, sz, sz, vp, sz, psz]),
         "sdrhip_iqbb_i16_plan_info": (C.c_int, [vp, C.POINTER(C.c_int), C.c_int]),
+        "sdrhip_iqbb_i16_high_merge": (C.c_int, [vp, i32p, C.c_int, C.POINTER(C.c_int), C.c_int]),
         "sdrhip_iqbb_i16_process_dev_multi": (C.c_int, [vp, vp, sz, sz, sz, vp, sz, psz, psz]),
         "sdrhip_iqbb_i16_reset": (C.c_int, [vp, C.c_int]),
         "sdrhip_iqbb_i16_adopt_state": (C.c_int, [vp, vp, C.c_int]),
diff --git a/libsdr_amd/csrc/iqbb_common.hpp b/libsdr_amd/csrc/iqbb_common.hpp
--- a/libsdr_amd/csrc/iqbb_common.hpp
+++ b/libsdr_amd/csrc/iqbb_common.hpp
@@ -66,6 +66,7 @@
   int Dreal, base_real;
   int fin_groups, fin_out, fin_epi;
   int mb_q1, mb_p, mb_qlast; unsigned mb_magic;
+  int hm;
   unsigned long long *stamps;
 };
 
diff --git a/libsdr_amd/csrc/iqbb_hot.hpp b/libsdr_amd/csrc/iqbb_hot.hpp
--- a/libsdr_amd/csrc/iqbb_hot.hpp
+++ b/libsdr_amd/csrc/iqbb_hot.hpp
@@ -39,6 +39,8 @@
 constexpr HotLoRange hot_lo_ranges_9[] = {{1, 7}, {0, 9}};
 template <int S> constexpr HotLoRange hot_lo_full[] = {{0, S}};
 
+constexpr bool hot_hmerge_class(int S, int NH, int in) { return S == 9 && NH >= 2 && (in == HOT_CS16 || in == HOT_CU8); }
+
 constexpr int hot_steps[] = {2, 3, 5, 9, 17, 33};
 template <int S> constexpr auto &hot_ranges_of() {
   if constexpr (S == 2) return hot_ranges_2;
@@ -122,7 +124,7 @@
   return ws >= 0 && ws + win <= N && qf >= (GS == 1 ? 2 : 1) && qf + GS - 1 < n_out - 1;
 }
 
-template <int S, int S0, int NH, bool ROT, int EPI, int IN, int NW, bool DG = false, bool SD = false, int L0 = 0, int NL = S>
+template <int S, int S0, int NH, bool ROT, int EPI, int IN, int NW, bool DG = false, bool SD = false, int L0 = 0, int NL = S, bool HM = false>
 __device__ __forceinline__ void iqbb_hot_body(const HotArgs &a, const IqbbArgs &b_kernarg) {
   IqbbArgs b_late;
   const IqbbArgs &b = DG ? b_late : b_kernarg;
@@ -131,6 +133,8 @@
   constexpr bool PART = EPI == HOT_EPI_PARTIAL;
   static_assert(!PART || (DG && !SD), "partial sums: a variant of the any-D form");
   static_assert(!SD || DG, "the small-decimation form is a variant of the any-D form");
+  static_assert(!HM || (!DG && hot_hmerge_class(S, NH, IN)), "merged high-plane edge steps: the /8 form's 9-step classes");
+  auto high_step = [](int s) { return HM ? (s > S0 && s < S0 + NH - 1) : (s >= S0 && s < S0 + NH); };
 
   const int DD = DG ? a.D : 8, GS = DG ? a.GS : 64;
   static_assert(S >= 2 && S0 >= 0 && NH >= 1 && S0 + NH <= S, "high-plane range inside the K loop");
@@ -224,6 +228,8 @@
     else { const int j = p >> 1; dofs[k] = (j & 1) * HALF + (j >> 1) * 16 + (p & 1) * 8; }
   }
   const int coff = REAL ? 16 * (n + h) : h * HALF + 16 * n;
+  const int coff_m = coff + KSB * (h ? S0 : S0 + NH - 1);
+  (void)coff_m;
   const uint32_t lane_cnt = (uint32_t)(MF_BLK * n + 8 * h) * a.inc;
   const uint32_t lane_pair = (lane_cnt & 0xffffu) | ((lane_cnt + a.inc) << 16);
 
@@ -275,7 +281,7 @@
     o.uh = *reinterpret_cast<const v4i *>(ph); o.ul = o.uh;
     if (!CU8) o.ul = *reinterpret_cast<const v4i *>(pl);
     o.Al = taps_s[L0 * 64 + l]; o.Ah = o.Al;
-    if (S0 == L0) o.Ah = taps_s[S * 64 + l];
+    if (high_step(L0)) o.Ah = taps_s[(S + L0 - S0) * 64 + l];
   };
   auto stageK = [&](const char *cb, KOps &o, v16i &acc_hh, v16i &acc_mid, v16i &acc_ll) __attribute__((always_inline)) {
     constexpr int SA = L0, SB = L0 + NL;
@@ -287,17 +293,26 @@
         nx.uh = *reinterpret_cast<const v4i *>(ph + KSB * (s + 1));
         if (!CU8) nx.ul = *reinterpret_cast<const v4i *>(pl + KSB * (s + 1));
         nx.Al = taps_s[(s + 1) * 64 + l];
-        if (s + 1 >= S0 && s + 1 < S0 + NH) nx.Ah = taps_s[(S + s + 1 - S0) * 64 + l];
+        if (high_step(s + 1)) nx.Ah = taps_s[(S + s + 1 - S0) * 64 + l];
+      } else if (HM) {
+        nx.uh = *reinterpret_cast<const v4i *>(cb + (CU8 ? 0 : PLB) + coff_m);
+        if (!CU8) nx.ul = *reinterpret_cast<const v4i *>(cb + coff_m);
+        nx.Ah = taps_s[S * 64 + l];
       }
       acc_mid = __builtin_amdgcn_mfma_i32_32x32x32_i8(o.Al, o.uh, acc_mid, 0, 0, 0);
       asm volatile("" : "+v"(acc_mid));
-      if (s >= S0 && s < S0 + NH) {
+      if (high_step(s)) {
         acc_hh = __builtin_amdgcn_mfma_i32_32x32x32_i8(o.Ah, o.uh, acc_hh, 0, 0, 0);
         asm volatile("" : "+v"(acc_hh));
         if (!CU8) { acc_mid = __builtin_amdgcn_mfma_i32_32x32x32_i8(o.Ah, o.ul, acc_mid, 0, 0, 0); asm volatile("" : "+v"(acc_mid)); }
       }
       if (!CU8) { acc_ll = __builtin_amdgcn_mfma_i32_32x32x32_i8(o.Al, o.ul, acc_ll, 0, 0, 0); asm volatile("" : "+v"(acc_ll)); }
       o = nx;
+    }
+    if (HM) {
+      acc_hh = __builtin_amdgcn_mfma_i32_32x32x32_i8(o.Ah, o.uh, acc_hh, 0, 0, 0);
+      asm volatile("" : "+v"(acc_hh));
+      if (!CU8) { acc_mid = __builtin_amdgcn_mfma_i32_32x32x32_i8(o.Ah, o.ul, acc_mid, 0, 0, 0); asm volatile("" : "+v"(acc_mid)); }
     }
   };
   int tm_sp = 8, tm_a0 = 0, tm_a1 = 0;
@@ -937,14 +952,19 @@
           if (!CU8) {
             const v4i ul = *reinterpret_cast<const v4i *>(pl + KSB * s_);
             acc_ll = __builtin_amdgcn_mfma_i32_32x32x32_i8(Al, ul, acc_ll, 0, 0, 0);
-            if (s_ >= S0 && s_ < S0 + NH) {
+            if (high_step(s_)) {
               const v4i Ah = taps_s[(S + s_ - S0) * 64 + l];
               acc_hh = __builtin_amdgcn_mfma_i32_32x32x32_i8(Ah, uh, acc_hh, 0, 0, 0);
               acc_mid = __builtin_amdgcn_mfma_i32_32x32x32_i8(Ah, ul, acc_mid, 0, 0, 0);
             }
-          } else if (s_ >= S0 && s_ < S0 + NH) {
+          } else if (high_step(s_)) {
             acc_hh = __builtin_amdgcn_mfma_i32_32x32x32_i8(taps_s[(S + s_ - S0) * 64 + l], uh, acc_hh, 0, 0, 0);
           }
+        }
+        if (HM) {
+          const v4i Am = taps_s[S * 64 + l];
+          acc_hh = __builtin_amdgcn_mfma_i32_32x32x32_i8(Am, *reinterpret_cast<const v4i *>(cb + (CU8 ? 0 : PLB) + coff_m), acc_hh, 0, 0, 0);
+          if (!CU8) acc_mid = __builtin_amdgcn_mfma_i32_32x32x32_i8(Am, *reinterpret_cast<const v4i *>(cb + coff_m), acc_mid, 0, 0, 0);
         }
         if (DG) {
           const int s0 = a.base0_rel + (q0 + gw) * DD;
@@ -1009,6 +1029,9 @@
 constexpr int K1_MINWAVES = 4;
 template <int S, int S0, int NH, bool ROT, int EPI, int IN, int NW, int L0 = 0, int NL = S>
 __global__ __launch_bounds__(64 * NW, K1_MINWAVES) void iqbb_hot_kernel(const HotArgs a, const IqbbArgs b) {
+  if constexpr (hot_hmerge_class(S, NH, IN)) {
+    if (a.hm) { iqbb_hot_body<S, S0, NH, ROT, EPI, IN, NW, false, false, L0, NL, true>(a, b); return; }
+  }
   iqbb_hot_body<S, S0, NH, ROT, EPI, IN, NW, false, false, L0, NL>(a, b);
 }
 template <int S, int S0, int NH, bool ROT, int EPI, int IN, int NW = 4>
diff --git a/libsdr_amd/csrc/iqbb_i16.hip b/libsdr_amd/csrc/iqbb_i16.hip
--- a/libsdr_amd/csrc/iqbb_i16.hip
+++ b/libsdr_amd/csrc/iqbb_i16.hip
@@ -648,6 +648,63 @@
   }
   return planes;
 }
+
+struct ComplexTapVectors {
+  int OPm;
+  std::vector<int> are, aim;
+  ComplexTapVectors(const int32_t *taps, int order, int S) : OPm(16 * (S - 1) + 1), are(2 * OPm, 0), aim(2 * OPm, 0) {
+    const int padm = OPm - order;
+    for (int i = 0; i < order; i++) {
+      const int kr = taps[2 * i], ki = taps[2 * i + 1];
+      are[2 * (padm + i)] = kr; are[2 * (padm + i) + 1] = -ki;
+      aim[2 * (padm + i)] = ki; aim[2 * (padm + i) + 1] = kr;
+    }
+  }
+  void pack(int S, bool permuted, std::vector<int8_t> &frag, uint64_t &ah_mask, uint64_t &al_mask) const {
+    frag.assign((size_t)S * 2 * 64 * 16, 0);
+    for (int st = 0; st < S; st++)
+      for (int l = 0; l < 64; l++)
+        for (int j = 0; j < 16; j++) {
+          const int m = l & 31, hh = l >> 5;
+          int t = m >> 1, comp = m & 1, ah, al;
+          if (permuted) hot_row(m, t, comp);
+          const int idx = 32 * st + 16 * hh + j - 2 * t;
+          split_planes((idx >= 0 && idx < 2 * OPm) ? (comp ? aim[idx] : are[idx]) : 0, ah, al);
+          frag[(((size_t)(2 * st) * 64 + l) * 16) + j] = (int8_t)ah;
+          if (ah != 0) ah_mask |= (uint64_t)1 << st;
+          if (al != 0) al_mask |= (uint64_t)1 << st;
+          frag[(((size_t)(2 * st + 1) * 64 + l) * 16) + j] = (int8_t)al;
+        }
+  }
+};
+
+void pick_ranges(int S, uint64_t ah_mask, uint64_t al_mask, bool d8, bool trim, int &hot_range, int &lo_range) {
+  auto covers = [](uint64_t mask, int first, int n) { return (mask & ~((((uint64_t)1 << n) - 1u) << first)) == 0; };
+  int nr = 0, nl = 0;
+  const HotRange *rg = hot_ranges(S, &nr);
+  for (int r = 0; r < nr && hot_range < 0; r++)
+    if (covers(ah_mask, rg[r].S0, rg[r].NH)) hot_range = r;
+  if (!d8 || hot_range < 0) return;
+  const HotLoRange *lr = hot_lo_ranges(S, &nl);
+  for (int r = 0; r < nl && lo_range < 0; r++) {
+    const bool inside = rg[hot_range].S0 >= lr[r].L0 && rg[hot_range].S0 + rg[hot_range].NH <= lr[r].L0 + lr[r].NL;
+    if ((covers(al_mask, lr[r].L0, lr[r].NL) && inside && trim) || r == nl - 1) lo_range = r;
+  }
+}
+
+bool high_edges_merge(const std::vector<int8_t> &frag, int S, int kind, const HotRange &r) {
+  if (!hot_hmerge_class(S, r.NH, kind)) return false;
+  const int8_t *first = frag.data() + (size_t)(2 * r.S0) * 64 * 16, *last = frag.data() + (size_t)(2 * (r.S0 + r.NH - 1)) * 64 * 16;
+  for (int i = 0; i < 32 * 16; i++)
+    if (first[i] != 0 || last[32 * 16 + i] != 0) return false;
+  return true;
+}
+void merge_high_edges(std::vector<int8_t> &frag, const HotRange &r) {
+  int8_t *first = frag.data() + (size_t)(2 * r.S0) * 64 * 16;
+  const int8_t *last = frag.data() + (size_t)(2 * (r.S0 + r.NH - 1)) * 64 * 16;
+  std::copy(last, last + 32 * 16, first);
+}
+bool env_is_zero(const char *name) { const char *e = getenv(name); return e && e[0] == '0'; }
 }
 
 struct sdrhip_iqbb_i16 {
@@ -669,6 +726,8 @@
   int hot_range = -1;
   int lo_range = -1;
   bool env_trim = true;
+  bool env_hmerge = true;
+  int hm = 0;
   int in_cu8 = 0, real = 0, i8 = 0;
   int path = 0, S = 0, cre = 0, cim = 0;
   uint64_t ah_mask = 0;
@@ -694,7 +753,7 @@
 
 
   void load_taps(const int32_t *taps) {
-    ah_mask = 0; al_mask = 0; hot_range = -1; lo_range = -1;
+    ah_mask = 0; al_mask = 0; hot_range = -1; lo_range = -1; hm = 0;
     std::vector<uint2> tp(OP);
     pack_valu_taps(taps, order, OP, real, tp.data());
     if (path == 4) {
@@ -719,29 +778,13 @@
       if (!tapfrag.p) tapfrag.alloc((size_t)S * 2 * 64);
       tapfrag.upload(reinterpret_cast<const v4i *>(frag.data()), (size_t)S * 2 * 64, ctx->stream);
     } else if (path >= 1) {
-      const int OPm = 16 * (S - 1) + 1, padm = OPm - order;
-      std::vector<int> are(2 * OPm, 0), aim(2 * OPm, 0);
-      for (int i = 0; i < order; i++) {
-        const int kr = taps[2 * i], ki = taps[2 * i + 1];
-        are[2 * (padm + i)] = kr; are[2 * (padm + i) + 1] = -ki;
-        aim[2 * (padm + i)] = ki; aim[2 * (padm + i) + 1] = kr;
-      }
-      cre = planes_const(are.data(), 2 * OPm); cim = planes_const(aim.data(), 2 * OPm);
-      std::vector<int8_t> frag((size_t)S * 2 * 64 * 16, 0);
-      auto build = [&](bool permuted) {
-        for (int st = 0; st < S; st++)
-          for (int l = 0; l < 64; l++)
-            for (int j = 0; j < 16; j++) {
-              const int m = l & 31, hh = l >> 5;
-              int t = m >> 1, comp = m & 1, ah, al;
-              if (permuted) hot_row(m, t, comp);
-              const int idx = 32 * st + 16 * hh + j - 2 * t;
-              split_planes((idx >= 0 && idx < 2 * OPm) ? (comp ? aim[idx] : are[idx]) : 0, ah, al);
-              frag[(((size_t)(2 * st) * 64 + l) * 16) + j] = (int8_t)ah;
-              if (ah != 0) ah_mask |= (uint64_t)1 << st;
-              if (al != 0) al_mask |= (uint64_t)1 << st;
-              frag[(((size_t)(2 * st + 1) * 64 + l) * 16) + j] = (int8_t)al;
-            }
+      const ComplexTapVectors tv(taps, order, S);
+      cre = planes_const(tv.are.data(), 2 * tv.OPm); cim = planes_const(tv.aim.data(), 2 * tv.OPm);
+      std::vector<int8_t> frag;
+      auto build = [&](bool permuted) { tv.pack(S, permuted, frag, ah_mask, al_mask); };
+      auto upload_hot = [&]() {
+        if (!tapfrag_hot.p) tapfrag_hot.alloc((size_t)S * 2 * 64);
+        tapfrag_hot.upload(reinterpret_cast<const v4i *>(frag.data()), (size_t)S * 2 * 64, ctx->stream);
       };
       auto upload_rot = [&]() {
         std::vector<int8_t> r(frag.size());
@@ -751,32 +794,29 @@
       };
       if (path == 3) {
         build(true);
-        if (!tapfrag_hot.p) tapfrag_hot.alloc((size_t)S * 2 * 64);
-        tapfrag_hot.upload(reinterpret_cast<const v4i *>(frag.data()), (size_t)S * 2 * 64, ctx->stream);
+        upload_hot();
         upload_rot();
       }
       build(path == 1);
-      if (path == 1) upload_rot();
       if (!tapfrag.p) tapfrag.alloc((size_t)S * 2 * 64);
       tapfrag.upload(reinterpret_cast<const v4i *>(frag.data()), (size_t)S * 2 * 64, ctx->stream);
+      if (path == 1) {
+        pick_hot_ranges();
+        int nr = 0;
+        const HotRange *rg = hot_ranges(S, &nr);
+        if (hot_range >= 0 && env_hmerge && !i8 && high_edges_merge(frag, S, HOT_CS16, rg[hot_range])) {
+          hm = 1;
+          merge_high_edges(frag, rg[hot_range]);
+          upload_hot();
+        }
+        upload_rot();
+      }
     }
     if (path != 0) pick_hot_ranges();
     if (!this->taps.p) this->taps.alloc(OP);
     this->taps.upload(tp.data(), OP, ctx->stream);
   }
-  void pick_hot_ranges() {
-    auto covers = [](uint64_t mask, int first, int n) { return (mask & ~((((uint64_t)1 << n) - 1u) << first)) == 0; };
-    int nr = 0, nl = 0;
-    const HotRange *rg = hot_ranges(S, &nr);
-    for (int r = 0; r < nr && hot_range < 0; r++)
-      if (covers(ah_mask, rg[r].S0, rg[r].NH)) hot_range = r;
-    if (path != 1 || hot_range < 0) return;
-    const HotLoRange *lr = hot_lo_ranges(S, &nl);
-    for (int r = 0; r < nl && lo_range < 0; r++) {
-      const bool inside = rg[hot_range].S0 >= lr[r].L0 && rg[hot_range].S0 + rg[hot_range].NH <= lr[r].L0 + lr[r].NL;
-      if ((covers(al_mask, lr[r].L0, lr[r].NL) && inside && env_trim) || r == nl - 1) lo_range = r;
-    }
-  }
+  void pick_hot_ranges() { pick_ranges(S, ah_mask, al_mask, path == 1, env_trim, hot_range, lo_range); }
   size_t valu_lds() const { return (TI + (size_t)OP + 8 + 256 + 2 * (((size_t)CG + 3) & ~(size_t)3)) * 4 + (fast8 ? 0 : (size_t)TI * 8); }
   int hot_nw() const { int n = 0; const HotRange *rg = hot_ranges(S, &n); return rg[std::min(hot_range, n - 1)].NW; }
 
@@ -789,6 +829,7 @@
     ha.in = in_dev; ha.in_stride = (long)in_stride; ha.out = out_dev; ha.out_stride = (long)out_stride;
     ha.tapfrag = tapfrag_; ha.lut = lut.p; ha.inc = inc; ha.n0_lo = (uint32_t)(n0 - phase0); ha.negative = negative;
     ha.cre = cre; ha.cim = cim; ha.N = (int)N; ha.C = C; ha.stamps = nullptr;
+    ha.hm = 0;
     return ha;
   }
   unsigned hot_grid(HotArgs &ha, int tiles, int NW, bool resident) const {
@@ -812,7 +853,8 @@
     long t = tiles - 1;
     while (t >= 2 && !(host_hot((int)t - 1, 0) && host_hot((int)t - 1, 1) && host_hot((int)t - 1, 2) && host_hot((int)t - 1, 3))) t--;
     if (t < 2) return false;
-    HotArgs ha = hot_args(in_dev, N, in_stride, out_dev, out_stride, in_cu8 ? tapfrag_rot.p : tapfrag.p);
+    HotArgs ha = hot_args(in_dev, N, in_stride, out_dev, out_stride, in_cu8 ? tapfrag_rot.p : hm ? tapfrag_hot.p : tapfrag.p);
+    ha.hm = hm;
     ha.base0_rel = g.base0_rel; ha.OG = OG; ha.ovl = ovl; ha.t_lo = 0; ha.t_hi = tiles; ha.n_out = g.n_out;
     ha.D = 8; ha.GS = 64; ha.lpg_sh = 0; ha.inv_d = 0.125f; ha.philast = nullptr; ha.philast_stride = 0; ha.part = nullptr; ha.fin_groups = 0;
     ha.mb_p = 0; ha.mb_q1 = 0; ha.mb_qlast = 0; ha.mb_magic = 0;
@@ -1122,6 +1164,7 @@
       { const char *e = getenv("SDRHIP_IQBB_WGPCU"); if (e) h->env_wgpcu = std::max(1, atoi(e)); }
       { const char *e = getenv("SDRHIP_IQBB_FM_RESIDENT"); if (e) h->env_fm_resident = atoi(e) != 0; }
       { const char *e = getenv("SDRHIP_IQBB_TRIM"); if (e && e[0] == '0') h->env_trim = false; }
+      h->env_hmerge = !env_is_zero("SDRHIP_IQBB_HMERGE");
       const char *force = getenv("SDRHIP_IQBB_PATH");
       if (force && !strcmp(force, "valu")) mfma_ok = false;
       h->path = mfma_ok ? 1 : 0;
@@ -1247,6 +1290,39 @@
       const bool lo = hot && h->lo_range >= 0 && h->lo_range < lcnt;
       info[9] = lo ? lr[h->lo_range].L0 : 0; info[10] = lo ? lr[h->lo_range].NL : (hot ? h->S : 0);
     }
+  });
+}
+
+int sdrhip_iqbb_i16_high_merge(sdrhip_iqbb_i16 *h, const int32_t *taps, int order, int *info, int n) {
+  return guarded([&] {
+    SDRHIP_REQUIRE(info && n >= 7, SDRHIP_E_INVALID, "info must hold 7 ints");
+    int path, S, hot_range = -1, lo_range = -1, hm = 0;
+    if (h) {
+      path = h->path; S = h->S; hot_range = h->hot_range; lo_range = h->lo_range; hm = h->hm;
+    } else {
+      SDRHIP_REQUIRE(taps, SDRHIP_E_INVALID, "NULL argument");
+      SDRHIP_REQUIRE(order >= 1 && order <= MAX_ORDER, SDRHIP_E_UNSUPPORTED, "order %d outside [1,%d]", order, MAX_ORDER);
+      const bool use_hot = !env_is_zero("SDRHIP_IQBB_HOT");
+      const char *force = getenv("SDRHIP_IQBB_PATH");
+      path = (check_taps(taps, order, false, false) && order <= (use_hot ? 513 : 257) && !(force && !strcmp(force, "valu"))) ? 1 : 0;
+      S = order <= 17 ? 2 : order <= 33 ? 3 : order <= 65 ? 5 : order <= 129 ? 9 : order <= 257 ? 17 : 33;
+      if (path == 1) {
+        std::vector<int8_t> frag;
+        uint64_t ah = 0, al = 0;
+        ComplexTapVectors(taps, order, S).pack(S, true, frag, ah, al);
+        pick_ranges(S, ah, al, true, !env_is_zero("SDRHIP_IQBB_TRIM"), hot_range, lo_range);
+        int nr = 0;
+        const HotRange *rg = hot_ranges(S, &nr);
+        hm = hot_range >= 0 && !env_is_zero("SDRHIP_IQBB_HMERGE") && high_edges_merge(frag, S, HOT_CS16, rg[hot_range]);
+      }
+    }
+    int cnt = 0, lcnt = 0;
+    const HotRange *rg = hot_ranges(S, &cnt);
+    const HotLoRange *lr = hot_lo_ranges(S, &lcnt);
+    const bool hot = path != 0 && hot_range >= 0 && hot_range < cnt, lo = hot && lo_range >= 0 && lo_range < lcnt;
+    info[0] = path; info[1] = path != 0 ? S : 0; info[2] = hot ? rg[hot_range].S0 : 0; info[3] = hot ? rg[hot_range].NH : 0;
+    info[4] = lo ? lr[lo_range].L0 : 0; info[5] = lo ? lr[lo_range].NL : (hot ? S : 0);
+    info[6] = hm;
   });
 }
 
diff --git a/libsdr_amd/nodes.py b/libsdr_amd/nodes.py
--- a/libsdr_amd/nodes.py
+++ b/libsdr_amd/nodes.py
@@ -285,8 +285,8 @@
 
 class IQBaseBandI16(_Counted):
     _prefix = "sdrhip_iqbb_i16"
-    _calls = ("path kernel_names plan_info out_count process process_dev process_dev_multi reset adopt_state set_taps set_shift "
-              "set_input_format")
+    _calls = ("path kernel_names plan_info high_merge out_count process process_dev process_dev_multi reset adopt_state set_taps "
+              "set_shift set_input_format")
     _create = "sdrhip_iqbb_i16_create"
     _assert_channels = True
 
@@ -311,6 +311,12 @@
         v = (C.c_int * 11)()
         check(self._c_plan_info(self._h, v, 11))
         return dict(zip(("path", "S", "S0", "NH", "NW", "kind", "OP", "HH", "multi_left", "L0", "NL"), list(v)))
+
+    @property
+    def high_merge(self):
+        v = (C.c_int * 7)()
+        check(self._c_high_merge(self._h, None, 0, v, 7))
+        return dict(zip(("path", "S", "S0", "NH", "L0", "NL", "hm"), list(v)))
 
     def process_dev_multi(self, in_ptr, n_buffers, n_per_buffer, in_stride, out_ptr, out_stride):
         counts = (C.c_size_t * max(1, n_buffers))()
```

After: 532,500. 6.1% lower.
